# VisionLearningGroup/UDA_PoseEstimation

Hardware: AMD Instinct MI355X
Metric: images/sec (student+teacher step) 256x256 b=32 (higher is better)
Workload: dtype bf16; 1 GPU; pose_resnet101 K=16 mean-teacher step (student fwd+bwd on 2x32, teacher fwd on 32, JointsMSE+Cons, Adam, EMA), 256x256, b=32/GPU, no AdaIN (BASELINE.json configs[1]); global_batch=32, parallelism=dp1

## Files before the change

### include/udapose.h

```cpp
#ifndef UDAPOSE_H
#define UDAPOSE_H
#include <stddef.h>
#include <stdint.h>
#ifdef __cplusplus
extern "C" {
#endif

#define UDAPOSE_OK 0
#define UDAPOSE_ERR_ARG (-1)
#define UDAPOSE_ERR_LAUNCH (-2)
#define UDAPOSE_ERR_UNSUPPORTED (-3)
#define UDAPOSE_ERR_NOT_PREPARED (-4)

int udapose_version(void);
int udapose_elem_kind(void);

typedef struct {
    int igemm_tile;
    int igemm_h3;
    int igemm_lean;
    int igemm_short_lds;
    int igemm_tap0;
    int wgrad_tile;
    int wgrad_ksplit;
    int wgrad_fastgeo;
    int wgrad_group;
    int wgrad_stages;
    int wgrad_group_stem;
    int bn_bwd_fused;
    int bn_fwd_chunked;
    int bn_bwd_chunked;
    int bn_bwd_pre_legacy;
    int igemm_wg_min;
    int wgrad_row3;
    int bn3_mask;
    int stem_fused;
    int debug_sync;
    int igemm_big_min;
    int patch_conv;
    int eval_fold;
    int bn_xcd_rows;
    int wgrad_det;
    int igemm_ns3_k;
    void* timeline;
    int wgrad_order;
    int wgrad_fastgeo_strided;
} udapose_policy;
void udapose_policy_default(udapose_policy* p);

typedef struct {
    int N, Hi, Wi, Ci;
    int Co, KH, KW, stride, pad;
    int transposed;
    int reflect;
    int upsample;
    const udapose_policy* policy;
} udapose_conv_desc;
int udapose_conv_prepare(const udapose_conv_desc* d);

#define UDAPOSE_EPI_RELU 1
#define UDAPOSE_EPI_OUT_F32 2
#define UDAPOSE_EPI_F32 4
#define UDAPOSE_EPI_SPLIT 8
void udapose_conv_out_hw(const udapose_conv_desc* d, int* Ho, int* Wo);
int udapose_conv_stat_rows(const udapose_conv_desc* d);
int udapose_conv2d_fwd(void* stream, const udapose_conv_desc* d, const void* x, const void* w_fwd, void* y, const void* res,
                       const float* bias, float* stats, int epilogue_flags);
int udapose_conv2d_bwd_data(void* stream, const udapose_conv_desc* d, const void* dy, const void* w_bwd, void* dx, const void* res,
                            int out_f32);
int udapose_conv_bwd_stat_rows(const udapose_conv_desc* d);
int udapose_conv2d_bwd_data_bn(void* stream, const udapose_conv_desc* d, const void* dy, const void* w_bwd, void* dx, const void* res,
                               int out_f32, const void* bn_y, const void* bn_z, const float* bn_mean, const float* bn_invstd,
                               const float* bn_gamma, const float* bn_beta, float* slab);
int udapose_conv2d_bwd_weight(void* stream, const udapose_conv_desc* d, const void* dy, const void* x, float* dw, int accumulate);
int udapose_cast_f32_bf16(void* stream, const float* src, void* dst, size_t n);
int udapose_transpose_cast(void* stream, const float* src, void* dst, int A, int T, int B);
int udapose_pack_strided(void* stream, const float* src, void* dst, int A, int KH, int KWp, int KW, int Bp, int B, long sa, long skh,
                         long skw, long sb);

int udapose_nchw_f32_to_nhwc_bf16(void* stream, const float* src, void* dst, int N, int C, int HW, int Cpad);
int udapose_nchw_f32_to_nhwc_f32(void* stream, const float* src, float* dst, int N, int C, int HW, int Cpad);
int udapose_nchw_f32_to_nhwc_split(void* stream, const float* src, void* dst, int N, int C, int HW, int Cpad);
int udapose_f32_to_split(void* stream, const float* src, void* dst, size_t n);
int udapose_split_to_f32(void* stream, const void* src, float* dst, size_t n);
int udapose_nhwc_to_nchw_f32(void* stream, const void* src, int src_is_f32, float* dst, int N, int C, int HW, int Cstride,
                             const float* lo, const float* hi);

int udapose_bn_finalize(void* stream, const float* stats, int stat_rows, int C, double count, const float* gamma, const float* beta,
                        float* running_mean, float* running_var, long long* num_batches_tracked, float momentum, float eps,
                        float* scale, float* shift, float* save_mean, float* save_invstd);
int udapose_bn_eval_coeff(void* stream, int C, const float* gamma, const float* beta, const float* running_mean,
                          const float* running_var, float eps, float* scale, float* shift);
int udapose_bn_apply(void* stream, const void* y, const void* res, void* z, size_t numel, int C, const float* scale, const float* shift,
                     int relu);
int udapose_bn_bwd_rows(size_t npix);
int udapose_bn_bwd(void* stream, const void* dz, int dz_is_f32, const void* z, const void* y, void* dy, void* gout, size_t npix, int C,
                   const float* gamma, const float* save_mean, const float* save_invstd, int relu, float* slab, float* coef,
                   float* dgamma, float* dbeta, float beta_acc, const float* beta);
int udapose_bn_bwd_pre(void* stream, const void* g, int g_is_f32, const void* y, void* dy, size_t npix, int C, const float* gamma,
                       const float* save_mean, const float* save_invstd, const float* slab, int rows, float* coef, float* dgamma,
                       float* dbeta, float beta_acc);

int udapose_bn_train_fwd_ex(void* stream, int kind, const void* y, const void* res, void* z, size_t npix, int C, const float* slab, int rows,
                            const float* gamma, const float* beta, const float* pre_bias, float* running_mean, float* running_var,
                            long long* num_batches_tracked, float momentum, float eps, float* scale, float* shift, float* save, int relu,
                            int fwd_chunked, int xcd_rows, unsigned char* mask, void* y16, void* z16);
int udapose_bn_bwd_ex(void* stream, const void* dz, int dz_is_f32, const void* z, const void* y, void* dy, void* gout, size_t npix, int C,
                      const float* gamma, const float* save_mean, const float* save_invstd, int relu, float* slab, float* coef,
                      float* dgamma, float* dbeta, float beta_acc, const float* beta, int chunked);
int udapose_bn_bwd_pre_ex(void* stream, const void* g, int g_is_f32, const void* y, void* dy, size_t npix, int C, const float* gamma,
                          const float* save_mean, const float* save_invstd, const float* slab, int rows, float* coef, float* dgamma,
                          float* dbeta, float beta_acc, int chunked, int legacy);
int udapose_bn_relu_maxpool3x3s2(void* stream, const void* x, void* y, unsigned char* idx, int N, int H, int W, int C, const float* scale,
                                 const float* shift);
int udapose_bn_bwd_pooled(void* stream, const void* pool_dy, const unsigned char* pool_idx, int H, int W, const void* y, void* dy, size_t npix,
                          int C, const float* gamma, const float* save_mean, const float* save_invstd, float* slab, float* coef,
                          float* dgamma, float* dbeta, float beta_acc, const float* beta);
int udapose_bn_running_update(void* stream, const float* save, int C, float* running_mean, float* running_var,
                              long long* num_batches_tracked, float momentum);
int udapose_bn_running_update_multi(void* stream, const void* d_jobs, int njobs, int max_c, const void* act, float momentum);

int udapose_maxpool3x3s2_fwd(void* stream, const void* x, void* y, unsigned char* idx, int N, int H, int W, int C);
int udapose_maxpool3x3s2_fwd_ex(void* stream, int kind, const void* x, void* y, unsigned char* idx, int N, int H, int W, int C, void* y16);
int udapose_maxpool3x3s2_bwd(void* stream, const void* dy, const unsigned char* idx, void* dx, int N, int H, int W, int C);
int udapose_maxpool2x2_ceil(void* stream, const void* x, void* y, int N, int H, int W, int C);
int udapose_maxpool2x2_ceil_f32(void* stream, const float* x, float* y, int N, int H, int W, int C);
int udapose_maxpool2x2_ceil_split(void* stream, const void* x, void* y, int N, int H, int W, int C);

typedef void* udapose_net_t;
int udapose_net_create(const int layers[4], int num_keypoints, int N, int H, int W, int fp32, udapose_net_t* out);
void udapose_net_destroy(udapose_net_t net);
int udapose_net_num_params(udapose_net_t net);
int udapose_net_num_buffers(udapose_net_t net);
long long udapose_net_param_numel(udapose_net_t net, int i);
size_t udapose_net_wpack_bytes(udapose_net_t net);
size_t udapose_net_act_bytes(udapose_net_t net);
size_t udapose_net_ws_bytes(udapose_net_t net);
void udapose_net_out_shape(udapose_net_t net, int shape[4]);
int udapose_net_set_policy(udapose_net_t net, const udapose_policy* p);
int udapose_net_get_policy(udapose_net_t net, udapose_policy* p);
int udapose_net_bind(udapose_net_t net, const void* const* h_params, void* const* h_buffers, void* wpack);
int udapose_net_bind_grads(udapose_net_t net, void* const* h_grads);
int udapose_net_pack_weights(udapose_net_t net, void* stream, const void* const* h_params, void* wpack, int with_bwd);
int udapose_net_forward(udapose_net_t net, void* stream, const float* x_nchw, const void* const* h_params, void* const* h_buffers,
                        const void* wpack, void* act, void* ws, float* out_nchw, int training, float momentum);
int udapose_net_apply_running(udapose_net_t net, void* stream, const void* act, void* const* h_buffers, float momentum);
int udapose_axpy_f32(void* stream, float* y, const float* x, size_t n);
int udapose_net_backward(udapose_net_t net, void* stream, const float* dout_nchw, const void* const* h_params, const void* wpack,
                         void* act, void* ws, void* const* h_grads, float beta);
int udapose_net_backward_part(udapose_net_t net, void* stream, const float* dout_nchw, const void* const* h_params, const void* wpack,
                              void* act, void* ws, void* const* h_grads, float beta, int part);
int udapose_net_backward_phase(udapose_net_t net, void* stream, const float* dout_nchw, const void* const* h_params, const void* wpack,
                               void* act, void* ws, void* const* h_grads, float beta, int part, int phase);
int udapose_net_wgrad_pair(udapose_net_t net, void* stream, const void* act_a, void* ws_a, void* const* h_grads_a, float beta_a,
                           const void* act_b, void* ws_b, void* const* h_grads_b, float beta_b, int part);
int udapose_net_wgrad_pair_defer(udapose_net_t net, void* stream, const void* act_a, void* ws_a, void* const* h_grads_a, float beta_a,
                                 const void* act_b, void* ws_b, void* const* h_grads_b, float beta_b, int part, int* deferred);
int udapose_net_split_sum_flush(udapose_net_t net, void* stream);
int udapose_stem_dgrad(void* stream, const void* dy, const float* w, int N, int H, int W, float* dx);
int udapose_net_input_grad(udapose_net_t net, void* stream, const void* const* h_params, void* ws, float* dx);
#define UDAPOSE_PERTURB_L2 0
#define UDAPOSE_PERTURB_LINF 1
long long udapose_perturb_ws_bytes(int N, int C, int HW);
int udapose_perturb(void* stream, const float* x, const float* g, const float* x0, int N, int C, int HW, int mode, const float* eps_dev,
                    const float* step_dev, const float* lo, const float* hi, void* ws, float* out, float* gnorm);
int udapose_wgrad_deal(const int* nblk, const int* stages, int n_units, int order, int* ent_xcd, int* ent_unit, int* ent_first, int* ent_count, int cap,
                       double* finish_out);
long long udapose_net_grad_split_param(udapose_net_t net);

int udapose_joints_mse_fwd(void* stream, const float* pred, const float* gt, const float* w, int R, int HW, float* rows, float* mean_out);
int udapose_joints_mse_bwd(void* stream, const float* pred, const float* gt, const float* w, const float* gscale, int R, int HW,
                           float* dpred);
int udapose_cons_loss_fwd(void* stream, const float* stu, const float* tea, const unsigned char* mask, int R, int HW, float* rows,
                          float* mean_out);
int udapose_cons_loss_bwd(void* stream, const float* stu, const float* tea, const unsigned char* mask, const float* gscale, int R,
                          int HW, float* dstu);
int udapose_mask_count(void* stream, const unsigned char* mask, size_t n, float* count);
int udapose_cons_loss_valid_fwd(void* stream, const float* stu, const float* tea, const unsigned char* mask, const unsigned char* valid,
                                const float* valid_count, int R, int K, int HW, float* rows, float* mean_out);
int udapose_cons_loss_valid_bwd(void* stream, const float* stu, const float* tea, const unsigned char* mask, const unsigned char* valid,
                                const float* valid_count, const float* gscale, int R, int K, int HW, float* dstu);
int udapose_joints_kl_fwd(void* stream, const float* pred, const float* gt, const float* w, float epsilon, int R, int group, int HW, float* rows,
                          float* stats, float* out);
int udapose_joints_kl_bwd(void* stream, const float* pred, const float* gt, const float* w, float epsilon, const float* stats,
                          const float* gscale, int R, int HW, float* dpred);
int udapose_entropy_loss_fwd(void* stream, const float* x, int R, int group, int HW, float threshold, float* rows, float* stats, float* out,
                             float* count);
int udapose_entropy_loss_bwd(void* stream, const float* x, const float* rows, const float* stats, const float* count, const float* gscale,
                             float threshold, int R, int HW, float* dx);
int udapose_cons_softmax_fwd(void* stream, const float* stu, const float* tea, const unsigned char* mask, const unsigned char* valid,
                             const float* valid_count, int R, int K, int HW, float* rows, float* stats, float* out);
// ... 198 lines not shown
```

### uda_poseestimation_amd/_hip.py

```python
import ctypes as C
import os

import torch

_HERE = os.path.dirname(os.path.abspath(__file__))
LIB_PATH = os.path.join(_HERE, "libudapose_hip.so")
LIB_PATHS = {"bf16": LIB_PATH, "fp16": os.path.join(_HERE, "libudapose_hip_f16.so")}
_libs = {}

vp, ci, cf, cd, sz, ll, cl = C.c_void_p, C.c_int, C.c_float, C.c_double, C.c_size_t, C.c_longlong, C.c_long


class Policy(C.Structure):
    _fields_ = [(k, C.c_int) for k in ("igemm_tile", "igemm_h3", "igemm_lean", "igemm_short_lds", "igemm_tap0", "wgrad_tile", "wgrad_ksplit",
                                       "wgrad_fastgeo", "wgrad_group", "wgrad_stages", "wgrad_group_stem", "bn_bwd_fused", "bn_fwd_chunked",
                                       "bn_bwd_chunked", "bn_bwd_pre_legacy", "igemm_wg_min", "wgrad_row3", "bn3_mask", "stem_fused", "debug_sync", "igemm_big_min", "patch_conv",
                                       "eval_fold", "bn_xcd_rows", "wgrad_det", "igemm_ns3_k")] + [("timeline", C.c_void_p), ("wgrad_order", C.c_int),
                                                                                                   ("wgrad_fastgeo_strided", C.c_int)]


def policy(**overrides):
    p = Policy()
    lib().udapose_policy_default(C.byref(p))
    for k, v in overrides.items():
        if k not in dict(Policy._fields_):
            raise KeyError(f"udapose_policy has no field {k!r}")
        setattr(p, k, v)
    return p


class ConvDesc(C.Structure):
    _fields_ = [(k, C.c_int) for k in ("N", "Hi", "Wi", "Ci", "Co", "KH", "KW", "stride", "pad", "transposed", "reflect", "upsample")] + \
               [("policy", C.POINTER(Policy))]


_SIGS = {
    "udapose_version": (ci, []),
    "udapose_elem_kind": (ci, []),
    "udapose_grad_scaler_check": (ci, [vp, vp, vp, vp, vp, ci, vp]),
    "udapose_grad_scaler_check2": (ci, [vp, vp, vp, vp, vp, ci, vp, ll]),
    "udapose_grad_scaler_update": (ci, [vp, vp, cf, cf, ci]),
    "udapose_grad_sumsq": (ci, [vp, vp, vp, vp, vp, ci, ll, vp, vp]),
    "udapose_grad_clip": (ci, [vp, vp, vp, vp, ci, vp, vp]),
    "udapose_grad_clip_restore": (ci, [vp, ci, vp, vp]),
    "udapose_policy_default": (None, [vp]),
    "udapose_conv_prepare": (ci, [vp]),
    "udapose_net_set_policy": (ci, [vp, vp]),
    "udapose_net_get_policy": (ci, [vp, vp]),
    "udapose_net_bind": (ci, [vp, vp, vp, vp]),
    "udapose_net_bind_grads": (ci, [vp, vp]),
    "udapose_conv_out_hw": (None, [vp, vp, vp]),
    "udapose_conv_stat_rows": (ci, [vp]),
    "udapose_conv2d_fwd": (ci, [vp, vp, vp, vp, vp, vp, vp, vp, ci]),
    "udapose_conv2d_bwd_data": (ci, [vp, vp, vp, vp, vp, vp, ci]),
    "udapose_conv_bwd_stat_rows": (ci, [vp]),
    "udapose_conv2d_bwd_data_bn": (ci, [vp, vp, vp, vp, vp, vp, ci, vp, vp, vp, vp, vp, vp, vp]),
    "udapose_conv2d_bwd_weight": (ci, [vp, vp, vp, vp, vp, ci]),
    "udapose_cast_f32_bf16": (ci, [vp, vp, vp, sz]),
    "udapose_transpose_cast": (ci, [vp, vp, vp, ci, ci, ci]),
    "udapose_pack_strided": (ci, [vp, vp, vp, ci, ci, ci, ci, ci, ci, cl, cl, cl, cl]),
    "udapose_nchw_f32_to_nhwc_bf16": (ci, [vp, vp, vp, ci, ci, ci, ci]),
    "udapose_nchw_f32_to_nhwc_f32": (ci, [vp, vp, vp, ci, ci, ci, ci]),
    "udapose_nhwc_to_nchw_f32": (ci, [vp, vp, ci, vp, ci, ci, ci, ci, vp, vp]),
    "udapose_nchw_f32_to_nhwc_split": (ci, [vp, vp, vp, ci, ci, ci, ci]),
    "udapose_f32_to_split": (ci, [vp, vp, vp, sz]),
    "udapose_split_to_f32": (ci, [vp, vp, vp, sz]),
    "udapose_maxpool2x2_ceil_split": (ci, [vp, vp, vp, ci, ci, ci, ci]),
    "udapose_adain_split": (ci, [vp, vp, vp, vp, ci, ci, ci, ci, cf, cf, vp, vp]),
    "udapose_bn_finalize": (ci, [vp, vp, ci, ci, cd, vp, vp, vp, vp, vp, cf, cf, vp, vp, vp, vp]),
    "udapose_bn_eval_coeff": (ci, [vp, ci, vp, vp, vp, vp, cf, vp, vp]),
    "udapose_bn_apply": (ci, [vp, vp, vp, vp, sz, ci, vp, vp, ci]),
    "udapose_bn_bwd_rows": (ci, [sz]),
    "udapose_bn_bwd": (ci, [vp, vp, ci, vp, vp, vp, vp, sz, ci, vp, vp, vp, ci, vp, vp, vp, vp, cf, vp]),
    "udapose_bn_bwd_pre": (ci, [vp, vp, ci, vp, vp, sz, ci, vp, vp, vp, vp, ci, vp, vp, vp, cf]),
    "udapose_bn_train_fwd_ex": (ci, [vp, ci, vp, vp, vp, sz, ci, vp, ci, vp, vp, vp, vp, vp, vp, cf, cf, vp, vp, vp, ci, ci, ci, vp, vp, vp]),
    "udapose_bn_bwd_ex": (ci, [vp, vp, ci, vp, vp, vp, vp, sz, ci, vp, vp, vp, ci, vp, vp, vp, vp, cf, vp, ci]),
    "udapose_bn_bwd_pre_ex": (ci, [vp, vp, ci, vp, vp, sz, ci, vp, vp, vp, vp, ci, vp, vp, vp, cf, ci, ci]),
    "udapose_bn_relu_maxpool3x3s2": (ci, [vp, vp, vp, vp, ci, ci, ci, ci, vp, vp]),
    "udapose_bn_bwd_pooled": (ci, [vp, vp, vp, ci, ci, vp, vp, sz, ci, vp, vp, vp, vp, vp, vp, vp, cf, vp]),
    "udapose_bn_running_update": (ci, [vp, vp, ci, vp, vp, vp, cf]),
    "udapose_bn_running_update_multi": (ci, [vp, vp, ci, ci, vp, cf]),
    "udapose_maxpool3x3s2_fwd_ex":(ci, [vp, ci, vp, vp, vp, ci, ci, ci, ci, vp]),
    "udapose_maxpool3x3s2_fwd": (ci, [vp, vp, vp, vp, ci, ci, ci, ci]),
    "udapose_maxpool3x3s2_bwd": (ci, [vp, vp, vp, vp, ci, ci, ci, ci]),
    "udapose_maxpool2x2_ceil": (ci, [vp, vp, vp, ci, ci, ci, ci]),
    "udapose_maxpool2x2_ceil_f32": (ci, [vp, vp, vp, ci, ci, ci, ci]),
    "udapose_net_create": (ci, [vp, ci, ci, ci, ci, ci, vp]),
    "udapose_net_destroy": (None, [vp]),
    "udapose_net_num_params": (ci, [vp]),
    "udapose_net_num_buffers": (ci, [vp]),
    "udapose_net_param_numel": (ll, [vp, ci]),
    "udapose_net_wpack_bytes": (sz, [vp]),
    "udapose_net_act_bytes": (sz, [vp]),
    "udapose_net_ws_bytes": (sz, [vp]),
    "udapose_net_out_shape": (None, [vp, vp]),
    "udapose_net_pack_weights": (ci, [vp, vp, vp, vp, ci]),
    "udapose_net_forward": (ci, [vp, vp, vp, vp, vp, vp, vp, vp, vp, ci, cf]),
    "udapose_net_apply_running": (ci, [vp, vp, vp, vp, cf]),
    "udapose_axpy_f32": (ci, [vp, vp, vp, sz]),
    "udapose_net_backward": (ci, [vp, vp, vp, vp, vp, vp, vp, vp, cf]),
    "udapose_net_backward_part": (ci, [vp, vp, vp, vp, vp, vp, vp, vp, cf, ci]),
    "udapose_net_backward_phase": (ci, [vp, vp, vp, vp, vp, vp, vp, vp, cf, ci, ci]),
    "udapose_net_wgrad_pair": (ci, [vp, vp, vp, vp, vp, cf, vp, vp, vp, cf, ci]),
    "udapose_net_wgrad_pair_defer": (ci, [vp, vp, vp, vp, vp, cf, vp, vp, vp, cf, ci, vp]),
    "udapose_net_split_sum_flush": (ci, [vp, vp]),
    "udapose_stem_dgrad": (ci, [vp, vp, vp, ci, ci, ci, vp]),
    "udapose_net_input_grad": (ci, [vp, vp, vp, vp, vp]),
    "udapose_perturb_ws_bytes": (ll, [ci, ci, ci]),
    "udapose_perturb": (ci, [vp, vp, vp, vp, ci, ci, ci, ci, vp, vp, vp, vp, vp, vp, vp]),
    "udapose_wgrad_deal": (ci, [vp, vp, ci, ci, vp, vp, vp, vp, ci, vp]),
    "udapose_net_grad_split_param": (ll, [vp]),
    "udapose_net_bind_update": (ci, [vp, vp, vp, vp, vp, vp, vp, vp, vp]),
    "udapose_net_fused_update": (ci, [vp, vp, vp, vp, vp, vp, vp, vp, vp, cf, cf, cf, cf, cf, ci, cf, vp, cf, cf, ci, ll]),
    "udapose_net_bind_update_groups": (ci, [vp, vp, ci, vp, vp, vp, vp, vp, vp, vp, vp]),
    "udapose_net_fused_update_groups": (ci, [vp, vp, vp, ci, vp, vp, vp, vp, vp, vp, cf, cf, cf, ci, ci, vp, vp, cf, cf, ci, ll]),
    "udapose_net_fused_update_dev": (ci, [vp, vp, vp, vp, vp, vp, vp, vp, vp, cf, cf, cf, cf, cf, ci, cf, vp, vp, ci, ll]),
    "udapose_net_fused_update_groups_dev": (ci, [vp, vp, vp, ci, vp, vp, vp, vp, vp, vp, cf, cf, cf, ci, ci, vp, vp, vp, ci, ll]),
    "udapose_joints_mse_fwd": (ci, [vp, vp, vp, vp, ci, ci, vp, vp]),
    "udapose_joints_mse_bwd": (ci, [vp, vp, vp, vp, vp, ci, ci, vp]),
    "udapose_cons_loss_fwd": (ci, [vp, vp, vp, vp, ci, ci, vp, vp]),
    "udapose_cons_loss_bwd": (ci, [vp, vp, vp, vp, vp, ci, ci, vp]),
    "udapose_mask_count": (ci, [vp, vp, sz, vp]),
    "udapose_cons_loss_valid_fwd": (ci, [vp, vp, vp, vp, vp, vp, ci, ci, ci, vp, vp]),
    "udapose_cons_loss_valid_bwd": (ci, [vp, vp, vp, vp, vp, vp, vp, ci, ci, ci, vp]),
    "udapose_joints_kl_fwd": (ci, [vp, vp, vp, vp, cf, ci, ci, ci, vp, vp, vp]),
    "udapose_joints_kl_bwd": (ci, [vp, vp, vp, vp, cf, vp, vp, ci, ci, vp]),
    "udapose_entropy_loss_fwd": (ci, [vp, vp, ci, ci, ci, cf, vp, vp, vp, vp]),
    "udapose_entropy_loss_bwd": (ci, [vp, vp, vp, vp, vp, vp, cf, ci, ci, vp]),
    "udapose_cons_softmax_fwd": (ci, [vp, vp, vp, vp, vp, vp, ci, ci, ci, vp, vp, vp]),
    "udapose_cons_softmax_bwd": (ci, [vp, vp, vp, vp, vp, vp, vp, vp, ci, ci, ci, vp]),
    "udapose_cons_kl_fwd": (ci, [vp, vp, vp, vp, vp, vp, ci, ci, ci, ci, vp, vp, vp]),
    "udapose_cons_kl_bwd": (ci, [vp, vp, vp, vp, vp, vp, ci, vp, vp, ci, ci, ci, vp]),
    "udapose_coral_ws_bytes": (ll, [ci, ci, ci, ci, ci]),
    "udapose_coral_fwd": (ci, [vp, vp, vp, ci, ci, ci, ci, ci, vp, vp, vp]),
    "udapose_coral_bwd": (ci, [vp, vp, vp, vp, vp, ci, ci, ci, ci, ci, vp, vp]),
    "udapose_soft_argmax_fwd": (ci, [vp, vp, ci, ci, ci, cf, ci, vp, vp, vp, vp]),
    "udapose_soft_argmax_bwd": (ci, [vp, vp, vp, vp, vp, ci, ci, ci, cf, ci, vp]),
    "udapose_coord_loss_fwd": (ci, [vp, vp, vp, vp, vp, ci, ci, ci, ci, cf, ci, ci, vp, vp, vp, vp]),
    "udapose_coord_loss_bwd": (ci, [vp, vp, vp, vp, vp, vp, vp, vp, ci, ci, ci, cf, ci, ci, vp]),
    "udapose_heatmap_argmax": (ci, [vp, vp, ci, ci, ci, vp, vp, vp, vp, vp, ci]),
    "udapose_prior_weights": (ci, [vp, vp, ci, cf, cf, ci, vp]),
    "udapose_prior_map": (ci, [vp, vp, vp, vp, vp, vp, ci, ci, ci, ci, cf, ci, vp]),
    "udapose_pair_dist_accumulate": (ci, [vp, vp, vp, ci, ci, vp]),
    "udapose_pair_dist_finish": (ci, [vp, vp, ci, vp, vp]),
    "udapose_hflip_batch": (ci, [vp, vp, vp, ci, sz, ci, ci]),
    "udapose_flip_merge": (ci, [vp, vp, vp, vp, ci, ci, ci, ci, ci, ci, vp, vp, vp, vp]),
    "udapose_refine_decode": (ci, [vp, vp, ci, ci, ci, ci, ci, cf, vp, vp, vp]),
    "udapose_kth_mask": (ci, [vp, vp, vp, ci, ci, vp, vp, vp, ci]),
# ... 126 lines not shown
```

### uda_poseestimation_amd/csrc/capi.hip

```cpp
#include <cstdio>
#include "net.h"
#include "pointwise.h"
#include "losses.h"
#include "optim.h"
#include "style.h"
#include "data.h"
#include "../../include/udapose.h"

static Policy from_c(const udapose_policy& c) {
    Policy p;
    static_cast<udapose_policy&>(p) = c;
    if (p.wgrad_stages <= 0) p.wgrad_stages = 128;
    return p;
}
static void to_c(const Policy& p, udapose_policy* c) { *c = p; }
struct Geom {
    Policy pol;
    ConvGeom g;
    explicit Geom(const udapose_conv_desc* d)
        : g{d->N, d->Hi, d->Wi, d->Ci, d->Co, d->KH, d->KW, d->stride, d->pad, d->transposed, d->reflect, d->upsample} {
        if (d->policy) { pol = from_c(*d->policy); g.pol = &pol; }
    }
};
#define S(x) ((hipStream_t)(x))
// ... 70 lines not shown
}
int udapose_bn_bwd_pre(void* stream, const void* g, int g_is_f32, const void* y, void* dy, size_t npix, int C, const float* gamma, const float* mean,
                       const float* invstd, const float* slab, int rows, float* coef, float* dgamma, float* dbeta, float beta_acc) {
    if (!g || !y || !dy || !gamma || !mean || !invstd || !slab || !coef) return UDAPOSE_ERR_ARG;
    return pw_bn_bwd_pre(S(stream), g, g_is_f32, CB16(y), B16(dy), npix, C, gamma, mean, invstd, slab, rows, coef, dgamma, dbeta, beta_acc,
                         default_policy().bn_bwd_chunked, default_policy().bn_bwd_pre_legacy);
}
int udapose_bn_train_fwd_ex(void* stream, int kind, const void* y, const void* res, void* z, size_t npix, int C, const float* slab, int rows,
                            const float* gamma, const float* beta, const float* pre_bias, float* running_mean, float* running_var,
                            long long* num_batches_tracked, float momentum, float eps, float* scale, float* shift, float* save, int relu,
                            int fwd_chunked, int xcd_rows, unsigned char* mask, void* y16, void* z16) {
    if (!y || !z || !slab || !gamma || !beta || !scale || !shift || !save || npix < 1 || rows < 1 || C < 8 || C % 8 || kind < 0 || kind > 3)
        return UDAPOSE_ERR_ARG;
    if ((kind == 3) != (y16 != nullptr) || (kind == 3) != (z16 != nullptr) || (mask && (kind == 1 || kind == 2))) return UDAPOSE_ERR_ARG;
    if (kind == 3 && UDAPOSE_ELEM_KIND != 1) return UDAPOSE_ERR_UNSUPPORTED;
    const int chunked = fwd_chunked | (xcd_rows ? (1 << 30) : 0);
    int took = 0;
    if (kind == 0 && !pre_bias)
        took = pw_bn_train_fused(S(stream), CB16(y), CB16(res), B16(z), npix, C, slab, rows, gamma, beta, running_mean, running_var,
                                 num_batches_tracked, momentum, eps, save, relu, chunked, mask);
    else if (kind >= 2 && !pre_bias)
        took = pw_bn_train_fused_split(S(stream), (const float*)y, res, z, npix, C, slab, rows, gamma, beta, running_mean, running_var,
                                       num_batches_tracked, momentum, eps, save, relu, chunked, y16, z16, mask);
    if (took < 0) return took;
    if (took) return 1 | (xcd_rows ? 2 : 0);
    int rc = pw_bn_finalize(S(stream), slab, rows, C, (double)npix, gamma, beta, running_mean, running_var, num_batches_tracked, momentum, eps, scale,
                            shift, save, save + C, pre_bias);
    if (rc != UDAPOSE_OK) return rc;
    const int xcd = xcd_rows >= 2;
    if (kind == 0) rc = pw_bn_apply(S(stream), CB16(y), CB16(res), B16(z), npix * C, C, scale, shift, relu, mask, xcd);
    else if (kind == 1) rc = pw_bn_apply_f32(S(stream), (const float*)y, (const float*)res, (float*)z, npix * C, C, scale, shift, relu);
    else rc = pw_bn_apply_split(S(stream), (const float*)y, res, z, npix * C, C, scale, shift, relu, y16, z16, mask, xcd);
    if (rc != UDAPOSE_OK) return rc;
    return (xcd && (kind == 0 || kind == 3) && pw_bn_apply_xcd_ok(npix * (C / 8), C)) ? 2 : 0;
}
int udapose_bn_bwd_ex(void* stream, const void* dz, int dz_is_f32, const void* z, const void* y, void* dy, void* gout, size_t npix, int C,
                      const float* gamma, const float* mean, const float* invstd, int relu, float* slab, float* coef, float* dgamma, float* dbeta,
                      float beta_acc, const float* beta, int chunked) {
    if (!dz || !y || !dy || !gamma || !mean || !invstd || !slab || !coef || npix < 1 || C < 8) return UDAPOSE_ERR_ARG;
    const int rc = pw_bn_bwd(S(stream), dz, dz_is_f32, CB16(z), CB16(y), B16(dy), B16(gout), npix, C, gamma, mean, invstd, relu, slab, coef, dgamma,
                             dbeta, beta_acc, beta, chunked);
    return rc != UDAPOSE_OK ? rc : pw_bn_bwd_takes_chunked(npix, C, chunked);
}
int udapose_bn_bwd_pre_ex(void* stream, const void* g, int g_is_f32, const void* y, void* dy, size_t npix, int C, const float* gamma,
                          const float* mean, const float* invstd, const float* slab, int rows, float* coef, float* dgamma, float* dbeta,
                          float beta_acc, int chunked, int legacy) {
    if (!g || !y || !dy || !gamma || !mean || !invstd || !slab || !coef || npix < 1 || C < 8) return UDAPOSE_ERR_ARG;
    const int rc = pw_bn_bwd_pre(S(stream), g, g_is_f32, CB16(y), B16(dy), npix, C, gamma, mean, invstd, slab, rows, coef, dgamma, dbeta, beta_acc,
                                 chunked, legacy);
    if (rc != UDAPOSE_OK) return rc;
    if (pw_bn_bwd_pre_takes_chunked(npix, C, rows, chunked)) return 1 | (((chunked >> 30) & 1) ? 2 : 0);
    return (!legacy && ((chunked >> 29) & 1) && pw_bn_apply_xcd_ok(npix * (C / 8), C)) ? 2 : 0;
}
int udapose_bn_relu_maxpool3x3s2(void* stream, const void* x, void* y, unsigned char* idx, int N, int H, int W, int C, const float* scale,
                                 const float* shift) {
    if (!x || !y || !scale || !shift || N < 1 || H < 1 || W < 1 || C < 8) return UDAPOSE_ERR_ARG;
    return pw_bn_relu_maxpool3x3s2(S(stream), CB16(x), B16(y), idx, N, H, W, C, scale, shift);
}
int udapose_bn_bwd_pooled(void* stream, const void* pool_dy, const unsigned char* pool_idx, int H, int W, const void* y, void* dy, size_t npix, int C,
                          const float* gamma, const float* mean, const float* invstd, float* slab, float* coef, float* dgamma, float* dbeta,
                          float beta_acc, const float* beta) {
    if (!pool_dy || !pool_idx || !y || !dy || !gamma || !mean || !invstd || !slab || !coef || H < 1 || W < 1 || npix < 1 || C < 8) return UDAPOSE_ERR_ARG;
    return pw_bn_bwd_pooled(S(stream), CB16(pool_dy), pool_idx, H, W, CB16(y), B16(dy), npix, C, gamma, mean, invstd, slab, coef, dgamma, dbeta,
                            beta_acc, beta);
}
int udapose_bn_running_update(void* stream, const float* save, int C, float* running_mean, float* running_var, long long* num_batches_tracked,
                              float momentum) {
    if (!save || !running_mean || !running_var || C < 1) return UDAPOSE_ERR_ARG;
    return pw_bn_running_update(S(stream), save, C, running_mean, running_var, num_batches_tracked, momentum);
}
int udapose_bn_running_update_multi(void* stream, const void* d_jobs, int njobs, int max_c, const void* act, float momentum) {
    if (!d_jobs || !act || njobs < 1 || max_c < 1) return UDAPOSE_ERR_ARG;
    return pw_bn_running_update_multi(S(stream), (const BnRunJob*)d_jobs, njobs, max_c, act, momentum);
}
int udapose_maxpool3x3s2_fwd_ex(void* stream, int kind, const void* x, void* y, unsigned char* idx, int N, int H, int W, int C, void* y16) {
    if (!x || !y || N < 1 || H < 1 || W < 1 || C < 8 || C % 8 || kind < 0 || kind > 3 || (kind == 3) != (y16 != nullptr)) return UDAPOSE_ERR_ARG;
    if (kind == 3 && UDAPOSE_ELEM_KIND != 1) return UDAPOSE_ERR_UNSUPPORTED;
    if (kind == 0) return pw_maxpool3x3s2_fwd(S(stream), CB16(x), B16(y), idx, N, H, W, C);
    if (kind == 1) return pw_maxpool3x3s2_fwd_f32(S(stream), (const float*)x, (float*)y, idx, N, H, W, C);
    return pw_maxpool3x3s2_fwd_split(S(stream), x, y, idx, N, H, W, C, y16);
}
int udapose_maxpool3x3s2_fwd(void* stream, const void* x, void* y, unsigned char* idx, int N, int H, int W, int C) {
    return pw_maxpool3x3s2_fwd(S(stream), CB16(x), B16(y), idx, N, H, W, C);
}
int udapose_maxpool3x3s2_bwd(void* stream, const void* dy, const unsigned char* idx, void* dx, int N, int H, int W, int C) {
    return pw_maxpool3x3s2_bwd(S(stream), CB16(dy), idx, B16(dx), N, H, W, C);
}
int udapose_maxpool2x2_ceil(void* stream, const void* x, void* y, int N, int H, int W, int C) {
    return pw_maxpool2x2_ceil(S(stream), CB16(x), B16(y), N, H, W, C);
}
int udapose_maxpool2x2_ceil_f32(void* stream, const float* x, float* y, int N, int H, int W, int C) {
    return pw_maxpool2x2_ceil_f32(S(stream), x, y, N, H, W, C);
}
int udapose_nchw_f32_to_nhwc_f32(void* stream, const float* src, float* dst, int N, int C, int HW, int Cpad) {
    return pw_nchw_f32_to_nhwc_f32(S(stream), src, dst, N, C, HW, Cpad);
}
int udapose_nchw_f32_to_nhwc_split(void* stream, const float* src, void* dst, int N, int C, int HW, int Cpad) {
    if (!src || !dst) return UDAPOSE_ERR_ARG;
    return pw_nchw_f32_to_nhwc_split(S(stream), src, dst, N, C, HW, Cpad);
}
int udapose_f32_to_split(void* stream, const float* src, void* dst, size_t n) {
    if (!src || !dst) return UDAPOSE_ERR_ARG;
    return pw_f32_to_split(S(stream), src, dst, n);
}
int udapose_split_to_f32(void* stream, const void* src, float* dst, size_t n) {
    if (!src || !dst) return UDAPOSE_ERR_ARG;
    return pw_split_to_f32(S(stream), src, dst, n);
}
int udapose_maxpool2x2_ceil_split(void* stream, const void* x, void* y, int N, int H, int W, int C) {
    if (!x || !y) return UDAPOSE_ERR_ARG;
    return pw_maxpool2x2_ceil_split(S(stream), x, y, N, H, W, C);
}

int udapose_net_create(const int layers[4], int K, int N, int H, int W, int fp32, udapose_net_t* out) {
    if (!out) return UDAPOSE_ERR_ARG;
    *out = net_create(layers, K, N, H, W, fp32);
    return *out ? UDAPOSE_OK : UDAPOSE_ERR_ARG;
}
void udapose_net_destroy(udapose_net_t n) { net_destroy(n); }
int udapose_net_set_policy(udapose_net_t n, const udapose_policy* p) {
    if (!n || !p) return UDAPOSE_ERR_ARG;
    net_set_policy(n, from_c(*p));
    return UDAPOSE_OK;
}
int udapose_net_get_policy(udapose_net_t n, udapose_policy* p) {
    if (!n || !p) return UDAPOSE_ERR_ARG;
    to_c(net_get_policy(n), p);
    return UDAPOSE_OK;
}
int udapose_net_bind(udapose_net_t n, const void* const* params, void* const* buffers, void* wpack) {
    if (!n || !params || !wpack) return UDAPOSE_ERR_ARG;
    return net_bind(n, params, buffers, wpack);
}
int udapose_net_bind_grads(udapose_net_t n, void* const* grads) {
    if (!n || !grads) return UDAPOSE_ERR_ARG;
    return net_bind_grads(n, grads);
}
int udapose_net_num_params(udapose_net_t n) { return net_num_params(n); }
int udapose_net_num_buffers(udapose_net_t n) { return net_num_buffers(n); }
long long udapose_net_param_numel(udapose_net_t n, int i) { return net_param_numel(n, i); }
size_t udapose_net_wpack_bytes(udapose_net_t n) { return net_wpack_bytes(n); }
size_t udapose_net_act_bytes(udapose_net_t n) { return net_act_bytes(n); }
size_t udapose_net_ws_bytes(udapose_net_t n) { return net_ws_bytes(n); }
void udapose_net_out_shape(udapose_net_t n, int shape[4]) { net_out_shape(n, shape); }
int udapose_net_pack_weights(udapose_net_t n, void* stream, const void* const* params, void* wpack, int with_bwd) {
    return net_pack_weights(n, S(stream), params, wpack, with_bwd);
}
int udapose_net_forward(udapose_net_t n, void* stream, const float* x, const void* const* params, void* const* buffers, const void* wpack, void* act,
                        void* ws, float* out, int training, float momentum) {
    return net_forward(n, S(stream), x, params, buffers, wpack, act, ws, out, training, momentum);
}
int udapose_net_apply_running(udapose_net_t n, void* stream, const void* act, void* const* buffers, float momentum) {
    return net_apply_running(n, S(stream), act, buffers, momentum);
}
int udapose_axpy_f32(void* stream, float* y, const float* x, size_t n) { return pw_axpy(S(stream), y, x, n); }
int udapose_net_backward(udapose_net_t n, void* stream, const float* dout, const void* const* params, const void* wpack, void* act, void* ws,
                         void* const* grads, float beta) {
    return net_backward(n, S(stream), dout, params, wpack, act, ws, grads, beta, 0, 0);
}
int udapose_net_backward_part(udapose_net_t n, void* stream, const float* dout, const void* const* params, const void* wpack, void* act,
                              void* ws, void* const* grads, float beta, int part) {
    if (part != 1 && part != 2) return UDAPOSE_ERR_ARG;
    return net_backward(n, S(stream), dout, params, wpack, act, ws, grads, beta, part, 0);
}
int udapose_net_wgrad_pair(udapose_net_t n, void* stream, const void* act_a, void* ws_a, void* const* grads_a, float beta_a, const void* act_b,
                           void* ws_b, void* const* grads_b, float beta_b, int part) {
    if (!n || !act_a || !ws_a || !grads_a || !act_b || !ws_b || !grads_b) return UDAPOSE_ERR_ARG;
    return net_wgrad_pair(n, S(stream), act_a, ws_a, grads_a, beta_a, act_b, ws_b, grads_b, beta_b, part);
}
int udapose_net_wgrad_pair_defer(udapose_net_t n, void* stream, const void* act_a, void* ws_a, void* const* grads_a, float beta_a, const void* act_b,
                                 void* ws_b, void* const* grads_b, float beta_b, int part, int* deferred) {
    if (!n || !act_a || !ws_a || !grads_a || !act_b || !ws_b || !grads_b) return UDAPOSE_ERR_ARG;
    return net_wgrad_pair_defer(n, S(stream), act_a, ws_a, grads_a, beta_a, act_b, ws_b, grads_b, beta_b, part, deferred);
}
int udapose_net_split_sum_flush(udapose_net_t n, void* stream) { return n ? net_split_sum_flush(n, S(stream)) : UDAPOSE_ERR_ARG; }
int udapose_wgrad_deal(const int* nblk, const int* stages, int n_units, int order, int* ent_xcd, int* ent_unit, int* ent_first, int* ent_count, int cap,
                       double* finish_out) {
    return net_wgrad_deal(nblk, stages, n_units, order, ent_xcd, ent_unit, ent_first, ent_count, cap, finish_out);
}
int udapose_net_backward_phase(udapose_net_t n, void* stream, const float* dout, const void* const* params, const void* wpack, void* act,
                               void* ws, void* const* grads, float beta, int part, int phase) {
    if (!n) return UDAPOSE_ERR_ARG;
    return net_backward(n, S(stream), dout, params, wpack, act, ws, grads, beta, part, phase);
}
int udapose_stem_dgrad(void* stream, const void* dy, const float* w, int N, int H, int W, float* dx) {
    return stem_dgrad(S(stream), (const elem_t*)dy, w, N, H, W, dx);
}
int udapose_net_input_grad(udapose_net_t n, void* stream, const void* const* params, void* ws, float* dx) {
    if (!n || !params || !ws || !dx) return UDAPOSE_ERR_ARG;
    return net_input_grad(n, S(stream), params, ws, dx);
}
long long udapose_perturb_ws_bytes(int N, int C, int HW) { return perturb_ws_bytes(N, C, HW); }
int udapose_perturb(void* stream, const float* x, const float* g, const float* x0, int N, int C, int HW, int mode, const float* eps_dev,
                    const float* step_dev, const float* lo, const float* hi, void* ws, float* out, float* gnorm) {
    return perturb(S(stream), x, g, x0, N, C, HW, mode, eps_dev, step_dev, lo, hi, ws, out, gnorm);
}
long long udapose_net_grad_split_param(udapose_net_t n) { return net_grad_split_param(n); }
// ... 421 lines not shown
```

### uda_poseestimation_amd/csrc/conv_plan.h

```cpp
#pragma once
#include <atomic>
#include <mutex>
#include <vector>
#include "igemm.h"

struct Policy : udapose_policy {
    Policy() : udapose_policy{} {
        igemm_tile = -1; igemm_h3 = 1; igemm_lean = 1; igemm_short_lds = 1; igemm_tap0 = 1;
        wgrad_tile = -1; wgrad_ksplit = -1; wgrad_fastgeo = 2;
        wgrad_group = 1; wgrad_stages = 128; wgrad_group_stem = 1;
        bn_bwd_fused = 1; bn_fwd_chunked = 1; bn_bwd_chunked = 1; bn_bwd_pre_legacy = 0;
        igemm_wg_min = 512; wgrad_row3 = 1; bn3_mask = 1; stem_fused = 1; debug_sync = 0;
        igemm_big_min = 0; patch_conv = 2; eval_fold = 1; bn_xcd_rows = 1; wgrad_det = 1; igemm_ns3_k = 0;
        timeline = nullptr; wgrad_order = 1; wgrad_fastgeo_strided = 1;
    }
};
inline const Policy& default_policy() { static const Policy p; return p; }

template <auto Kernel>
inline void max_dynamic_lds(int bytes) {
    static std::atomic<unsigned long long> done{0};
    static std::mutex mu;
    int dev = 0;
    (void)hipGetDevice(&dev);
    const unsigned long long bit = 1ull << (dev & 63);
    if (done.load(std::memory_order_acquire) & bit) return;
    std::lock_guard<std::mutex> lk(mu);
    if (done.load(std::memory_order_relaxed) & bit) return;
    (void)hipFuncSetAttribute((const void*)Kernel, hipFuncAttributeMaxDynamicSharedMemorySize, bytes);
    done.fetch_or(bit, std::memory_order_release);
}

struct ConvGeom {
    int N, Hi, Wi, Ci;
    int Co, KH, KW, stride, pad;
    int transposed;
    int reflect;
    int upsample;
    const Policy* pol = nullptr;
    const Policy& policy() const { return pol ? *pol : default_policy(); }
    int Ho() const { return transposed ? (Hi - 1) * stride - 2 * pad + KH : (((Hi << upsample) + 2 * pad - KH) / stride + 1); }
    int Wo() const { return transposed ? (Wi - 1) * stride - 2 * pad + KW : (((Wi << upsample) + 2 * pad - KW) / stride + 1); }
    bool smallc() const { return Ci == 8; }
    int KWp() const { return smallc() ? ((KW + 7) & ~7) : KW; }
    int wtaps() const { return KH * KWp(); }
};

struct TapPlan {
    std::vector<IgTap> taps;
    int nclass = 1;
    IgClass cls[4];
    const IgTap* d_taps = nullptr;
};

const TapPlan* get_tap_plan(const ConvGeom& g, int direction, hipStream_t stream = nullptr);
int conv_prepare(const ConvGeom& g);

int igemm_pick_tile(int M, int Co, int nclass, int K, int h3_ok, const Policy& pol);
int conv_h3_ok(const ConvGeom& g);
int igemm_stat_rows(int M, int Co, int nclass, int tile);
int igemm_launch(IgParams& p, int tile, hipStream_t stream, const Policy& pol);
int wgrad_pick_tile(int Rdim, int Cdim, int smallc, const Policy& pol);
int wgrad_launch(WgParams& p, int tile, int accumulate, hipStream_t stream, const Policy& pol);
int wgrad_parts_plan(int M, int Ci, int Co, int total_taps, int* tile_out);
int wgrad_launch_parts(WgParams& p, float* parts, hipStream_t stream);
#define WG_STAMP_BLOCKS (1 << 17)
#define WG_CLASSES 2
// ... 39 lines not shown
```

### uda_poseestimation_amd/csrc/net.h

```cpp
#pragma once
#include "conv_plan.h"

void* net_create(const int layers[4], int K, int N, int H, int W, int mode);
void net_destroy(void* h);
void net_set_policy(void* h, const Policy& p);
const Policy& net_get_policy(void* h);
int net_num_params(void* h);
int net_num_buffers(void* h);
long long net_param_numel(void* h, int i);
size_t net_wpack_bytes(void* h);
size_t net_act_bytes(void* h);
size_t net_ws_bytes(void* h);
void net_out_shape(void* h, int* shp);
int net_bind(void* h, const void* const* params, void* const* buffers, void* wpack_);
int net_pack_weights(void* h, hipStream_t s, const void* const* params, void* wpack_, int with_bwd);
int net_forward(void* h, hipStream_t s, const float* x_nchw, const void* const* params, void* const* buffers, const void* wpack_, void* act_, void* ws_,
                float* out_nchw, int training, float momentum);
int net_wgrad_pair(void* h, hipStream_t s, const void* actA, void* wsA, void* const* gradsA, float betaA, const void* actB, void* wsB,
                   void* const* gradsB, float betaB, int part);
int net_wgrad_pair_defer(void* h, hipStream_t s, const void* actA, void* wsA, void* const* gradsA, float betaA, const void* actB, void* wsB,
                         void* const* gradsB, float betaB, int part, int* deferred);
int net_split_sum_flush(void* h, hipStream_t s);
int net_wgrad_deal(const int* nblk, const int* stages, int n_units, int order, int* ent_xcd, int* ent_unit, int* ent_first, int* ent_count, int cap,
                   double* finish_out);
int net_backward(void* h, hipStream_t s, const float* dout_nchw, const void* const* params, const void* wpack_, void* act_, void* ws_,
                 void* const* grads, float beta, int part, int phase);
int net_input_grad(void* h, hipStream_t s, const void* const* params, void* ws_, float* dx);
int net_apply_running(void* h, hipStream_t s, const void* act_, void* const* buffers, float momentum);
int net_bind_grads(void* h, void* const* grads);
long long net_grad_split_param(void* h);
int net_bind_update_groups(void* hs, void* ht, int kind, void* const* params_s, void* const* grads, void* const* h_m, void* const* h_v,
                           void* const* params_t, void* wpack_s_, void* wpack_t_, const int* group_idx);
int net_bind_update(void* hs, void* ht, void* const* params_s, void* const* grads, void* const* h_m, void* const* h_v, void* const* params_t,
                    void* wpack_s_, void* wpack_t_);
int net_fused_update(void* hs, void* ht, hipStream_t s, void* const* params_s, void* const* grads, void* const* h_m, void* const* params_t,
                     void* wpack_s_, void* wpack_t_, float lr, float beta1, float beta2, float eps, float wd, int step, float gscale,
                     float* dev_state, float alpha, float oma, int do_adam, long long grad2_delta, const float* ema_dev);
int net_fused_update_groups(void* hs, void* ht, hipStream_t s, int kind, void* const* params_s, void* const* grads, void* const* h_m,
                            void* const* params_t, void* wpack_s_, void* wpack_t_, float beta1, float beta2, float eps, int nesterov, int ngroups,
                            float* const* states, const float* wds, float alpha, float oma, int do_opt, long long grad2_delta, const float* ema_dev);
int prof_before(hipStream_t s, int kind, double flops);
void prof_after(hipStream_t s, int token);
void prof_begin();
int prof_end(double* out);
```

### uda_poseestimation_amd/csrc/net.hip

```cpp
#include <algorithm>
#include <deque>
#include <functional>
#include <queue>
#include <cstdio>
#include <cstdlib>
#include <string>
#include <type_traits>
#include <vector>
#include "net.h"
#include "pointwise.h"
#include "optim.h"

namespace {

inline size_t align_up(size_t v, size_t a = 256) { return (v + a - 1) / a * a; }
static thread_local int t_dbg_sync = 0;
struct DbgSyncScope { int prev; explicit DbgSyncScope(int on) : prev(t_dbg_sync) { t_dbg_sync = on; } ~DbgSyncScope() { t_dbg_sync = prev; } };
#define CK(expr) do { int _e = (expr); \
    if (t_dbg_sync) { fprintf(stderr, "[udapose] net.hip:%d %s\n", __LINE__, #expr); fflush(stderr); \
        if (hipDeviceSynchronize() != hipSuccess) { fprintf(stderr, "[udapose] FAILED at net.hip:%d\n", __LINE__); return UDAPOSE_ERR_LAUNCH; } } \
    if (_e != UDAPOSE_OK) return _e; } while (0)

struct ConvL {
    ConvGeom g;
// ... 241 lines not shown
        for (int k = 0; k < SC_COUNT; ++k) n.sc.off[k] = act_alloc(n, n.sc.need[k]);
    }
    const int hw_out = layout(n);
    const int Hc = hw_out >> 16, Wc = hw_out & 0xffff;

    size_t max_slab = 0, max_act = 0;
    auto upd = [&](const ConvL& c) {
        const size_t rows = (size_t)conv_stat_rows(c.g);
        max_slab = std::max(max_slab, rows * 2 * c.g.Co * 4);
        max_act = std::max(max_act, (size_t)n.N * c.g.Ho() * c.g.Wo() * c.g.Co * 2);
        max_act = std::max(max_act, (size_t)n.N * c.g.Hi * c.g.Wi * c.g.Ci * 2);
    };
    for_each_conv(n, upd);
    max_slab = std::max(max_slab, (size_t)1024 * 2 * 2048 * 4);
    size_t o = 0;
    n.ws_slab = o; o = align_up(o + max_slab);
    n.ws_slabf = o; o = align_up(o + max_slab);
    n.ws_coef = o; o = align_up(o + (size_t)3 * 2048 * 4 + 2 * 2048 * 4);
    for_each_conv(n, [&](ConvL& c) { c.g.pol = &n.policy; });
    n.head.g.pol = &n.policy;
    if (n.fwd_only) {
        n.ws_bytes = o;
        return np;
    }
    n.gbuf_bytes = align_up(2 * max_act);
    for (int i = 0; i < 6; ++i) { n.ws_gbuf[i] = o; o += n.gbuf_bytes; }
    n.ws_dyhead = o; o = align_up(o + (size_t)N * Hc * Wc * 64 * 2);
    n.ws_dwtmp = o; o = align_up(o + std::max((size_t)64 * 56 * 8 * 4, (size_t)64 * 256 * 4));
    auto dyb = [&](ConvL& c) { c.dy_off = o; o = align_up(o + (size_t)n.N * c.g.Ho() * c.g.Wo() * c.g.Co * 2); };
    for_each_conv(n, dyb);
    n.ws_wgpart = o;
    n.ws_bytes = o;
    return np;
}

struct Pool {
    char* base; size_t off[6]; bool used[6] = {false, false, false, false, false, false};
    elem_t* get() { for (int i = 0; i < 6; ++i) if (!used[i]) { used[i] = true; return (elem_t*)(base + off[i]); } return nullptr; }
    void put(const void* p) { for (int i = 0; i < 6; ++i) if ((char*)p == base + off[i]) used[i] = false; }
};

int pack_conv(hipStream_t s, const Net& n, const ConvL& c, const void* const* params, char* wpack) {
    const float* w = (const float*)params[c.w_idx];
    const ConvGeom& g = c.g;
    if (g.smallc()) {
        if (n.f32 == 2) return pw_pack_strided_split(s, w, wpack + c.wf_off, g.Co, g.KH, g.KWp(), g.KW, 8, 3, (long)g.KH * g.KW * 3, (long)g.KW * 3, 3, 1);
        if (n.f32) return pw_pack_strided_f32(s, w, (float*)(wpack + c.wf_off), g.Co, g.KH, g.KWp(), g.KW, 8, 3, (long)g.KH * g.KW * 3, (long)g.KW * 3, 3, 1);
        return pw_pack_strided(s, w, (elem_t*)(wpack + c.wf_off), g.Co, g.KH, g.KWp(), g.KW, 8, 3, (long)g.KH * g.KW * 3, (long)g.KW * 3, 3, 1);
    }
    if (n.f32 != 1) return UDAPOSE_ERR_UNSUPPORTED;
    return g.transposed ? pw_transpose_f32(s, w, (float*)(wpack + c.wf_off), g.Ci, g.KH * g.KW, g.Co) : UDAPOSE_OK;
}

int conv_bn_fwd(hipStream_t s, const Net& n, const ConvL& c, const BnL& b, const void* const* params, void* const* buffers, const char* wpack,
                char* act, char* ws, int training, float momentum, const elem_t* res, int relu, bool upd, bool no_apply = false) {
    ConvEpilogue e;
    float* slab = (float*)(ws + n.ws_slab);
    float* scale = (float*)(ws + n.ws_coef);
    float* shift = scale + 2048;
    float* save = (float*)(act + b.save_off);
    e.stats = training ? slab : nullptr;
    e.f32 = n.f32 != 0;
    e.split = n.f32 == 2;
    e.out_f32 = n.f32 == 2;
    const float* pre_bias = c.bias_idx >= 0 ? (const float*)params[c.bias_idx] : nullptr;
    e.bias = pre_bias;
    unsigned char* mask = (b.mask_off && n.policy.bn3_mask && relu) ? (unsigned char*)(act + b.mask_off) : nullptr;
    const bool sh = n.strict && training;
    void* y16 = sh ? (void*)(act + c.y_off) : nullptr;
    void* z16 = sh ? (void*)(act + b.z_off) : nullptr;
    const void* wptr = (n.f32 == 1 && !c.g.smallc() && !c.g.transposed) ? params[c.w_idx] : (const void*)(wpack + c.wf_off);
    const float* gamma = (const float*)params[b.g_idx];
    const float* beta = (const float*)params[b.b_idx];
    float* rm = upd ? (float*)buffers[b.rm_idx] : nullptr;
    float* rv = upd ? (float*)buffers[b.rv_idx] : nullptr;
    long long* nbt = upd ? (long long*)buffers[b.nbt_idx] : nullptr;
    const int chunked = n.policy.bn_fwd_chunked | (n.policy.bn_xcd_rows ? (1 << 30) : 0);
    if (!training && !no_apply && !pre_bias && n.policy.eval_fold) {
        CK(pw_bn_eval_coeff(s, b.C, gamma, beta, (const float*)buffers[b.rm_idx], (const float*)buffers[b.rv_idx], 1e-5f, scale, shift));
        e.stats = nullptr;
        e.scale = scale; e.bias = shift; e.relu = relu;
        e.res = res;
        e.out_f32 = 0;
        return conv_fprop(s, c.g, (const elem_t*)(act + c.fin_off), (const elem_t*)wptr, act + b.fz_off, e);
    }
    CK(conv_fprop(s, c.g, (const elem_t*)(act + c.fin_off), (const elem_t*)wptr, act + c.fy_off, e));
    if (training && !n.f32 && !no_apply && !pre_bias) {
        const int took = pw_bn_train_fused(s, (const elem_t*)(act + c.y_off), res, (elem_t*)(act + b.z_off), b.npix, b.C, slab, conv_stat_rows(c.g), gamma,
                                           beta, rm, rv, nbt, momentum, 1e-5f, save, relu, chunked, mask);
        if (took < 0) return took;
        if (took) return UDAPOSE_OK;
    }
    if (training && n.f32 == 2 && !no_apply && !pre_bias) {
        const int took = pw_bn_train_fused_split(s, (const float*)(act + c.fy_off), res, act + b.fz_off, b.npix, b.C, slab, conv_stat_rows(c.g), gamma, beta,
                                                 rm, rv, nbt, momentum, 1e-5f, save, relu, chunked, y16, z16, sh ? mask : nullptr);
        if (took < 0) return took;
        if (took) return UDAPOSE_OK;
    }
    if (training)
        CK(pw_bn_finalize(s, slab, conv_stat_rows(c.g), b.C, (double)b.npix, gamma, beta, rm, rv, nbt, momentum, 1e-5f, scale, shift, save,
                          save + b.C, pre_bias));
    else
        CK(pw_bn_eval_coeff(s, b.C, gamma, beta, (const float*)buffers[b.rm_idx], (const float*)buffers[b.rv_idx], 1e-5f, scale, shift));
    if (no_apply) return UDAPOSE_OK;
    if (n.f32 == 2)
        return pw_bn_apply_split(s, (const float*)(act + c.fy_off), res, act + b.fz_off, b.npix * b.C, b.C, scale, shift, relu, y16, z16, sh ? mask : nullptr,
                                 n.policy.bn_xcd_rows >= 2);
    if (n.f32)
        return pw_bn_apply_f32(s, (const float*)(act + c.y_off), (const float*)res, (float*)(act + b.z_off), b.npix * b.C, b.C, scale, shift, relu);
    return pw_bn_apply(s, (const elem_t*)(act + c.y_off), res, (elem_t*)(act + b.z_off), b.npix * b.C, b.C, scale, shift, relu, mask, n.policy.bn_xcd_rows >= 2);
}

}

void* net_create(const int layers[4], int K, int N, int H, int W, int mode) {
    if (K < 1 || K > 64 || N < 1 || H % 32 || W % 32 || (mode & 0xff) > 3 || (mode >> 10)) return nullptr;
    if ((mode & 0xff) == 3 && ((mode >> 9) & 1 || UDAPOSE_ELEM_KIND != 1)) return nullptr;
    return build(layers, K, N, H, W, mode);
}
void net_destroy(void* h) {
    delete (Net*)h;
}
void net_set_policy(void* h, const Policy& p) { ((Net*)h)->policy = p; }
const Policy& net_get_policy(void* h) { return ((Net*)h)->policy; }
int net_num_params(void* h) { return ((Net*)h)->n_params; }
int net_num_buffers(void* h) { return ((Net*)h)->n_buffers; }
long long net_param_numel(void* h, int i) { return ((Net*)h)->param_numel[i]; }
size_t net_wpack_bytes(void* h) { return ((Net*)h)->wpack_bytes; }
size_t net_act_bytes(void* h) { return ((Net*)h)->act_bytes; }
namespace { size_t wg_partial_bytes(Net& n); }
size_t net_ws_bytes(void* h) {
    Net& n = *(Net*)h;
    if ((n.f32 && !n.strict) || n.fwd_only || !n.policy.wgrad_group || !n.policy.wgrad_det) { n.ws_wgpart_bytes = 0; return n.ws_bytes; }
    n.ws_wgpart_bytes = wg_partial_bytes(n);
    return n.ws_bytes + n.ws_wgpart_bytes;
}
void net_out_shape(void* h, int* shp) { Net& n = *(Net*)h; shp[0] = n.N; shp[1] = n.K; shp[2] = n.Hout; shp[3] = n.Wout; }

namespace {
void add_pack_jobs(const Net& n, const ConvL& c, const void* const* params, char* wpack, bool with_bwd, std::vector<PackJobH>& jobs) {
    const ConvGeom& g = c.g;
    if (g.smallc()) return;
    const float* w = (const float*)params[c.w_idx];
    const int T = g.KH * g.KW;
    elem_t* wf = (elem_t*)(wpack + c.wf_off);
    elem_t* wb = (elem_t*)(wpack + c.wb_off);
    const int sp = n.f32 == 2 ? 2 : 0;
    if (sp && !n.strict) with_bwd = false;
    if (!g.transposed) {
        jobs.push_back(PackJobH{w, wf, 0, 0, 0, sp, (long long)g.Co * T * g.Ci});
        if (with_bwd) jobs.push_back(PackJobH{w, wb, g.Co, T, g.Ci, 1, 0});
    } else {
        jobs.push_back(PackJobH{w, wf, g.Ci, T, g.Co, 1 | sp, 0});
        if (with_bwd) jobs.push_back(PackJobH{w, wb, 0, 0, 0, 0, (long long)g.Ci * T * g.Co});
    }
}
int build_pack_table(Net& n, Net::PackTab& tab, const void* const* params, char* wpack, bool with_bwd) {
    std::vector<PackJobH> jobs;
    for_each_conv(n, [&](const ConvL& c) { add_pack_jobs(n, c, params, wpack, with_bwd, jobs); });
    jobs.push_back(PackJobH{(const float*)params[n.head.w_idx], (elem_t*)(wpack + n.head.wf_off), 0, 0, 0, n.f32 == 2 ? 2 : 0, (long long)n.K * 256});
    std::vector<int> bj, bs;
    for (size_t j = 0; j < jobs.size(); ++j) {
        const PackJobH& q = jobs[j];
        const long nb = (q.kind & 1) == 0 ? (long)((q.n + 8191) / 8192) : (long)((q.A + 31) / 32) * ((q.B + 31) / 32) * q.T;
        for (long k = 0; k < nb; ++k) { bj.push_back((int)j); bs.push_back((int)k); }
    }
    CK(tab.upload(jobs, bj, bs));
    tab.key0 = params[0]; tab.key1 = params[n.n_params - 1]; tab.keyw = wpack;
    return UDAPOSE_OK;
}
int build_run_jobs(Net& n, void* const* buffers) {
    std::vector<BnRunJob> jobs;
    for_each_bn(n, [&](const BnL& b) {
        jobs.push_back(BnRunJob{b.save_off, (float*)buffers[b.rm_idx], (float*)buffers[b.rv_idx], (long long*)buffers[b.nbt_idx], b.C, 0});
    });
    CK(n.d_runjobs.upload(jobs));
    n.runjobs_key = buffers[0];
    return UDAPOSE_OK;
}
}

int net_bind(void* h, const void* const* params, void* const* buffers, void* wpack_) {
    Net& n = *(Net*)h;
    char* wpack = (char*)wpack_;
    CK(for_each_conv(n, [](const ConvL& c) { return conv_prepare(c.g); }));
    { ConvGeom hg = n.head.g; CK(conv_prepare(hg)); hg.Co = 64; CK(conv_prepare(hg)); }
    if (n.f32 != 1) {
        CK(build_pack_table(n, n.pack_fwd, params, wpack, false));
// ... 2 lines not shown
    if (buffers) CK(build_run_jobs(n, buffers));
    return UDAPOSE_OK;
}

int net_pack_weights(void* h, hipStream_t s, const void* const* params, void* wpack_, int with_bwd) {
    Net& n = *(Net*)h;
    DbgSyncScope dbg(n.policy.debug_sync);
    char* wpack = (char*)wpack_;
    if (n.f32 != 1) {
        if (n.f32 == 2 && !n.strict) with_bwd = 0;
        Net::PackTab& tab = with_bwd ? n.pack_all : n.pack_fwd;
        if (!tab.jobs.d || tab.key0 != params[0] || tab.key1 != params[n.n_params - 1] || tab.keyw != (const void*)wpack)
            return UDAPOSE_ERR_NOT_PREPARED;
        CK(pack_conv(s, n, n.stem, params, wpack));
        CK(pw_pack_multi(s, tab.jobs.d, tab.blk_job.d, tab.blk_sub.d, tab.nblocks()));
        if (with_bwd)
            CK(pw_pack_strided(s, (const float*)params[n.head.w_idx], (elem_t*)(wpack + n.head.wb_off), 256, 1, 1, 1, 64, n.K, 1, 0, 0, 256));
        return UDAPOSE_OK;
    }
    return for_each_conv(n, [&](const ConvL& c) -> int { CK(pack_conv(s, n, c, params, wpack)); return UDAPOSE_OK; });
}

int net_forward(void* h, hipStream_t s, const float* x_nchw, const void* const* params, void* const* buffers, const void* wpack_, void* act_, void* ws_,
                float* out_nchw, int training, float momentum) {
    const Net& n = *(const Net*)h;
    DbgSyncScope dbg(n.policy.debug_sync);
    const bool upd = !(training & 2);
    training &= 1;
    const char* wpack = (const char*)wpack_;
    char* act = (char*)act_;
    char* ws = (char*)ws_;
    const bool sh = n.strict && training;
    if (n.f32 == 2) CK(pw_nchw_f32_to_nhwc_split(s, x_nchw, act + n.fx8_off, n.N, 3, n.H * n.W, 8, sh ? act + n.x8_off : nullptr));
    else if (n.f32) CK(pw_nchw_f32_to_nhwc_f32(s, x_nchw, (float*)(act + n.x8_off), n.N, 3, n.H * n.W, 8));
    else CK(pw_nchw_f32_to_nhwc_bf16(s, x_nchw, (elem_t*)(act + n.x8_off), n.N, 3, n.H * n.W, 8));
    const bool stem_fused = n.policy.stem_fused && !n.f32;
    CK(conv_bn_fwd(s, n, n.stem, n.stem_bn, params, buffers, wpack, act, ws, training, momentum, nullptr, 1, upd, stem_fused));
    if (stem_fused)
        CK(pw_bn_relu_maxpool3x3s2(s, (const elem_t*)(act + n.stem.y_off), (elem_t*)(act + n.pool_off), (unsigned char*)(act + n.poolidx_off), n.N,
                                   n.Hs, n.Ws, 64, (const float*)(ws + n.ws_coef), (const float*)(ws + n.ws_coef) + 2048));
    else if (n.f32 == 2)
        CK(pw_maxpool3x3s2_fwd_split(s, act + n.stem_bn.fz_off, act + n.fpool_off, (unsigned char*)(act + n.poolidx_off), n.N, n.Hs, n.Ws, 64,
                                     sh ? act + n.pool_off : nullptr));
    else if (n.f32)
        CK(pw_maxpool3x3s2_fwd_f32(s, (const float*)(act + n.stem_bn.z_off), (float*)(act + n.pool_off), (unsigned char*)(act + n.poolidx_off), n.N,
                                   n.Hs, n.Ws, 64));
    else
        CK(pw_maxpool3x3s2_fwd(s, (const elem_t*)(act + n.stem_bn.z_off), (elem_t*)(act + n.pool_off), (unsigned char*)(act + n.poolidx_off), n.N,
                               n.Hs, n.Ws, 64));
    for (auto& b : n.blocks) {
        CK(conv_bn_fwd(s, n, b.c1, b.b1, params, buffers, wpack, act, ws, training, momentum, nullptr, 1, upd));
        CK(conv_bn_fwd(s, n, b.c2, b.b2, params, buffers, wpack, act, ws, training, momentum, nullptr, 1, upd));
        const elem_t* res = (const elem_t*)(act + b.fin_off);
        if (b.has_ds) {
            CK(conv_bn_fwd(s, n, b.cd, b.bd, params, buffers, wpack, act, ws, training, momentum, nullptr, 0, upd));
            res = (const elem_t*)(act + b.fzd_off);
        }
        CK(conv_bn_fwd(s, n, b.c3, b.b3, params, buffers, wpack, act, ws, training, momentum, res, 1, upd));
    }
    for (int i = 0; i < 3; ++i) CK(conv_bn_fwd(s, n, n.up[i], n.up_bn[i], params, buffers, wpack, act, ws, training, momentum, nullptr, 1, upd));
    ConvEpilogue e;
    e.bias = (const float*)params[n.head.bias_idx];
    e.out_f32 = 1;
    e.f32 = n.f32 != 0;
    e.split = n.f32 == 2;
    const void* hwp = n.f32 == 1 ? params[n.head.w_idx] : (const void*)(wpack + n.head.wf_off);
    CK(conv_fprop(s, n.head.g, (const elem_t*)(act + n.head.fin_off), (const elem_t*)hwp, act + n.head_out_off, e));
    return pw_nhwc_to_nchw_f32(s, act + n.head_out_off, 1, out_nchw, n.N, n.K, n.Hout * n.Wout, n.K, nullptr, nullptr);
}

namespace {
int conv_bn_bwd(hipStream_t s, const Net& n, const ConvL& c, const BnL& b, const void* const* params, const char* wpack, char* act, char* ws,
                void* const* grads, float beta, Pool& pool, const void* dz, int dz_f32, elem_t* gout, int relu, const elem_t* dx_res,
                elem_t** dx_out, bool need_dx, int dx_f32, bool grouped_wgrad, const DgradBnStat* pre = nullptr, DgradBnStat* next = nullptr) {
    float* slab = (float*)(ws + n.ws_slab);
    float* coef = (float*)(ws + n.ws_coef) + 4096;
    const float* save = (const float*)(act + b.save_off);
    elem_t* dy = (elem_t*)(ws + c.dy_off);
    if (pre)
        CK(pw_bn_bwd_pre(s, dz, dz_f32, (const elem_t*)(act + c.y_off), dy, b.npix, b.C, (const float*)params[b.g_idx], save, save + b.C, pre->slab,
                         pre->rows, coef, (float*)grads[b.g_idx], (float*)grads[b.b_idx], beta, n.policy.bn_bwd_chunked | (n.policy.bn_xcd_rows ? (1 << 30) : 0) | (n.policy.bn_xcd_rows >= 2 ? (1 << 29) : 0),
                         n.policy.bn_bwd_pre_legacy));
    else
        CK(pw_bn_bwd(s, dz, dz_f32, (const elem_t*)(act + b.z_off), (const elem_t*)(act + c.y_off), dy, gout, b.npix, b.C, (const float*)params[b.g_idx],
                     save, save + b.C, relu, slab, coef, (float*)grads[b.g_idx], (float*)grads[b.b_idx], beta, (const float*)params[b.b_idx],
                     n.policy.bn_bwd_chunked));
    const elem_t* xin = (const elem_t*)(act + c.in_off);
    if (c.bias_idx >= 0 && beta == 0.f) {
        if (pw_zero(s, grads[c.bias_idx], (size_t)c.g.Co * sizeof(float)) != UDAPOSE_OK) return UDAPOSE_ERR_LAUNCH;
    }
    if (c.g.smallc() && grouped_wgrad && n.policy.wgrad_group_stem) {
    } else if (c.g.smallc()) {
        float* tmp = (float*)(ws + n.ws_dwtmp);
        CK(conv_wgrad(s, c.g, dy, xin, tmp, 0, -1));
        CK(pw_unpack_strided(s, tmp, (float*)grads[c.w_idx], c.g.Co, c.g.KH, c.g.KWp(), c.g.KW, 8, 3, (long)c.g.KH * c.g.KW * 3, (long)c.g.KW * 3, 3, 1,
                             beta));
    } else if (!grouped_wgrad) {
        CK(conv_wgrad(s, c.g, dy, xin, (float*)grads[c.w_idx], beta != 0.f, -1));
    }
    if (need_dx) {
        elem_t* dx = pool.get();
        if (!dx) return UDAPOSE_ERR_ARG;
        CK(conv_dgrad(s, c.g, dy, (const elem_t*)(wpack + c.wb_off), dx, dx_res, dx_f32, next));
        *dx_out = dx;
    }
    return UDAPOSE_OK;
}

DgradBnStat bn_stat_of(const Net& n, const ConvL& c, const BnL& b, const void* const* params, char* act, char* ws, int relu) {
    DgradBnStat st;
    const float* save = (const float*)(act + b.save_off);
    st.y = (const elem_t*)(act + c.y_off);
    st.z = relu == 1 ? (const elem_t*)(act + b.z_off) : nullptr;
    st.mask = (relu == 1 && b.mask_off && n.policy.bn3_mask) ? (const unsigned char*)(act + b.mask_off) : nullptr;
    st.mean = save; st.invstd = save + b.C;
    st.gamma = (const float*)params[b.g_idx]; st.beta = (const float*)params[b.b_idx];
    st.slab = (float*)(ws + n.ws_slabf);
    return st;
}


inline int split_block(const Net& n) { return n.layers[0] + n.layers[1]; }

struct PartSel { bool head_up; int hi, lo; bool stem; };
PartSel part_sel(const Net& n, int part) {
    const int nb = (int)n.blocks.size(), split = split_block(n);
    if (part == 1) return PartSel{true, nb - 1, split, false};
    if (part == 2) return PartSel{false, split - 1, 0, true};
    return PartSel{true, nb - 1, 0, true};
}
template <class N, class F> int for_each_conv_wgrad(N& n, const PartSel& sel, F fn) {
    int rc = UDAPOSE_OK;
    for (int i = 2; sel.head_up && rc == UDAPOSE_OK && i >= 0; --i) rc = walk_rc(fn, n.up[i]);
    for (int bi = sel.hi; rc == UDAPOSE_OK && bi >= sel.lo; --bi) {
        auto& b = n.blocks[bi];
// ... 354 lines not shown
    char* ws = (char*)ws_;
    Pool pool;
    pool.base = ws;
    for (int i = 0; i < 6; ++i) pool.off[i] = n.ws_gbuf[i];
    const bool grouped = n.policy.wgrad_group != 0;
    if (grouped && (!find_wg_group(n, grads, beta, part))) return UDAPOSE_ERR_NOT_PREPARED;
    const int HWo = n.Hout * n.Wout;
    const int split = split_block(n);
    const bool fused = n.policy.bn_bwd_fused != 0;
    DgradBnStat cur, nxt;
    bool have = false;
    elem_t* dz = nullptr;
    if (part != 2) {
    elem_t* dyh = (elem_t*)(ws + n.ws_dyhead);
    CK(pw_nchw_f32_to_nhwc_bf16(s, dout_nchw, dyh, n.N, n.K, HWo, 64));
    ConvGeom hg = n.head.g;
    hg.Co = 64;
    float* tmp = (float*)(ws + n.ws_dwtmp);
    if (!grouped) {
        CK(conv_wgrad(s, hg, dyh, (const elem_t*)(act + n.head.in_off), tmp, 0, n.K));
        CK(pw_unpack_strided(s, tmp, (float*)grads[n.head.w_idx], n.K, 1, 1, 1, 256, 256, 256, 0, 0, 1, beta));
    }
    dz = pool.get();
    if (fused) { cur = bn_stat_of(n, n.up[2], n.up_bn[2], params, act, ws, 2); have = true; }
    CK(conv_dgrad(s, hg, dyh, (const elem_t*)(wpack + n.head.wb_off), dz, nullptr, 1, have ? &cur : nullptr));
    CK(pw_plane_sum(s, dout_nchw, (float*)grads[n.head.bias_idx], n.N, n.K, HWo, beta));
    for (int i = 2; i >= 0; --i) {
        elem_t* dx = nullptr;
        if (fused) {
            if (i > 0) nxt = bn_stat_of(n, n.up[i - 1], n.up_bn[i - 1], params, act, ws, 2);
            else nxt = bn_stat_of(n, n.blocks.back().c3, n.blocks.back().b3, params, act, ws, 1);
        }
        CK(conv_bn_bwd(s, n, n.up[i], n.up_bn[i], params, wpack, act, ws, grads, beta, pool, dz, 1, nullptr, 2, nullptr, &dx, true, i > 0, grouped,
                       have ? &cur : nullptr, fused ? &nxt : nullptr));
        if (fused) cur = nxt;
        pool.put(dz);
        dz = dx;
    }
    } else {
        if (split < 1 || split >= (int)n.blocks.size() || n.split_dz_idx < 0) return UDAPOSE_ERR_ARG;
        pool.used[n.split_dz_idx] = true;
        dz = (elem_t*)(ws + pool.off[n.split_dz_idx]);
        if (fused) {
            cur = bn_stat_of(n, n.blocks[split - 1].c3, n.blocks[split - 1].b3, params, act, ws, 1);
            cur.rows = conv_dgrad_stat_rows(n.blocks[split].c1.g);
            have = true;
        }
    }
    const int bi_hi = part == 2 ? split - 1 : (int)n.blocks.size() - 1, bi_lo = part == 1 ? split : 0;
    for (int bi = bi_hi; bi >= bi_lo; --bi) {
        Block& b = n.blocks[bi];
        elem_t *dz2 = nullptr, *dz1 = nullptr, *dxd = nullptr, *dxin = nullptr;
        if (fused) nxt = bn_stat_of(n, b.c2, b.b2, params, act, ws, 2);
        CK(conv_bn_bwd(s, n, b.c3, b.b3, params, wpack, act, ws, grads, beta, pool, dz, 0, dz, 1, nullptr, &dz2, true, 0, grouped, have ? &cur : nullptr,
                       fused ? &nxt : nullptr));
        if (fused) { cur = nxt; nxt = bn_stat_of(n, b.c1, b.b1, params, act, ws, 2); }
        CK(conv_bn_bwd(s, n, b.c2, b.b2, params, wpack, act, ws, grads, beta, pool, dz2, 0, nullptr, 2, nullptr, &dz1, true, 0, grouped,
                       have ? &cur : nullptr, fused ? &nxt : nullptr));
        if (fused) cur = nxt;
        pool.put(dz2);
        const elem_t* skip = dz;
        if (b.has_ds) {
            CK(conv_bn_bwd(s, n, b.cd, b.bd, params, wpack, act, ws, grads, beta, pool, dz, 0, nullptr, 0, nullptr, &dxd, true, 0, grouped));
            skip = dxd;
        }
        const bool chain = fused && bi > 0;
        if (chain) nxt = bn_stat_of(n, n.blocks[bi - 1].c3, n.blocks[bi - 1].b3, params, act, ws, 1);
        CK(conv_bn_bwd(s, n, b.c1, b.b1, params, wpack, act, ws, grads, beta, pool, dz1, 0, nullptr, 2, skip, &dxin, true, 0, grouped,
                       have ? &cur : nullptr, chain ? &nxt : nullptr));
        if (chain) cur = nxt;
        pool.put(dz1);
        if (dxd) pool.put(dxd);
        pool.put(dz);
        dz = dxin;
    }
    if (part == 1) {
        for (int i = 0; i < 6; ++i) if ((char*)dz == ws + pool.off[i]) n.split_dz_idx = i;
        if (grouped && phase == 0) CK(run_wg_group(s, n, act, ws, grads, beta, 1));
        if (beta == 0.f) {
            if (pw_zero(s, grads[n.fc_w_idx], (size_t)1000 * 2048 * 4) != UDAPOSE_OK) return UDAPOSE_ERR_LAUNCH;
            if (pw_zero(s, grads[n.fc_b_idx], (size_t)1000 * 4) != UDAPOSE_OK) return UDAPOSE_ERR_LAUNCH;
        }
        return UDAPOSE_OK;
    }
    if (n.policy.stem_fused >= 2 && grouped && n.policy.wgrad_group_stem) {
        const BnL& sb = n.stem_bn;
        const float* save = (const float*)(act + sb.save_off);
        CK(pw_bn_bwd_pooled(s, dz, (const unsigned char*)(act + n.poolidx_off), n.Hs, n.Ws, (const elem_t*)(act + n.stem.y_off),
                            (elem_t*)(ws + n.stem.dy_off), sb.npix, sb.C, (const float*)params[sb.g_idx], save, save + sb.C, (float*)(ws + n.ws_slab),
                            (float*)(ws + n.ws_coef) + 4096, (float*)grads[sb.g_idx], (float*)grads[sb.b_idx], beta, (const float*)params[sb.b_idx]));
        pool.put(dz);
    } else {
    elem_t* dzs = pool.get();
    CK(pw_maxpool3x3s2_bwd(s, dz, (const unsigned char*)(act + n.poolidx_off), dzs, n.N, n.Hs, n.Ws, 64));
    pool.put(dz);
    elem_t* none = nullptr;
    CK(conv_bn_bwd(s, n, n.stem, n.stem_bn, params, wpack, act, ws, grads, beta, pool, dzs, 0, nullptr, 2, nullptr, &none, false, 0, grouped));
    pool.put(dzs);
    }
    if (grouped && phase == 0) CK(run_wg_group(s, n, act, ws, grads, beta, part));
    if (beta == 0.f && part == 0) {
        if (pw_zero(s, grads[n.fc_w_idx], (size_t)1000 * 2048 * 4) != UDAPOSE_OK) return UDAPOSE_ERR_LAUNCH;
        if (pw_zero(s, grads[n.fc_b_idx], (size_t)1000 * 4) != UDAPOSE_OK) return UDAPOSE_ERR_LAUNCH;
    }
    return UDAPOSE_OK;
}

int net_input_grad(void* h, hipStream_t s, const void* const* params, void* ws_, float* dx) {
    Net& n = *(Net*)h;
    if ((n.f32 && !n.strict) || n.fwd_only) return UDAPOSE_ERR_UNSUPPORTED;
    DbgSyncScope dbg(n.policy.debug_sync);
    CK(stem_dgrad(s, (const elem_t*)((const char*)ws_ + n.stem.dy_off), (const float*)params[n.stem.w_idx], n.N, n.H, n.W, dx));
    return UDAPOSE_OK;
}

int net_apply_running(void* h, hipStream_t s, const void* act_, void* const* buffers, float momentum) {
// ... 140 lines not shown
```

### uda_poseestimation_amd/csrc/pointwise.h

```cpp
#pragma once
#include "common.h"

struct BnRunJob { size_t save_off; float* rm; float* rv; long long* nbt; int C, pad; };
struct ZeroJob { long long off; long long n16; };
#define UDAPOSE_SPLIT_SUM_CHUNK 1024u
struct SumJob { long long part_off; long long dst_off; unsigned n; unsigned stride; int ks; int dst_ws; float beta; int pad; };

int pw_zero(hipStream_t s, void* p, size_t bytes);
int pw_split_sum(hipStream_t s, const SumJob* d_jobs, const int* d_blk, int nblk, void* ws, void* grad_base, void* ws2 = nullptr, void* grad_base2 = nullptr);

int pw_nchw_f32_to_nhwc_bf16(hipStream_t s, const float* src, elem_t* dst, int N, int C, int HW, int Cp);
int pw_nchw_f32_to_nhwc_f32(hipStream_t s, const float* src, float* dst, int N, int C, int HW, int Cp);
int pw_nchw_f32_to_nhwc_split(hipStream_t s, const float* src, void* dst, int N, int C, int HW, int Cp, void* dst16 = nullptr);
int pw_nhwc_to_nchw_f32(hipStream_t s, const void* src, int src_is_f32, float* dst, int N, int C, int HW, int Cs, const float* lo, const float* hi);
int pw_cast_f32_bf16(hipStream_t s, const float* src, elem_t* dst, size_t n);
int pw_transpose_cast(hipStream_t s, const float* src, elem_t* dst, int A, int T, int B);
int pw_transpose_f32(hipStream_t s, const float* src, float* dst, int A, int T, int B);
int pw_f32_to_split(hipStream_t s, const float* src, void* dst, size_t n);
int pw_split_to_f32(hipStream_t s, const void* src, float* dst, size_t n);
int pw_transpose_split(hipStream_t s, const float* src, void* dst, int A, int T, int B);
int pw_pack_strided_split(hipStream_t s, const float* src, void* dst, int A, int KH, int KWp, int KW, int Bp, int B, long sa, long skh, long skw, long sb);
int pw_pack_multi(hipStream_t s, const void* jobs, const int* blk_job, const int* blk_sub, int nblocks);
int pw_pack_strided(hipStream_t s, const float* src, elem_t* dst, int A, int KH, int KWp, int KW, int Bp, int B, long sa, long skh, long skw, long sb);
int pw_pack_strided_f32(hipStream_t s, const float* src, float* dst, int A, int KH, int KWp, int KW, int Bp, int B, long sa, long skh, long skw, long sb);
int pw_unpack_strided(hipStream_t s, const float* src, float* dst, int A, int KH, int KWp, int KW, int Bp, int B, long sa, long skh, long skw, long sb, float beta);
int pw_bn_finalize(hipStream_t s, const float* slab, int rows, int C, double count, const float* gamma, const float* beta, float* rm, float* rv,
                   long long* nbt, float momentum, float eps, float* scale, float* shift, float* save_mean, float* save_invstd, const float* pre_bias);
int pw_bn_train_fused(hipStream_t s, const elem_t* y, const elem_t* res, elem_t* z, size_t npix, int C, const float* slab, int rows,
                      const float* gamma, const float* beta, float* rm, float* rv, long long* nbt, float momentum, float eps, float* save,
                      int relu, int enabled, unsigned char* mask);
int pw_bn_train_fused_split(hipStream_t s, const float* y, const void* res, void* z, size_t npix, int C, const float* slab, int rows,
                            const float* gamma, const float* beta, float* rm, float* rv, long long* nbt, float momentum, float eps, float* save,
                            int relu, int enabled, void* y16, void* z16, unsigned char* mask);
int pw_bn_running_update_multi(hipStream_t s, const BnRunJob* d_jobs, int njobs, int maxC, const void* act, float momentum);
int pw_bn_running_update(hipStream_t s, const float* save, int C, float* rm, float* rv, long long* nbt, float momentum);
int pw_zero_multi(hipStream_t s, const ZeroJob* d_jobs, int njobs, void* base);
int pw_axpy(hipStream_t s, float* y, const float* x, size_t n);
int pw_bn_eval_coeff(hipStream_t s, int C, const float* gamma, const float* beta, const float* rm, const float* rv, float eps, float* scale, float* shift);
int pw_bn_apply_xcd_ok(size_t n8, int C);
int pw_bn_apply(hipStream_t s, const elem_t* y, const elem_t* res, elem_t* z, size_t n, int C, const float* scale, const float* shift, int relu,
                unsigned char* mask, int xcd);
int pw_bn_apply_split(hipStream_t s, const float* y, const void* res, void* z, size_t n, int C, const float* scale, const float* shift, int relu,
                      void* y16, void* z16, unsigned char* mask, int xcd);
int pw_bn_apply_f32(hipStream_t s, const float* y, const float* res, float* z, size_t n, int C, const float* scale, const float* shift, int relu);
int pw_bn_bwd_rows(size_t npix);
int pw_bn_bwd_takes_chunked(size_t npix, int C, int chunked);
int pw_bn_bwd_pre_takes_chunked(size_t npix, int C, int rows, int chunked);
int pw_bn_bwd(hipStream_t s, const void* dz, int dz_is_f32, const elem_t* z, const elem_t* y, elem_t* dy, elem_t* gout, size_t npix, int C,
              const float* gamma, const float* mean, const float* invstd, int relu, float* slab, float* coef, float* dgamma, float* dbeta,
              float beta_acc, const float* beta, int chunked);
int pw_bn_bwd_pre(hipStream_t s, const void* g, int g_is_f32, const elem_t* y, elem_t* dy, size_t npix, int C, const float* gamma, const float* mean,
                  const float* invstd, const float* slab, int rows, float* coef, float* dgamma, float* dbeta, float beta_acc, int chunked,
                  int legacy);
int pw_maxpool3x3s2_fwd(hipStream_t s, const elem_t* x, elem_t* y, unsigned char* idx, int N, int H, int W, int C);
int pw_bn_relu_maxpool3x3s2(hipStream_t s, const elem_t* x, elem_t* y, unsigned char* idx, int N, int H, int W, int C, const float* scale,
                            const float* shift);
int pw_bn_bwd_pooled(hipStream_t s, const elem_t* pool_dy, const unsigned char* pool_idx, int H, int W, const elem_t* y, elem_t* dy, size_t npix, int C,
                     const float* gamma, const float* mean, const float* invstd, float* slab, float* coef, float* dgamma, float* dbeta, float beta_acc,
                     const float* beta);
int pw_maxpool3x3s2_fwd_f32(hipStream_t s, const float* x, float* y, unsigned char* idx, int N, int H, int W, int C);
int pw_maxpool3x3s2_fwd_split(hipStream_t s, const void* x, void* y, unsigned char* idx, int N, int H, int W, int C, void* y16);
int pw_maxpool2x2_ceil_split(hipStream_t s, const void* x, void* y, int N, int H, int W, int C);
int pw_maxpool3x3s2_bwd(hipStream_t s, const elem_t* dy, const unsigned char* idx, elem_t* dx, int N, int H, int W, int C);
int pw_maxpool2x2_ceil(hipStream_t s, const elem_t* x, elem_t* y, int N, int H, int W, int C);
int pw_maxpool2x2_ceil_f32(hipStream_t s, const float* x, float* y, int N, int H, int W, int C);
int pw_plane_sum(hipStream_t s, const float* x, float* out, int N, int C, int HW, float beta);
unsigned long long sp_sat_read_pointwise(int reset);
long long perturb_ws_bytes(int N, int C, int HW);
int perturb(hipStream_t s, const float* x, const float* g, const float* x0, int N, int C, int HW, int mode, const float* eps, const float* step,
            const float* lo, const float* hi, void* ws, float* out, float* gnorm);
```

### uda_poseestimation_amd/csrc/pointwise.hip

```cpp
#include <stdlib.h>
#include <type_traits>
#include "pointwise.h"
#include "storage8.h"

namespace {

constexpr int TPB = 256;
constexpr size_t GRID_CAP = 8192;

__device__ __forceinline__ void st8_f16(_Float16* p, const float (&v)[8]) {
    half8 o;
#pragma unroll
    for (int e = 0; e < 8; ++e) o[e] = (_Float16)v[e];
    *(half8*)p = o;
}
__device__ __forceinline__ half8 st8_split_shadow(sp32* p, _Float16* h16, const float (&v)[8]) {
    half8 h, l;
    sp_split8(v, h, l);
    char* c = (char*)p;
    *(half8*)c = h;
    *(half8*)(c + 16) = l;
    *(half8*)h16 = h;
    return h;
}
// ... 158 lines not shown
            a += ((double)a0 + (double)a1) + ((double)a2 + (double)a3);
            b += ((double)b0 + (double)b1) + ((double)b2 + (double)b3);
            a += ((double)a4 + (double)a5) + ((double)a6 + (double)a7);
            b += ((double)b4 + (double)b5) + ((double)b6 + (double)b7);
        }
        for (; r + 3 * FIN_RL < rows; r += 4 * FIN_RL) {
            const float* q = slab + (size_t)r * 2 * C + c;
            const size_t st = (size_t)FIN_RL * 2 * C;
            const float a0 = q[0], b0 = q[C], a1 = q[st], b1 = q[st + C];
            const float a2 = q[2 * st], b2 = q[2 * st + C], a3 = q[3 * st], b3 = q[3 * st + C];
            a += ((double)a0 + (double)a1) + ((double)a2 + (double)a3);
            b += ((double)b0 + (double)b1) + ((double)b2 + (double)b3);
        }
        for (; r < rows; r += FIN_RL) {
            a += (double)slab[(size_t)r * 2 * C + c];
            b += (double)slab[(size_t)r * 2 * C + C + c];
        }
    }
    red[rl][cl][0] = a; red[rl][cl][1] = b;
    __syncthreads();
    for (int st = FIN_RL / 2; st > 0; st >>= 1) {
        if (rl < st) { red[rl][cl][0] += red[rl + st][cl][0]; red[rl][cl][1] += red[rl + st][cl][1]; }
        __syncthreads();
    }
    s1 = red[0][cl][0]; s2 = red[0][cl][1];
}
__device__ __forceinline__ void bn_stats_finish(double s1, double s2, double count, double& mean, double& var) {
    mean = s1 / count;
    var = s2 / count - mean * mean;
    if (var < 0.0) var = 0.0;
}
__device__ __forceinline__ float bn_invstd(double var, float eps) { return (float)(1.0 / sqrt(var + (double)eps)); }
__device__ __forceinline__ double bn_unbiased_var(double var, double count) { return count > 1.0 ? var * count / (count - 1.0) : var; }
__device__ __forceinline__ void bn_running_update1(float* __restrict__ rm, float* __restrict__ rv, int c, float momentum, float mean, float unb) {
    rm[c] = (1.f - momentum) * rm[c] + momentum * mean;
    rv[c] = (1.f - momentum) * rv[c] + momentum * unb;
}
__device__ __forceinline__ float bn_affine(float v, float sc, float sh) { return v * sc + sh; }
__device__ __forceinline__ float bn_relu(float o, int relu) { return (relu && o < 0.f) ? 0.f : o; }
template <typename T>
__device__ __forceinline__ void bn_apply8(const float (&v)[8], const float (&sc)[8], const float (&sh)[8], const T* __restrict__ res, size_t off, int relu,
                                          float (&o)[8]) {
#pragma unroll
    for (int e = 0; e < 8; ++e) o[e] = bn_affine(v[e], sc[e], sh[e]);
    if (res) {
        float r[8];
        ld8<T>(res + off, r);
#pragma unroll
        for (int e = 0; e < 8; ++e) o[e] += r[e];
    }
#pragma unroll
    for (int e = 0; e < 8; ++e) o[e] = bn_relu(o[e], relu);
}
template <typename T, bool SH>
__device__ __forceinline__ void bn_store8(T* __restrict__ z, _Float16* __restrict__ z16, unsigned char* __restrict__ mask, size_t off, size_t mi,
                                          const float (&o)[8]) {
    if constexpr (SH) {
        const half8 h = st8_split_shadow(z + off, z16 + off, o);
        if (mask) mask[mi] = mask_of(h);
    } else {
        st8<T>(z + off, o);
        if constexpr (sizeof(T) == sizeof(elem_t)) {
            if (mask) mask[mi] = mask_of_stored(o);
        }
    }
}
__device__ __forceinline__ void pix_range(size_t sp, int P, size_t npix, size_t& p0, size_t& p1) {
    p0 = sp * P;
    p1 = p0 + P;
    if (p1 > npix) p1 = npix;
}
__device__ __forceinline__ void xcd_stream_range(size_t n8, int G, int xcd, size_t& i, size_t& iend, size_t& istep) {
    i = (size_t)blockIdx.x * TPB + threadIdx.x, iend = n8, istep = (size_t)gridDim.x * TPB;
    if (xcd) {
        const size_t rows = n8 / G, per = (rows + 7) / 8;
        const unsigned x = blockIdx.x & 7u, local = blockIdx.x >> 3, nb = gridDim.x >> 3;
        const unsigned RB = TPB / G;
        size_t rend = (size_t)(x + 1) * per;
        if (rend > rows) rend = rows;
        i = ((size_t)x * per + (size_t)local * RB + threadIdx.x / G) * G + threadIdx.x % G;
        iend = rend * G;
        istep = (size_t)nb * RB * G;
    }
}
__device__ __forceinline__ void xcd_chunk_of(int xcd, int& chunk, int& sp) {
    chunk = blockIdx.x, sp = blockIdx.y;
    if (xcd) {
        const uint32_t w = xcd_remap(blockIdx.x + gridDim.x * blockIdx.y, gridDim.x * gridDim.y);
        sp = (int)(w / gridDim.x);
        chunk = (int)(w - (uint32_t)sp * gridDim.x);
    }
}
__device__ __forceinline__ void slab_colsum64(const float* __restrict__ slab, int rows, int C, int chunk, double (*part)[128]) {
    const int q = threadIdx.x & 31, rg = threadIdx.x >> 5;
    const float* base = slab + (size_t)(q >> 4) * C + chunk * 64 + (q & 15) * 4;
    double a0 = 0.0, a1 = 0.0, a2 = 0.0, a3 = 0.0;
    int r = rg;
    for (; r + 56 < rows; r += 64) {
        const f32x4 u = *(const f32x4*)(base + (size_t)r * 2 * C), v = *(const f32x4*)(base + (size_t)(r + 8) * 2 * C);
        const f32x4 w = *(const f32x4*)(base + (size_t)(r + 16) * 2 * C), x = *(const f32x4*)(base + (size_t)(r + 24) * 2 * C);
        const f32x4 u2 = *(const f32x4*)(base + (size_t)(r + 32) * 2 * C), v2 = *(const f32x4*)(base + (size_t)(r + 40) * 2 * C);
        const f32x4 w2 = *(const f32x4*)(base + (size_t)(r + 48) * 2 * C), x2 = *(const f32x4*)(base + (size_t)(r + 56) * 2 * C);
        a0 += ((double)u[0] + (double)v[0]) + ((double)w[0] + (double)x[0]);
        a1 += ((double)u[1] + (double)v[1]) + ((double)w[1] + (double)x[1]);
        a2 += ((double)u[2] + (double)v[2]) + ((double)w[2] + (double)x[2]);
        a3 += ((double)u[3] + (double)v[3]) + ((double)w[3] + (double)x[3]);
// ... 17 lines not shown
    part[rg][q * 4 + 0] = a0; part[rg][q * 4 + 1] = a1; part[rg][q * 4 + 2] = a2; part[rg][q * 4 + 3] = a3;
}
__global__ __launch_bounds__(FIN_T) void bn_finalize_k(const float* __restrict__ slab, int rows, int C, double count, const float* __restrict__ gamma,
                              const float* __restrict__ beta, float* __restrict__ running_mean, float* __restrict__ running_var,
                              long long* __restrict__ nbt, float momentum, float eps, float* __restrict__ scale,
                              float* __restrict__ shift, float* __restrict__ save_mean, float* __restrict__ save_invstd,
                              const float* __restrict__ pre_bias = nullptr) {
    __shared__ double red[FIN_RL][FIN_C][2];
    const int c = blockIdx.x * FIN_C + (threadIdx.x % FIN_C);
    if (blockIdx.x == 0 && threadIdx.x == 0 && nbt) *nbt += 1;
    double s1, s2;
    slab_colsum(slab, rows, C, c, c < C, s1, s2, red);
    if ((threadIdx.x / FIN_C) != 0 || c >= C) return;
    double mean, var;
    bn_stats_finish(s1, s2, count, mean, var);
    if (pre_bias) mean += (double)pre_bias[c];
    const float invstd = bn_invstd(var, eps);
    const float sc = bn_scale(gamma[c], invstd);
    scale[c] = sc;
    shift[c] = bn_shift(beta[c], (float)mean, sc);
    save_mean[c] = (float)mean;
    save_invstd[c] = invstd;
    const double unb = bn_unbiased_var(var, count);
    save_invstd[C + c] = (float)unb;
    if (running_mean) bn_running_update1(running_mean, running_var, c, momentum, (float)mean, (float)unb);
}
__global__ void bn_running_update_k(const float* __restrict__ save, int C, float* __restrict__ rm, float* __restrict__ rv,
                                    long long* __restrict__ nbt, float momentum) {
    const int c = blockIdx.x * TPB + threadIdx.x;
    if (c == 0 && nbt) *nbt += 1;
    if (c >= C) return;
    bn_running_update1(rm, rv, c, momentum, save[c], save[2 * C + c]);
}
__global__ void axpy_k(float* __restrict__ y, const float* __restrict__ x, size_t n4) {
    for (size_t i = (size_t)blockIdx.x * TPB + threadIdx.x; i < n4; i += (size_t)gridDim.x * TPB) {
        f32x4 a = *(f32x4*)(y + i * 4);
        const f32x4 b = *(const f32x4*)(x + i * 4);
        a[0] += b[0]; a[1] += b[1]; a[2] += b[2]; a[3] += b[3];
        *(f32x4*)(y + i * 4) = a;
    }
}
__global__ void axpy_tail_k(float* __restrict__ y, const float* __restrict__ x, int n) {
    if ((int)threadIdx.x < n) y[threadIdx.x] += x[threadIdx.x];
}
__global__ void bn_eval_coeff_k(int C, const float* __restrict__ gamma, const float* __restrict__ beta, const float* __restrict__ rm,
                                const float* __restrict__ rv, float eps, float* __restrict__ scale, float* __restrict__ shift) {
    const int c = blockIdx.x * TPB + threadIdx.x;
    if (c >= C) return;
    const float sc = gamma[c] / sqrtf(rv[c] + eps);
    scale[c] = sc;
    shift[c] = beta[c] - rm[c] * sc;
}

template <typename T, typename TY = T, bool SH = false>
__global__ void bn_apply_k(const TY* __restrict__ y, const T* __restrict__ res, T* __restrict__ z, size_t n8, int C,
                           const float* __restrict__ scale, const float* __restrict__ shift, int relu, unsigned char* __restrict__ mask = nullptr,
                           int xcd = 0, _Float16* __restrict__ y16 = nullptr, _Float16* __restrict__ z16 = nullptr) {
    const int G = C >> 3;
    const int c0 = (int)(((size_t)blockIdx.x * TPB + threadIdx.x) % G) * 8;
    float sc[8], sh[8];
    ld8<float>(scale + c0, sc);
    ld8<float>(shift + c0, sh);
    size_t i, iend, istep;
    xcd_stream_range(n8, G, xcd, i, iend, istep);
    for (; i < iend; i += istep) {
        float v[8], o[8];
        ld8<TY>(y + i * 8, v);
        if constexpr (SH) st8_f16(y16 + i * 8, v);
        bn_apply8<T>(v, sc, sh, res, i * 8, relu, o);
        bn_store8<T, SH>(z, z16, mask, i * 8, i, o);
    }
}

__host__ __device__ inline int pool3x3s2_out(int H) { return (H + 2 - 3) / 2 + 1; }
struct PoolSrc { const elem_t* dy; const unsigned char* idx; int H, W; };
__device__ __forceinline__ void pool_grad8(const PoolSrc& ps, size_t pix, int C, int c0, float (&d)[8]) {
    const int w = (int)(pix % ps.W);
    const size_t r = pix / ps.W;
    const int h = (int)(r % ps.H);
    const size_t n = r / ps.H;
    const int Ho = pool3x3s2_out(ps.H), Wo = pool3x3s2_out(ps.W);
    float acc[8];
#pragma unroll
    for (int e = 0; e < 8; ++e) acc[e] = 0.f;
    for (int ho = h >> 1; ho <= ((h + 1) >> 1); ++ho)
        for (int wo = w >> 1; wo <= ((w + 1) >> 1); ++wo) {
            if (ho >= Ho || wo >= Wo) continue;
            const int kh = h - (ho * 2 - 1), kw = w - (wo * 2 - 1);
            if (kh < 0 || kh > 2 || kw < 0 || kw > 2) continue;
            const size_t o = ((n * Ho + ho) * Wo + wo) * C + c0;
            const unsigned long long pk = *(const unsigned long long*)(ps.idx + o);
            const elem8 dd = *(const elem8*)(ps.dy + o);
            const unsigned tap = (unsigned)(kh * 3 + kw);
#pragma unroll
            for (int e = 0; e < 8; ++e)
                if (((pk >> (8 * e)) & 0xFF) == tap) acc[e] += (float)dd[e];
        }
#pragma unroll
    for (int e = 0; e < 8; ++e) d[e] = (float)(elem_t)acc[e];
}

__device__ __forceinline__ void bn_bwd_mask_coef8(int relu, const float* __restrict__ gamma, const float* __restrict__ beta, int c0, const float (&mu)[8],
                                                  const float (&is)[8], float (&sc)[8], float (&sh)[8]) {
#pragma unroll
    for (int e = 0; e < 8; ++e) { sc[e] = 0.f; sh[e] = 0.f; }
    if (relu == 2) {
        float ga[8], be[8];
        ld8<float>(gamma + c0, ga);
        ld8<float>(beta + c0, be);
        bn_scale_shift8(ga, be, mu, is, sc, sh);
    }
}
__device__ __forceinline__ elem8 bn_bwd_ldz8(int relu, const elem_t* __restrict__ z, size_t off) {
    elem8 zz = {};
    if (relu == 1) zz = *(const elem8*)(z + off);
    return zz;
}
__device__ __forceinline__ float bn_bwd_g(int relu, float d, float y, float z, float sc, float sh) {
    float gv = d;
    if (relu == 1 && !(z > 0.f)) gv = 0.f;
    if (relu == 2 && !(y * sc + sh > 0.f)) gv = 0.f;
    return gv;
// ... 70 lines not shown
#pragma unroll
    for (int e = 0; e < 8; ++e) { red[threadIdx.x][e] = s1[e]; red[threadIdx.x][8 + e] = s2[e]; }
    __syncthreads();
    if (threadIdx.x < G) {
        float a[16];
#pragma unroll
        for (int e = 0; e < 16; ++e) a[e] = 0.f;
        for (int k = 0; k < pstep; ++k)
#pragma unroll
            for (int e = 0; e < 16; ++e) a[e] += red[threadIdx.x + k * G][e];
        float* sp = slab + (size_t)blockIdx.x * 2 * C;
#pragma unroll
        for (int e = 0; e < 8; ++e) { sp[c0 + e] = a[e]; sp[C + c0 + e] = a[8 + e]; }
    }
}
__global__ __launch_bounds__(FIN_T) void bn_bwd_finalize_k(const float* __restrict__ slab, int rows, int C, double count, const float* __restrict__ gamma,
                                  const float* __restrict__ invstd, float* __restrict__ dgamma, float* __restrict__ dbeta,
                                  float beta_acc, float* __restrict__ coef) {
    __shared__ double red[FIN_RL][FIN_C][2];
    const int c = blockIdx.x * FIN_C + (threadIdx.x % FIN_C);
    double s1, s2;
    slab_colsum(slab, rows, C, c, c < C, s1, s2, red);
    if ((threadIdx.x / FIN_C) != 0 || c >= C) return;
    if (dgamma) bwd_param_acc(dgamma, dbeta, c, beta_acc, s1, s2);
    bn_bwd_coef(gamma[c], invstd[c], s1, s2, count, coef[c], coef[C + c], coef[2 * C + c]);
}
template <typename DZ, bool POOL = false>
__global__ void bn_bwd_apply_k(const DZ* __restrict__ dz, const elem_t* __restrict__ z, const elem_t* __restrict__ y,
                               elem_t* __restrict__ dy, elem_t* __restrict__ gout, size_t n8, int C, const float* __restrict__ mean,
                               const float* __restrict__ invstd, const float* __restrict__ coef, int relu, const float* __restrict__ gamma,
                               const float* __restrict__ beta, PoolSrc ps = PoolSrc{nullptr, nullptr, 0, 0}) {
    const int G = C >> 3;
    for (size_t i = (size_t)blockIdx.x * TPB + threadIdx.x; i < n8; i += (size_t)gridDim.x * TPB) {
        const int c0 = (int)(i % G) * 8;
        float d[8];
        if constexpr (POOL) pool_grad8(ps, i / G, C, c0, d);
        else ld8<DZ>(dz + i * 8, d);
        const elem8 yy = *(const elem8*)(y + i * 8);
        const elem8 zz = bn_bwd_ldz8(relu, z, i * 8);
        float mu[8], is[8], ca[8], cb[8], cc[8], sc[8], sh[8];
        ld8<float>(mean + c0, mu);
        ld8<float>(invstd + c0, is);
        ld8<float>(coef + c0, ca);
        ld8<float>(coef + C + c0, cb);
        ld8<float>(coef + 2 * C + c0, cc);
        bn_bwd_mask_coef8(relu, gamma, beta, c0, mu, is, sc, sh);
        elem8 o, go;
        bn_bwd_g8_dy8(relu, d, yy, zz, sc, sh, mu, is, ca, cb, cc, o, go);
        *(elem8*)(dy + i * 8) = o;
        if (gout) *(elem8*)(gout + i * 8) = go;
    }
}

template <typename TY, typename TZ, bool SH = false>
__global__ __launch_bounds__(TPB) void bn_apply_chunk_k(const TY* __restrict__ y, const TZ* __restrict__ res, TZ* __restrict__ z,
                                                        size_t npix, int C, const float* __restrict__ slab, int rows, double count,
                                                        const float* __restrict__ gamma, const float* __restrict__ beta, float eps,
                                                        float momentum, float* __restrict__ running_mean, float* __restrict__ running_var,
                                                        long long* __restrict__ nbt, float* __restrict__ save, int relu, int P,
                                                        unsigned char* __restrict__ mask, int xcd, _Float16* __restrict__ y16 = nullptr,
                                                        _Float16* __restrict__ z16 = nullptr) {
    __shared__ double part[8][128];
    __shared__ float scs[64], shs[64];
    int chunk, sp;
    xcd_chunk_of(xcd, chunk, sp);
    slab_colsum64(slab, rows, C, chunk, part);
    __syncthreads();
    if (threadIdx.x < 64) {
        const int col = threadIdx.x, c = chunk * 64 + col;
        double s1 = 0.0, s2 = 0.0;
#pragma unroll
        for (int k = 0; k < 8; ++k) { s1 += part[k][col]; s2 += part[k][64 + col]; }
        double mean, var;
        bn_stats_finish(s1, s2, count, mean, var);
        const float invstd = bn_invstd(var, eps);
        const float sc = bn_scale(gamma[c], invstd);
        scs[col] = sc;
        shs[col] = bn_shift(beta[c], (float)mean, sc);
        if (sp == 0) {
            const double unb = bn_unbiased_var(var, count);
            save[c] = (float)mean;
            save[C + c] = invstd;
            save[2 * C + c] = (float)unb;
            if (running_mean) bn_running_update1(running_mean, running_var, c, momentum, (float)mean, (float)unb);
            if (c == 0 && nbt) *nbt += 1;
        }
    }
    __syncthreads();
    const int cg = threadIdx.x & 7, prow = threadIdx.x >> 3;
    const int c0 = chunk * 64 + cg * 8;
    float sc[8], sh[8];
#pragma unroll
    for (int e = 0; e < 8; ++e) { sc[e] = scs[cg * 8 + e]; sh[e] = shs[cg * 8 + e]; }
    size_t p0, p1;
    pix_range(sp, P, npix, p0, p1);
    for (size_t p = p0 + prow; p < p1; p += 32) {
        const size_t off = p * C + c0;
        float v[8], o[8];
        ld8<TY>(y + off, v);
        if constexpr (SH) st8_f16(y16 + off, v);
        bn_apply8<TZ>(v, sc, sh, res, off, relu, o);
        bn_store8<TZ, SH>(z, z16, mask, off, off >> 3, o);
    }
}

template <typename DZ>
__global__ __launch_bounds__(TPB) void bn_bwd_reduce_chunk_k(const DZ* __restrict__ dz, const elem_t* __restrict__ z, const elem_t* __restrict__ y,
                                                             size_t npix, int C, const float* __restrict__ mean,
                                                             const float* __restrict__ invstd, int relu, float* __restrict__ slab, int P,
                                                             const float* __restrict__ gamma, const float* __restrict__ beta) {
    __shared__ float red[32][8][17];
    const int chunk = blockIdx.x, sp = blockIdx.y, S = gridDim.y;
    const int cg = threadIdx.x & 7, prow = threadIdx.x >> 3;
    const int c0 = chunk * 64 + cg * 8;
    float mu[8], is[8], s1[8], s2[8], sc[8], sh[8];
    ld8<float>(mean + c0, mu);
    ld8<float>(invstd + c0, is);
#pragma unroll
    for (int e = 0; e < 8; ++e) { s1[e] = 0.f; s2[e] = 0.f; }
    bn_bwd_mask_coef8(relu, gamma, beta, c0, mu, is, sc, sh);
    size_t p0, p1;
    pix_range(sp, P, npix, p0, p1);
    for (size_t p = p0 + prow; p < p1; p += 32) {
        const size_t off = p * C + c0;
        float d[8];
        ld8<DZ>(dz + off, d);
        const elem8 yy = *(const elem8*)(y + off);
        bn_bwd_sums8(relu, d, yy, bn_bwd_ldz8(relu, z, off), sc, sh, mu, is, s1, s2);
    }
#pragma unroll
    for (int e = 0; e < 8; ++e) { red[prow][cg][e] = s1[e]; red[prow][cg][8 + e] = s2[e]; }
    __syncthreads();
    if (threadIdx.x < 128) {
        const int g = threadIdx.x >> 4, e = threadIdx.x & 15;
        float a = 0.f;
        for (int k = 0; k < 32; ++k) a += red[k][g][e];
        slab[(((size_t)chunk * S + sp) * 2 + (e >> 3)) * 64 + g * 8 + (e & 7)] = a;
    }
}
template <typename DZ>
__global__ __launch_bounds__(TPB) void bn_bwd_apply_chunk_k(const DZ* __restrict__ dz, const elem_t* __restrict__ z, const elem_t* __restrict__ y,
                                                            elem_t* __restrict__ dy, elem_t* __restrict__ gout, size_t npix, int C,
                                                            const float* __restrict__ mean, const float* __restrict__ invstd, int relu,
                                                            const float* __restrict__ gamma, const float* __restrict__ beta,
                                                            const float* __restrict__ slab, int P, float* __restrict__ dgamma,
                                                            float* __restrict__ dbeta, float beta_acc) {
    __shared__ double tot[2][64];
    const int chunk = blockIdx.x, sp = blockIdx.y, S = gridDim.y;
    if (threadIdx.x < 128) {
        const int st = threadIdx.x >> 6, col = threadIdx.x & 63;
        const float* q = slab + ((size_t)chunk * S * 2 + st) * 64 + col;
        double a = 0.0;
        int k = 0;
        for (; k + 4 <= S; k += 4)
            a += ((double)q[(size_t)k * 128] + (double)q[(size_t)(k + 1) * 128]) + ((double)q[(size_t)(k + 2) * 128] + (double)q[(size_t)(k + 3) * 128]);
        for (; k < S; ++k) a += (double)q[(size_t)k * 128];
        tot[st][col] = a;
    }
    __syncthreads();
    if (sp == 0 && threadIdx.x < 64 && dgamma) bwd_param_acc(dgamma, dbeta, chunk * 64 + threadIdx.x, beta_acc, tot[0][threadIdx.x], tot[1][threadIdx.x]);
    const int cg = threadIdx.x & 7, prow = threadIdx.x >> 3;
    const int c0 = chunk * 64 + cg * 8;
    float mu[8], is[8], ga[8], ca[8], cb[8], cc[8], sc[8], sh[8];
    ld8<float>(mean + c0, mu);
    ld8<float>(invstd + c0, is);
    ld8<float>(gamma + c0, ga);
    chunk_bwd_coef8(tot, cg, (double)npix, ga, is, ca, cb, cc);
    bn_bwd_mask_coef8(relu, gamma, beta, c0, mu, is, sc, sh);
    size_t p0, p1;
    pix_range(sp, P, npix, p0, p1);
    for (size_t p = p0 + prow; p < p1; p += 32) {
        const size_t off = p * C + c0;
        float d[8];
        ld8<DZ>(dz + off, d);
        const elem8 yy = *(const elem8*)(y + off);
        elem8 o, go;
        bn_bwd_g8_dy8(relu, d, yy, bn_bwd_ldz8(relu, z, off), sc, sh, mu, is, ca, cb, cc, o, go);
        *(elem8*)(dy + off) = o;
        if (gout) *(elem8*)(gout + off) = go;
    }
}

template <typename DZ>
__global__ __launch_bounds__(TPB) void bn_bwd_apply_pre_k(const DZ* __restrict__ g, const elem_t* __restrict__ y, elem_t* __restrict__ dy, size_t n8,
                                                          int C, const float* __restrict__ mean, const float* __restrict__ invstd,
                                                          const float* __restrict__ coef, int xcd = 0) {
    const int G = C >> 3;
    const int c0 = (int)(((size_t)blockIdx.x * TPB + threadIdx.x) % G) * 8;
    float mu[8], is[8], ca[8], cb[8], cc[8];
    ld8<float>(mean + c0, mu);
    ld8<float>(invstd + c0, is);
    ld8<float>(coef + c0, ca);
    ld8<float>(coef + C + c0, cb);
    ld8<float>(coef + 2 * C + c0, cc);
    size_t i, iend, istep;
    xcd_stream_range(n8, G, xcd, i, iend, istep);
    for (; i < iend; i += istep) {
        float d[8];
        ld8<DZ>(g + i * 8, d);
        const elem8 yy = *(const elem8*)(y + i * 8);
        *(elem8*)(dy + i * 8) = bn_bwd_dy8(d, yy, mu, is, ca, cb, cc);
    }
}

template <typename DZ>
__global__ __launch_bounds__(TPB) void bn_bwd_apply_pre_chunk_k(const DZ* __restrict__ g, const elem_t* __restrict__ y, elem_t* __restrict__ dy,
                                                                size_t npix, int C, const float* __restrict__ mean,
                                                                const float* __restrict__ invstd, const float* __restrict__ gamma,
                                                                const float* __restrict__ slab, int rows, int P, float* __restrict__ dgamma,
                                                                float* __restrict__ dbeta, float beta_acc, int xcd) {
    __shared__ double part[8][128];
    __shared__ double tot[2][64];
    int chunk, sp;
    xcd_chunk_of(xcd, chunk, sp);
    slab_colsum64(slab, rows, C, chunk, part);
    __syncthreads();
    if (threadIdx.x < 128) {
        double a = 0.0;
#pragma unroll
        for (int k = 0; k < 8; ++k) a += part[k][threadIdx.x];
        tot[threadIdx.x >> 6][threadIdx.x & 63] = a;
    }
    __syncthreads();
    if (sp == 0 && threadIdx.x < 64 && dgamma) bwd_param_acc(dgamma, dbeta, chunk * 64 + threadIdx.x, beta_acc, tot[0][threadIdx.x], tot[1][threadIdx.x]);
    const int cg = threadIdx.x & 7, prow = threadIdx.x >> 3;
    const int c0 = chunk * 64 + cg * 8;
    float mu[8], is[8], ga[8], ca[8], cb[8], cc[8];
    ld8<float>(mean + c0, mu);
    ld8<float>(invstd + c0, is);
    ld8<float>(gamma + c0, ga);
    chunk_bwd_coef8(tot, cg, (double)npix, ga, is, ca, cb, cc);
    size_t p0, p1;
    pix_range(sp, P, npix, p0, p1);
    for (size_t p = p0 + prow; p < p1; p += 32) {
        const size_t off = p * C + c0;
        float d[8];
        ld8<DZ>(g + off, d);
        const elem8 yy = *(const elem8*)(y + off);
        *(elem8*)(dy + off) = bn_bwd_dy8(d, yy, mu, is, ca, cb, cc);
    }
}

template <typename T, typename F>
__device__ __forceinline__ void pool3x3s2_scan(const T* __restrict__ x, int n, int ho, int wo, int g, int H, int W, int C, const F& tap, float (&best)[8],
                                               unsigned char (&bi)[8]) {
#pragma unroll
    for (int e = 0; e < 8; ++e) { best[e] = -INFINITY; bi[e] = 0; }
    bool first = true;
#pragma unroll
    for (int kh = 0; kh < 3; ++kh)
#pragma unroll
        for (int kw = 0; kw < 3; ++kw) {
            const int h = ho * 2 - 1 + kh, w = wo * 2 - 1 + kw;
            if ((unsigned)h < (unsigned)H && (unsigned)w < (unsigned)W) {
                float v[8];
                ld8<T>(x + (((size_t)n * H + h) * W + w) * C + g * 8, v);
#pragma unroll
                for (int e = 0; e < 8; ++e) {
                    const float f = tap(v[e], e);
                    if (first || f > best[e] || f != f) { best[e] = f; bi[e] = (unsigned char)(kh * 3 + kw); }
                }
                first = false;
            }
        }
}
__device__ __forceinline__ unsigned long long pack_taps(const unsigned char (&bi)[8]) {
    unsigned long long pk = 0;
#pragma unroll
    for (int e = 0; e < 8; ++e) pk |= (unsigned long long)bi[e] << (8 * e);
    return pk;
}
struct TapIdentity {
    __device__ __forceinline__ float operator()(float v, int) const { return v; }
};
struct TapBnRelu {
    float sc[8], sh[8];
    __device__ __forceinline__ float operator()(float v, int e) const { return (float)(elem_t)bn_relu(bn_affine(v, sc[e], sh[e]), 1); }
};
template <typename T, bool SH = false>
__global__ void maxpool3x3s2_fwd_k(const T* __restrict__ x, T* __restrict__ y, unsigned char* __restrict__ idx, int N, int H,
                                   int W, int C, int Ho, int Wo, _Float16* __restrict__ y16 = nullptr) {
    const int G = C >> 3;
    const size_t total = (size_t)N * Ho * Wo * G;
    for (size_t i = (size_t)blockIdx.x * TPB + threadIdx.x; i < total; i += (size_t)gridDim.x * TPB) {
        int n, ho, wo, g;
        nhwg_of(i, G, Ho, Wo, n, ho, wo, g);
        float best[8];
        unsigned char bi[8];
        pool3x3s2_scan<T>(x, n, ho, wo, g, H, W, C, TapIdentity{}, best, bi);
        if constexpr (SH) (void)st8_split_shadow(y + i * 8, y16 + i * 8, best);
        else st8<T>(y + i * 8, best);
        if (idx) *(unsigned long long*)(idx + i * 8) = pack_taps(bi);
// ... 160 lines not shown
    hipLaunchKernelGGL(pack_strided_k<sp32>, dim3(grid_for((size_t)A * KH * KWp * Bp, TPB, GRID_CAP)), dim3(TPB), 0, s, src, (sp32*)dst, A, KH, KWp, KW, Bp, B, sa, skh, skw, sb);
    return udapose_check_launch();
}
int pw_pack_multi(hipStream_t s, const void* jobs, const int* blk_job, const int* blk_sub, int nblocks) {
    if (nblocks <= 0) return UDAPOSE_OK;
    hipLaunchKernelGGL(pack_multi_k, dim3(nblocks), dim3(TPB), 0, s, (const PackJob*)jobs, blk_job, blk_sub);
    return udapose_check_launch();
}
int pw_pack_strided(hipStream_t s, const float* src, elem_t* dst, int A, int KH, int KWp, int KW, int Bp, int B, long sa, long skh, long skw, long sb) {
    hipLaunchKernelGGL(pack_strided_k<elem_t>, dim3(grid_for((size_t)A * KH * KWp * Bp, TPB, GRID_CAP)), dim3(TPB), 0, s, src, dst, A, KH, KWp, KW, Bp, B, sa, skh, skw, sb);
    return udapose_check_launch();
}
int pw_pack_strided_f32(hipStream_t s, const float* src, float* dst, int A, int KH, int KWp, int KW, int Bp, int B, long sa, long skh, long skw, long sb) {
    hipLaunchKernelGGL(pack_strided_k<float>, dim3(grid_for((size_t)A * KH * KWp * Bp, TPB, GRID_CAP)), dim3(TPB), 0, s, src, dst, A, KH, KWp, KW, Bp, B, sa, skh, skw, sb);
    return udapose_check_launch();
}
int pw_unpack_strided(hipStream_t s, const float* src, float* dst, int A, int KH, int KWp, int KW, int Bp, int B, long sa, long skh, long skw, long sb, float beta) {
    hipLaunchKernelGGL(unpack_strided_k, dim3(grid_for((size_t)A * KH * KW * B, TPB, GRID_CAP)), dim3(TPB), 0, s, src, dst, A, KH, KWp, KW, Bp, B, sa, skh, skw, sb, beta);
    return udapose_check_launch();
}
int pw_bn_finalize(hipStream_t s, const float* slab, int rows, int C, double count, const float* gamma, const float* beta, float* rm, float* rv,
                   long long* nbt, float momentum, float eps, float* scale, float* shift, float* save_mean, float* save_invstd, const float* pre_bias) {
    hipLaunchKernelGGL(bn_finalize_k, dim3((C + FIN_C - 1) / FIN_C), dim3(FIN_T), 0, s, slab, rows, C, count, gamma, beta, rm, rv, nbt, momentum, eps, scale, shift,
                       save_mean, save_invstd, pre_bias);
    return udapose_check_launch();
}
struct ChunkGeom { int chunks, S, P; };
static ChunkGeom chunk_geometry(size_t npix, int C, int target) {
    const int chunks = C / 64;
    int S = (target > 1 ? target : 1024) / chunks;
    if (S > 64) S = 64;
    if (S < 1) S = 1;
    int P = (int)((npix + S - 1) / S);
    P = (P + 31) & ~31;
    S = (int)((npix + P - 1) / P);
    return {chunks, S, P};
}
static bool fused_fwd_geometry(size_t npix, int C, int rows, int enabled, ChunkGeom& g, int& xcd) {
    xcd = (enabled >> 30) & 1;
    enabled &= ~(1 << 30);
    if (!enabled || C < 256 || C % 64 || npix > 8192 || npix < 1024 || rows > 128) return false;
    g = chunk_geometry(npix, C, enabled);
    return true;
}
int pw_bn_train_fused(hipStream_t s, const elem_t* y, const elem_t* res, elem_t* z, size_t npix, int C, const float* slab, int rows,
                      const float* gamma, const float* beta, float* rm, float* rv, long long* nbt, float momentum, float eps, float* save,
                      int relu, int enabled, unsigned char* mask) {
    ChunkGeom g;
    int xcd;
    if (!fused_fwd_geometry(npix, C, rows, enabled, g, xcd)) return 0;
    hipLaunchKernelGGL((bn_apply_chunk_k<elem_t, elem_t>), dim3(g.chunks, g.S), dim3(TPB), 0, s, y, res, z, npix, C, slab, rows, (double)npix, gamma, beta, eps,
                       momentum, rm, rv, nbt, save, relu, g.P, mask, xcd);
    return udapose_check_launch() == UDAPOSE_OK ? 1 : UDAPOSE_ERR_LAUNCH;
}
int pw_bn_train_fused_split(hipStream_t s, const float* y, const void* res, void* z, size_t npix, int C, const float* slab, int rows,
                            const float* gamma, const float* beta, float* rm, float* rv, long long* nbt, float momentum, float eps, float* save,
                            int relu, int enabled, void* y16, void* z16, unsigned char* mask) {
    ChunkGeom g;
    int xcd;
    if (!fused_fwd_geometry(npix, C, rows, enabled, g, xcd)) return 0;
    if (y16)
        hipLaunchKernelGGL((bn_apply_chunk_k<float, sp32, true>), dim3(g.chunks, g.S), dim3(TPB), 0, s, y, (const sp32*)res, (sp32*)z, npix, C, slab, rows,
                           (double)npix, gamma, beta, eps, momentum, rm, rv, nbt, save, relu, g.P, mask, xcd, (_Float16*)y16, (_Float16*)z16);
    else
        hipLaunchKernelGGL((bn_apply_chunk_k<float, sp32>), dim3(g.chunks, g.S), dim3(TPB), 0, s, y, (const sp32*)res, (sp32*)z, npix, C, slab, rows, (double)npix,
                           gamma, beta, eps, momentum, rm, rv, nbt, save, relu, g.P, (unsigned char*)nullptr, xcd);
    return udapose_check_launch() == UDAPOSE_OK ? 1 : UDAPOSE_ERR_LAUNCH;
}
__global__ void bn_running_update_multi_k(const BnRunJob* __restrict__ jobs, const char* __restrict__ act, float momentum) {
    const BnRunJob j = jobs[blockIdx.x];
    const int c = blockIdx.y * TPB + threadIdx.x;
    if (c == 0 && j.nbt) *j.nbt += 1;
    if (c >= j.C) return;
    const float* save = (const float*)(act + j.save_off);
    bn_running_update1(j.rm, j.rv, c, momentum, save[c], save[2 * j.C + c]);
}
int pw_bn_running_update_multi(hipStream_t s, const BnRunJob* d_jobs, int njobs, int maxC, const void* act, float momentum) {
    hipLaunchKernelGGL(bn_running_update_multi_k, dim3(njobs, grid_for(maxC, TPB, GRID_NO_CAP)), dim3(TPB), 0, s, d_jobs, (const char*)act, momentum);
    return udapose_check_launch();
}
int pw_bn_running_update(hipStream_t s, const float* save, int C, float* rm, float* rv, long long* nbt, float momentum) {
    hipLaunchKernelGGL(bn_running_update_k, dim3(grid_for(C, TPB, GRID_NO_CAP)), dim3(TPB), 0, s, save, C, rm, rv, nbt, momentum);
    return udapose_check_launch();
}
__global__ void zero_multi_k(const ZeroJob* __restrict__ jobs, char* __restrict__ base) {
    const ZeroJob j = jobs[blockIdx.x];
    u32x4* p = (u32x4*)(base + j.off);
    const u32x4 z = {0u, 0u, 0u, 0u};
    for (long long i = (long long)blockIdx.y * TPB + threadIdx.x; i < j.n16; i += (long long)gridDim.y * TPB) p[i] = z;
}
int pw_zero_multi(hipStream_t s, const ZeroJob* d_jobs, int njobs, void* base) {
    if (njobs <= 0) return UDAPOSE_OK;
    hipLaunchKernelGGL(zero_multi_k, dim3(njobs, 32), dim3(TPB), 0, s, d_jobs, (char*)base);
    return udapose_check_launch();
}
__global__ void zero_k(unsigned int* __restrict__ p, size_t head, size_t n16, size_t tail) {
    const size_t t = (size_t)blockIdx.x * TPB + threadIdx.x, step = (size_t)gridDim.x * TPB;
    if (t < head) p[t] = 0u;
    u32x4* b = (u32x4*)(p + head);
    const u32x4 z = {0u, 0u, 0u, 0u};
    for (size_t i = t; i < n16; i += step) b[i] = z;
    if (t < tail) p[head + n16 * 4 + t] = 0u;
}
int pw_zero(hipStream_t s, void* p, size_t bytes) {
    if (!bytes) return UDAPOSE_OK;
    if (!p || (bytes & 3) || ((uintptr_t)p & 3)) return UDAPOSE_ERR_ARG;
// ... 19 lines not shown
        for (unsigned e = c0 + threadIdx.x * 4u; e < c1; e += TPB * 4u) {
            f32x4 a = *(const f32x4*)(part + e);
#pragma unroll 8
            for (int z = 1; z < j.ks; ++z) a += *(const f32x4*)(part + (size_t)z * j.stride + e);
            if (j.beta != 0.f) a = *(const f32x4*)(dst + e) + a;
            *(f32x4*)(dst + e) = a;
        }
    } else {
        for (unsigned e = c0 + threadIdx.x; e < c1; e += TPB) {
            float a = part[e];
            for (int z = 1; z < j.ks; ++z) a += part[(size_t)z * j.stride + e];
            if (j.beta != 0.f) a = dst[e] + a;
            dst[e] = a;
        }
    }
}
int pw_split_sum(hipStream_t s, const SumJob* d_jobs, const int* d_blk, int nblk, void* ws, void* grad_base, void* ws2, void* grad_base2) {
    if (nblk <= 0) return UDAPOSE_OK;
    hipLaunchKernelGGL(split_sum_k, dim3(ws2 ? 2 * nblk : nblk), dim3(TPB), 0, s, d_jobs, d_blk, nblk, (char*)ws, (char*)grad_base, (char*)ws2, (char*)grad_base2);
    return udapose_check_launch();
}
int pw_axpy(hipStream_t s, float* y, const float* x, size_t n) {
    const size_t n4 = n / 4;
    if (n4) hipLaunchKernelGGL(axpy_k, dim3(grid_for(n4, TPB, GRID_CAP)), dim3(TPB), 0, s, y, x, n4);
    if (n % 4) hipLaunchKernelGGL(axpy_tail_k, dim3(1), dim3(64), 0, s, y + n4 * 4, x + n4 * 4, (int)(n % 4));
    return udapose_check_launch();
}
int pw_bn_eval_coeff(hipStream_t s, int C, const float* gamma, const float* beta, const float* rm, const float* rv, float eps, float* scale, float* shift) {
    hipLaunchKernelGGL(bn_eval_coeff_k, dim3(grid_for(C, TPB, GRID_NO_CAP)), dim3(TPB), 0, s, C, gamma, beta, rm, rv, eps, scale, shift);
    return udapose_check_launch();
}
static int bn_apply_grid(size_t n8, int C) {
    const int G = C / 8;
    int g = grid_for(n8, TPB, GRID_CAP);
    if (g > 2048) g = 2048;
    if ((TPB % G) != 0) {
        g = (g / G) * G;
        if (g < G) g = G;
    }
    return g;
}
int pw_bn_apply_xcd_ok(size_t n8, int C) {
    const int grid = bn_apply_grid(n8, C), G = C / 8;
    return (TPB % G) == 0 && (grid % 8) == 0 && (n8 / G) >= (size_t)8 * (TPB / G);
}
int pw_bn_apply(hipStream_t s, const elem_t* y, const elem_t* res, elem_t* z, size_t n, int C, const float* scale, const float* shift, int relu,
                unsigned char* mask, int xcd) {
    if (C % 8 || n % 8) return UDAPOSE_ERR_ARG;
    const int grid = bn_apply_grid(n / 8, C);
    const int ok = xcd && pw_bn_apply_xcd_ok(n / 8, C);
    hipLaunchKernelGGL(bn_apply_k<elem_t>, dim3(grid), dim3(TPB), 0, s, y, res, z, n / 8, C, scale, shift, relu, mask, ok);
    return udapose_check_launch();
}
int pw_bn_apply_split(hipStream_t s, const float* y, const void* res, void* z, size_t n, int C, const float* scale, const float* shift, int relu,
                      void* y16, void* z16, unsigned char* mask, int xcd) {
    if (C % 8 || n % 8) return UDAPOSE_ERR_ARG;
    if (y16) {
        const int grid = bn_apply_grid(n / 8, C);
        const int ok = xcd && pw_bn_apply_xcd_ok(n / 8, C);
        hipLaunchKernelGGL((bn_apply_k<sp32, float, true>), dim3(grid), dim3(TPB), 0, s, y, (const sp32*)res, (sp32*)z, n / 8, C, scale, shift, relu, mask,
                           ok, (_Float16*)y16, (_Float16*)z16);
        return udapose_check_launch();
    }
    hipLaunchKernelGGL((bn_apply_k<sp32, float>), dim3(bn_apply_grid(n / 8, C)), dim3(TPB), 0, s, y, (const sp32*)res, (sp32*)z, n / 8, C, scale, shift, relu,
                       (unsigned char*)nullptr);
    return udapose_check_launch();
}
int pw_bn_apply_f32(hipStream_t s, const float* y, const float* res, float* z, size_t n, int C, const float* scale, const float* shift, int relu) {
    if (C % 8 || n % 8) return UDAPOSE_ERR_ARG;
    hipLaunchKernelGGL(bn_apply_k<float>, dim3(bn_apply_grid(n / 8, C)), dim3(TPB), 0, s, y, res, z, n / 8, C, scale, shift, relu, (unsigned char*)nullptr);
    return udapose_check_launch();
}
int pw_bn_bwd_rows(size_t npix) {
    return (int)(npix < 1024 ? (npix < 1 ? 1 : npix) : 1024);
}
int pw_bn_bwd_takes_chunked(size_t npix, int C, int chunked) { return chunked && C >= 256 && npix <= 32768 && npix >= 1024; }
int pw_bn_bwd_pre_takes_chunked(size_t npix, int C, int rows, int chunked) {
    return pw_bn_bwd_takes_chunked(npix, C, chunked & ~(3 << 29)) && rows <= 128;
}
struct ReduceGeom { int rows, ppb; };
static ReduceGeom stream_reduce_geometry(size_t npix, int G) {
    const int pstep = TPB / G;
    size_t want = (npix + pstep - 1) / pstep;
    if (want > 1024) want = 1024;
    const int rows = (int)(want < 1 ? 1 : want);
    return {rows, (int)((npix + rows - 1) / rows)};
}
static void launch_bwd_finalize(hipStream_t s, const float* slab, int rows, int C, size_t npix, const float* gamma, const float* invstd, float* dgamma,
                                float* dbeta, float beta_acc, float* coef) {
    hipLaunchKernelGGL(bn_bwd_finalize_k, dim3((C + FIN_C - 1) / FIN_C), dim3(FIN_T), 0, s, slab, rows, C, (double)npix, gamma, invstd, dgamma, dbeta, beta_acc, coef);
}
template <typename F>
static void with_grad_type(const void* g, int is_f32, F&& f) {
    if (is_f32) f((const float*)g);
    else f((const elem_t*)g);
}
template <typename P> using pointee_t = std::remove_const_t<std::remove_pointer_t<P>>;
int pw_bn_bwd(hipStream_t s, const void* dz, int dz_is_f32, const elem_t* z, const elem_t* y, elem_t* dy, elem_t* gout, size_t npix, int C,
              const float* gamma, const float* mean, const float* invstd, int relu, float* slab, float* coef, float* dgamma, float* dbeta,
              float beta_acc, const float* beta, int chunked) {
    if (relu == 2 && !beta) return UDAPOSE_ERR_ARG;
    if (relu == 1 && !z) return UDAPOSE_ERR_ARG;
    const int G = C / 8;
    if (C % 8 || G > 256 || (G & (G - 1))) return UDAPOSE_ERR_UNSUPPORTED;
    if (pw_bn_bwd_takes_chunked(npix, C, chunked)) {
        const ChunkGeom cg = chunk_geometry(npix, C, 1024);
        const dim3 grid(cg.chunks, cg.S);
        with_grad_type(dz, dz_is_f32, [&](auto d) {
            using DZ = pointee_t<decltype(d)>;
            hipLaunchKernelGGL(bn_bwd_reduce_chunk_k<DZ>, grid, dim3(TPB), 0, s, d, z, y, npix, C, mean, invstd, relu, slab, cg.P, gamma, beta);
            hipLaunchKernelGGL(bn_bwd_apply_chunk_k<DZ>, grid, dim3(TPB), 0, s, d, z, y, dy, gout, npix, C, mean, invstd, relu, gamma, beta, slab, cg.P, dgamma,
                               dbeta, beta_acc);
        });
        return udapose_check_launch();
    }
    const ReduceGeom rg = stream_reduce_geometry(npix, G);
    with_grad_type(dz, dz_is_f32, [&](auto d) {
        using DZ = pointee_t<decltype(d)>;
        hipLaunchKernelGGL(bn_bwd_reduce_k<DZ>, dim3(rg.rows), dim3(TPB), 0, s, d, z, y, npix, C, mean, invstd, relu, slab, rg.ppb, gamma, beta);
        launch_bwd_finalize(s, slab, rg.rows, C, npix, gamma, invstd, dgamma, dbeta, beta_acc, coef);
        hipLaunchKernelGGL(bn_bwd_apply_k<DZ>, dim3(grid_for(npix * G, TPB, GRID_CAP)), dim3(TPB), 0, s, d, z, y, dy, gout, npix * G, C, mean, invstd, coef, relu, gamma, beta);
    });
    return udapose_check_launch();
}
int pw_bn_bwd_pre(hipStream_t s, const void* g, int g_is_f32, const elem_t* y, elem_t* dy, size_t npix, int C, const float* gamma, const float* mean,
                  const float* invstd, const float* slab, int rows, float* coef, float* dgamma, float* dbeta, float beta_acc, int chunked,
                  int legacy) {
    const int G = C / 8;
    if (C % 8 || G > 256 || (G & (G - 1)) || rows < 1) return UDAPOSE_ERR_UNSUPPORTED;
    const int xcd = (chunked >> 30) & 1, xcd_stream = (chunked >> 29) & 1;
    chunked &= ~(3 << 29);
    if (pw_bn_bwd_pre_takes_chunked(npix, C, rows, chunked)) {
        const ChunkGeom cg = chunk_geometry(npix, C, chunked);
        with_grad_type(g, g_is_f32, [&](auto d) {
            hipLaunchKernelGGL(bn_bwd_apply_pre_chunk_k<pointee_t<decltype(d)>>, dim3(cg.chunks, cg.S), dim3(TPB), 0, s, d, y, dy, npix, C, mean, invstd, gamma, slab,
                               rows, cg.P, dgamma, dbeta, beta_acc, xcd);
        });
        return udapose_check_launch();
    }
    launch_bwd_finalize(s, slab, rows, C, npix, gamma, invstd, dgamma, dbeta, beta_acc, coef);
    if (legacy) {
        with_grad_type(g, g_is_f32, [&](auto d) {
            hipLaunchKernelGGL(bn_bwd_apply_k<pointee_t<decltype(d)>>, dim3(grid_for(npix * G, TPB, GRID_CAP)), dim3(TPB), 0, s, d, (const elem_t*)nullptr, y, dy, (elem_t*)nullptr,
                               npix * G, C, mean, invstd, coef, 0, gamma, (const float*)nullptr);
        });
        return udapose_check_launch();
    }
    const int grid = bn_apply_grid(npix * G, C);
    const int ok = xcd_stream && pw_bn_apply_xcd_ok(npix * G, C);
    with_grad_type(g, g_is_f32, [&](auto d) {
        hipLaunchKernelGGL(bn_bwd_apply_pre_k<pointee_t<decltype(d)>>, dim3(grid), dim3(TPB), 0, s, d, y, dy, npix * G, C, mean, invstd, coef, ok);
    });
    return udapose_check_launch();
}
int pw_maxpool3x3s2_fwd(hipStream_t s, const elem_t* x, elem_t* y, unsigned char* idx, int N, int H, int W, int C) {
    const int Ho = pool3x3s2_out(H), Wo = pool3x3s2_out(W);
    hipLaunchKernelGGL(maxpool3x3s2_fwd_k<elem_t>, dim3(grid_for((size_t)N * Ho * Wo * (C / 8), TPB, GRID_CAP)), dim3(TPB), 0, s, x, y, idx, N, H, W, C, Ho, Wo);
    return udapose_check_launch();
}
int pw_bn_relu_maxpool3x3s2(hipStream_t s, const elem_t* x, elem_t* y, unsigned char* idx, int N, int H, int W, int C, const float* scale,
                            const float* shift) {
    if (C % 8 || !idx) return UDAPOSE_ERR_ARG;
    const int Ho = pool3x3s2_out(H), Wo = pool3x3s2_out(W);
    hipLaunchKernelGGL(bn_relu_maxpool3x3s2_k, dim3(grid_for((size_t)N * Ho * Wo * (C / 8), TPB, GRID_CAP)), dim3(TPB), 0, s, x, y, idx, N, H, W, C, Ho, Wo, scale, shift);
    return udapose_check_launch();
}
int pw_bn_bwd_pooled(hipStream_t s, const elem_t* pool_dy, const unsigned char* pool_idx, int H, int W, const elem_t* y, elem_t* dy, size_t npix, int C,
                     const float* gamma, const float* mean, const float* invstd, float* slab, float* coef, float* dgamma, float* dbeta, float beta_acc,
                     const float* beta) {
    const int G = C / 8;
    if (C % 8 || G > 256 || (G & (G - 1)) || !beta || npix % ((size_t)H * W)) return UDAPOSE_ERR_UNSUPPORTED;
    const PoolSrc ps{pool_dy, pool_idx, H, W};
    const ReduceGeom rg = stream_reduce_geometry(npix, G);
    hipLaunchKernelGGL((bn_bwd_reduce_k<elem_t, true>), dim3(rg.rows), dim3(TPB), 0, s, (const elem_t*)nullptr, (const elem_t*)nullptr, y, npix, C, mean, invstd,
                       2, slab, rg.ppb, gamma, beta, ps);
    launch_bwd_finalize(s, slab, rg.rows, C, npix, gamma, invstd, dgamma, dbeta, beta_acc, coef);
    hipLaunchKernelGGL((bn_bwd_apply_k<elem_t, true>), dim3(grid_for(npix * G, TPB, GRID_CAP)), dim3(TPB), 0, s, (const elem_t*)nullptr, (const elem_t*)nullptr, y, dy,
                       (elem_t*)nullptr, npix * G, C, mean, invstd, coef, 2, gamma, beta, ps);
    return udapose_check_launch();
}
int pw_maxpool3x3s2_fwd_f32(hipStream_t s, const float* x, float* y, unsigned char* idx, int N, int H, int W, int C) {
    const int Ho = pool3x3s2_out(H), Wo = pool3x3s2_out(W);
    hipLaunchKernelGGL(maxpool3x3s2_fwd_k<float>, dim3(grid_for((size_t)N * Ho * Wo * (C / 8), TPB, GRID_CAP)), dim3(TPB), 0, s, x, y, idx, N, H, W, C, Ho, Wo);
    return udapose_check_launch();
}
int pw_maxpool3x3s2_fwd_split(hipStream_t s, const void* x, void* y, unsigned char* idx, int N, int H, int W, int C, void* y16) {
    const int Ho = pool3x3s2_out(H), Wo = pool3x3s2_out(W);
    if (y16) {
        hipLaunchKernelGGL((maxpool3x3s2_fwd_k<sp32, true>), dim3(grid_for((size_t)N * Ho * Wo * (C / 8), TPB, GRID_CAP)), dim3(TPB), 0, s, (const sp32*)x, (sp32*)y, idx, N, H, W,
                           C, Ho, Wo, (_Float16*)y16);
        return udapose_check_launch();
    }
    hipLaunchKernelGGL(maxpool3x3s2_fwd_k<sp32>, dim3(grid_for((size_t)N * Ho * Wo * (C / 8), TPB, GRID_CAP)), dim3(TPB), 0, s, (const sp32*)x, (sp32*)y, idx, N, H, W, C, Ho, Wo);
    return udapose_check_launch();
}
int pw_maxpool2x2_ceil_split(hipStream_t s, const void* x, void* y, int N, int H, int W, int C) {
    if (C % 8) return UDAPOSE_ERR_ARG;
    const int Ho = (H + 1) / 2, Wo = (W + 1) / 2;
    hipLaunchKernelGGL(maxpool2x2_ceil_k<sp32>, dim3(grid_for((size_t)N * Ho * Wo * (C / 8), TPB, GRID_CAP)), dim3(TPB), 0, s, (const sp32*)x, (sp32*)y, N, H, W, C, Ho, Wo);
    return udapose_check_launch();
}
int pw_maxpool3x3s2_bwd(hipStream_t s, const elem_t* dy, const unsigned char* idx, elem_t* dx, int N, int H, int W, int C) {
    hipLaunchKernelGGL(maxpool3x3s2_bwd_k, dim3(grid_for((size_t)N * H * W * (C / 8), TPB, GRID_CAP)), dim3(TPB), 0, s, dy, idx, dx, N, H, W, C);
    return udapose_check_launch();
}
int pw_maxpool2x2_ceil(hipStream_t s, const elem_t* x, elem_t* y, int N, int H, int W, int C) {
// ... 17 lines not shown
```

### uda_poseestimation_amd/ops.py

```python
import ctypes as C

import torch

from . import _hip
from ._hip import ConvDesc, check, lib, lib_for, ptr, require_cuda, stream

EPI_RELU, EPI_OUT_F32, EPI_F32, EPI_SPLIT = 1, 2, 4, 8
SPLIT = torch.int32


def conv_desc(N, Hi, Wi, Ci, Co, K, stride=1, pad=0, transposed=False, reflect=False, upsample=False, policy=None):
    d = ConvDesc(N, Hi, Wi, Ci, Co, K, K, stride, pad, int(transposed), int(reflect), int(upsample))
    if policy is not None:
        d.policy = C.pointer(policy)
    return d


def with_policy(d, policy):
    return conv_desc(d.N, d.Hi, d.Wi, d.Ci, d.Co, d.KH, d.stride, d.pad, d.transposed, d.reflect, d.upsample, policy)


def conv_out_hw(d):
    ho, wo = C.c_int(), C.c_int()
    lib().udapose_conv_out_hw(C.byref(d), C.byref(ho), C.byref(wo))
# ... 166 lines not shown
    dbeta = torch.empty(C_, dtype=torch.float32, device=dev)
    dy = torch.empty_like(y)
    g = torch.empty_like(y) if want_g else None
    check(lib_for(y).udapose_bn_bwd(stream(), ptr(dz), int(dz.dtype == torch.float32), ptr(z), ptr(y), ptr(dy), ptr(g), npix, C_, ptr(gamma), ptr(mean),
                               ptr(invstd), int(relu),
                               ptr(slab), ptr(coef), ptr(dgamma), ptr(dbeta), 0.0, ptr(beta)), "bn_bwd")
    return dy, dgamma, dbeta, g


def bn_bwd_pre(g, y, gamma, mean, invstd, slab):
    C_ = y.shape[-1]
    npix = y.numel() // C_
    dev = y.device
    coef = torch.empty(3, C_, dtype=torch.float32, device=dev)
    dgamma = torch.empty(C_, dtype=torch.float32, device=dev)
    dbeta = torch.empty(C_, dtype=torch.float32, device=dev)
    dy = torch.empty_like(y)
    check(lib_for(y).udapose_bn_bwd_pre(stream(), ptr(g), int(g.dtype == torch.float32), ptr(y), ptr(dy), npix, C_, ptr(gamma), ptr(mean), ptr(invstd),
                                   ptr(slab), slab.shape[0], ptr(coef), ptr(dgamma), ptr(dbeta), 0.0), "bn_bwd_pre")
    return dy, dgamma, dbeta


BN_KINDS = {"16bit": 0, "f32": 1, "split": 2, "strict": 3}


def _form(code, what):
    if code < 0:
        check(code, what)
    return code


def bn_train_fwd_ex(kind, y, z, slab, gamma, beta, scale, shift, save, res=None, pre_bias=None, running_mean=None, running_var=None, nbt=None,
                    momentum=0.1, eps=1e-5, relu=True, fwd_chunked=1, xcd_rows=1, mask=None, y16=None, z16=None, build=None):
    npix, C_ = y.shape
    L = lib(build) if build else lib_for(y, z)
    return _form(L.udapose_bn_train_fwd_ex(stream(), BN_KINDS[kind], ptr(y), ptr(res), ptr(z), npix, C_, ptr(slab), slab.shape[0], ptr(gamma),
                                           ptr(beta), ptr(pre_bias), ptr(running_mean), ptr(running_var), ptr(nbt), momentum, eps, ptr(scale),
                                           ptr(shift), ptr(save), int(relu), int(fwd_chunked), int(xcd_rows), ptr(mask), ptr(y16), ptr(z16)),
                 "bn_train_fwd_ex")


def bn_bwd_ex(dz, z, y, dy, gamma, mean, invstd, slab, coef, dgamma, dbeta, relu=1, gout=None, beta=None, beta_acc=0.0, chunked=1):
    npix, C_ = y.shape
    return _form(lib_for(y).udapose_bn_bwd_ex(stream(), ptr(dz), int(dz.dtype == torch.float32), ptr(z), ptr(y), ptr(dy), ptr(gout), npix, C_,
                                              ptr(gamma), ptr(mean), ptr(invstd), int(relu), ptr(slab), ptr(coef), ptr(dgamma), ptr(dbeta),
                                              float(beta_acc), ptr(beta), int(chunked)), "bn_bwd_ex")


def bn_bwd_pre_ex(g, y, dy, gamma, mean, invstd, slab, coef, dgamma, dbeta, beta_acc=0.0, chunked=1, legacy=0):
    npix, C_ = y.shape
    return _form(lib_for(y).udapose_bn_bwd_pre_ex(stream(), ptr(g), int(g.dtype == torch.float32), ptr(y), ptr(dy), npix, C_, ptr(gamma), ptr(mean),
                                                  ptr(invstd), ptr(slab), slab.shape[0], ptr(coef), ptr(dgamma), ptr(dbeta), float(beta_acc),
                                                  int(chunked), int(legacy)), "bn_bwd_pre_ex")


def bn_relu_maxpool3x3s2(x, y, idx, scale, shift):
    N, H, W, C_ = x.shape
    check(lib_for(x).udapose_bn_relu_maxpool3x3s2(stream(), ptr(x), ptr(y), ptr(idx), N, H, W, C_, ptr(scale), ptr(shift)), "bn_relu_maxpool3x3s2")


def bn_bwd_pooled(pool_dy, pool_idx, y, dy, gamma, mean, invstd, beta, slab, coef, dgamma, dbeta, beta_acc=0.0):
    N, H, W, C_ = y.shape
    check(lib_for(y).udapose_bn_bwd_pooled(stream(), ptr(pool_dy), ptr(pool_idx), H, W, ptr(y), ptr(dy), N * H * W, C_, ptr(gamma), ptr(mean),
                                           ptr(invstd), ptr(slab), ptr(coef), ptr(dgamma), ptr(dbeta), float(beta_acc), ptr(beta)), "bn_bwd_pooled")


def maxpool3x3s2_fwd_ex(kind, x, y, idx, y16=None, build=None):
    N, H, W, C_ = x.shape
    L = lib(build) if build else lib_for(x)
    check(L.udapose_maxpool3x3s2_fwd_ex(stream(), BN_KINDS[kind], ptr(x), ptr(y), ptr(idx), N, H, W, C_, ptr(y16)), "maxpool3x3s2_fwd_ex")


def maxpool3x3s2_fwd(x):
    N, H, W, C_ = x.shape
    Ho, Wo = (H - 1) // 2 + 1, (W - 1) // 2 + 1
    y = torch.empty(N, Ho, Wo, C_, dtype=x.dtype, device=x.device)
    idx = torch.empty(N, Ho, Wo, C_, dtype=torch.uint8, device=x.device)
    check(lib_for(x).udapose_maxpool3x3s2_fwd(stream(), ptr(x), ptr(y), ptr(idx), N, H, W, C_), "maxpool_fwd")
    return y, idx


def maxpool3x3s2_bwd(dy, idx, H, W):
    N, _, _, C_ = dy.shape
    dx = torch.empty(N, H, W, C_, dtype=dy.dtype, device=dy.device)
    check(lib_for(dy).udapose_maxpool3x3s2_bwd(stream(), ptr(dy), ptr(idx), ptr(dx), N, H, W, C_), "maxpool_bwd")
    return dx


def maxpool2x2_ceil(x):
    N, H, W, C_ = x.shape
    y = torch.empty(N, (H + 1) // 2, (W + 1) // 2, C_, dtype=x.dtype, device=x.device)
    fn = lib().udapose_maxpool2x2_ceil_split if x.dtype == SPLIT else (
        lib().udapose_maxpool2x2_ceil_f32 if x.dtype == torch.float32 else lib_for(x).udapose_maxpool2x2_ceil)
    check(fn(stream(), ptr(x), ptr(y), N, H, W, C_), "maxpool2x2")
    return y


def adain(content, style, alpha=1.0, eps=1e-5, want_stats=False, stats_only=False):
    N, H, W, C_ = content.shape
    assert content.dtype == style.dtype and content.dtype in (torch.bfloat16, torch.float16, torch.float32, SPLIT)
    assert style.shape[0] == N and style.shape[3] == C_
    out = None if stats_only else torch.empty_like(content)
    st = torch.empty(N, C_, 4, dtype=torch.float32, device=content.device) if (want_stats or stats_only) else None
    f32 = content.dtype == torch.float32
    if content.dtype == SPLIT:
        dev_alpha = torch.is_tensor(alpha)
# ... 107 lines not shown
```

Before: 2044 images/sec.

## Fold downsample-branch BN into bottleneck conv3 BN apply in forward and backward

In bottleneck blocks that have a downsample branch, the downsample BN normalize is no longer applied as its own pass. Its normalized output is computed inline inside the conv3 BN apply (residual add plus ReLU) kernel, and in backward the downsample BN statistics are gathered inside the conv3 BN bwd-pre kernel. This removes separate elementwise passes and their full-activation reads and writes for four blocks, in exchange for more template variants, extra slab workspace and coupling of the two BN geometries.

```diff
diff --git a/include/udapose.h b/include/udapose.h
--- a/include/udapose.h
+++ b/include/udapose.h
@@ -45,6 +45,8 @@
     void* timeline;
     int wgrad_order;
     int wgrad_fastgeo_strided;
+    int ds_fold;
+    int ds_bwd_fold;
 } udapose_policy;
 void udapose_policy_default(udapose_policy* p);
 
@@ -111,6 +113,10 @@
 int udapose_bn_bwd_pre_ex(void* stream, const void* g, int g_is_f32, const void* y, void* dy, size_t npix, int C, const float* gamma,
                           const float* save_mean, const float* save_invstd, const float* slab, int rows, float* coef, float* dgamma,
                           float* dbeta, float beta_acc, int chunked, int legacy);
+int udapose_bn_bwd_pre_ds(void* stream, const void* g, int g_is_f32, const void* y, void* dy, size_t npix, int C, const float* gamma,
+                          const float* mean, const float* invstd, const float* slab, int rows, float* coef, float* dgamma, float* dbeta,
+                          float beta_acc, int chunked, const void* yd, const float* mean_d, const float* invstd_d, float* slab_d, int slab_d_rows,
+                          int* rows_d);
 int udapose_bn_relu_maxpool3x3s2(void* stream, const void* x, void* y, unsigned char* idx, int N, int H, int W, int C, const float* scale,
                                  const float* shift);
 int udapose_bn_bwd_pooled(void* stream, const void* pool_dy, const unsigned char* pool_idx, int H, int W, const void* y, void* dy, size_t npix,
@@ -137,6 +143,7 @@
 size_t udapose_net_act_bytes(udapose_net_t net);
 size_t udapose_net_ws_bytes(udapose_net_t net);
 void udapose_net_out_shape(udapose_net_t net, int shape[4]);
+int udapose_net_block_tensor(udapose_net_t net, int block, int what, size_t* off, size_t* bytes);
 int udapose_net_set_policy(udapose_net_t net, const udapose_policy* p);
 int udapose_net_get_policy(udapose_net_t net, udapose_policy* p);
 int udapose_net_bind(udapose_net_t net, const void* const* h_params, void* const* h_buffers, void* wpack);
diff --git a/uda_poseestimation_amd/_hip.py b/uda_poseestimation_amd/_hip.py
--- a/uda_poseestimation_amd/_hip.py
+++ b/uda_poseestimation_amd/_hip.py
@@ -16,7 +16,7 @@
                                        "wgrad_fastgeo", "wgrad_group", "wgrad_stages", "wgrad_group_stem", "bn_bwd_fused", "bn_fwd_chunked",
                                        "bn_bwd_chunked", "bn_bwd_pre_legacy", "igemm_wg_min", "wgrad_row3", "bn3_mask", "stem_fused", "debug_sync", "igemm_big_min", "patch_conv",
                                        "eval_fold", "bn_xcd_rows", "wgrad_det", "igemm_ns3_k")] + [("timeline", C.c_void_p), ("wgrad_order", C.c_int),
-                                                                                                   ("wgrad_fastgeo_strided", C.c_int)]
+                                                                                                   ("wgrad_fastgeo_strided", C.c_int), ("ds_fold", C.c_int), ("ds_bwd_fold", C.c_int)]
 
 
 def policy(**overrides):
@@ -77,6 +77,7 @@
     "udapose_bn_bwd_ex": (ci, [vp, vp, ci, vp, vp, vp, vp, sz, ci, vp, vp, vp, ci, vp, vp, vp, vp, cf, vp, ci]),
     "udapose_bn_bwd_pre_ex": (ci, [vp, vp, ci, vp, vp, sz, ci, vp, vp, vp, vp, ci, vp, vp, vp, cf, ci, ci]),
     "udapose_bn_relu_maxpool3x3s2": (ci, [vp, vp, vp, vp, ci, ci, ci, ci, vp, vp]),
+    "udapose_bn_bwd_pre_ds": (ci, [vp, vp, ci, vp, vp, sz, ci, vp, vp, vp, vp, ci, vp, vp, vp, cf, ci, vp, vp, vp, vp, ci, vp]),
     "udapose_bn_bwd_pooled": (ci, [vp, vp, vp, ci, ci, vp, vp, sz, ci, vp, vp, vp, vp, vp, vp, vp, cf, vp]),
     "udapose_bn_running_update": (ci, [vp, vp, ci, vp, vp, vp, cf]),
     "udapose_bn_running_update_multi": (ci, [vp, vp, ci, ci, vp, cf]),
@@ -94,6 +95,7 @@
     "udapose_net_act_bytes": (sz, [vp]),
     "udapose_net_ws_bytes": (sz, [vp]),
     "udapose_net_out_shape": (None, [vp, vp]),
+    "udapose_net_block_tensor": (ci, [vp, ci, ci, vp, vp]),
     "udapose_net_pack_weights": (ci, [vp, vp, vp, vp, ci]),
     "udapose_net_forward": (ci, [vp, vp, vp, vp, vp, vp, vp, vp, vp, ci, cf]),
     "udapose_net_apply_running": (ci, [vp, vp, vp, vp, cf]),
diff --git a/uda_poseestimation_amd/csrc/capi.hip b/uda_poseestimation_amd/csrc/capi.hip
--- a/uda_poseestimation_amd/csrc/capi.hip
+++ b/uda_poseestimation_amd/csrc/capi.hip
@@ -146,6 +146,20 @@
     if (pw_bn_bwd_pre_takes_chunked(npix, C, rows, chunked)) return 1 | (((chunked >> 30) & 1) ? 2 : 0);
     return (!legacy && ((chunked >> 29) & 1) && pw_bn_apply_xcd_ok(npix * (C / 8), C)) ? 2 : 0;
 }
+int udapose_bn_bwd_pre_ds(void* stream, const void* g, int g_is_f32, const void* y, void* dy, size_t npix, int C, const float* gamma,
+                          const float* mean, const float* invstd, const float* slab, int rows, float* coef, float* dgamma, float* dbeta,
+                          float beta_acc, int chunked, const void* yd, const float* mean_d, const float* invstd_d, float* slab_d, int slab_d_rows,
+                          int* rows_d) {
+    if (!g || !y || !dy || !gamma || !mean || !invstd || !slab || !coef || !yd || !mean_d || !invstd_d || !slab_d || !rows_d || npix < 1 || C < 8 ||
+        C % 8 || rows < 1)
+        return UDAPOSE_ERR_ARG;
+    if (pw_bn_bwd_pre_ds_rows(npix, C, rows, chunked) > slab_d_rows) return UDAPOSE_ERR_ARG;
+    const int rc = pw_bn_bwd_pre_ds(S(stream), g, g_is_f32, CB16(y), B16(dy), npix, C, gamma, mean, invstd, slab, rows, coef, dgamma, dbeta, beta_acc,
+                                    chunked, CB16(yd), mean_d, invstd_d, slab_d, rows_d);
+    if (rc != UDAPOSE_OK) return rc;
+    if (pw_bn_bwd_pre_takes_chunked(npix, C, rows, chunked)) return 1 | (((chunked >> 30) & 1) ? 2 : 0);
+    return (((chunked >> 29) & 1) && pw_bn_apply_xcd_ok(npix * (C / 8), C)) ? 2 : 0;
+}
 int udapose_bn_relu_maxpool3x3s2(void* stream, const void* x, void* y, unsigned char* idx, int N, int H, int W, int C, const float* scale,
                                  const float* shift) {
     if (!x || !y || !scale || !shift || N < 1 || H < 1 || W < 1 || C < 8) return UDAPOSE_ERR_ARG;
@@ -237,6 +251,10 @@
 size_t udapose_net_act_bytes(udapose_net_t n) { return net_act_bytes(n); }
 size_t udapose_net_ws_bytes(udapose_net_t n) { return net_ws_bytes(n); }
 void udapose_net_out_shape(udapose_net_t n, int shape[4]) { net_out_shape(n, shape); }
+int udapose_net_block_tensor(udapose_net_t n, int block, int what, size_t* off, size_t* bytes) {
+    if (!n || !off || !bytes) return UDAPOSE_ERR_ARG;
+    return net_block_tensor(n, block, what, off, bytes);
+}
 int udapose_net_pack_weights(udapose_net_t n, void* stream, const void* const* params, void* wpack, int with_bwd) {
     return net_pack_weights(n, S(stream), params, wpack, with_bwd);
 }
diff --git a/uda_poseestimation_amd/csrc/conv_plan.h b/uda_poseestimation_amd/csrc/conv_plan.h
--- a/uda_poseestimation_amd/csrc/conv_plan.h
+++ b/uda_poseestimation_amd/csrc/conv_plan.h
@@ -12,7 +12,7 @@
         bn_bwd_fused = 1; bn_fwd_chunked = 1; bn_bwd_chunked = 1; bn_bwd_pre_legacy = 0;
         igemm_wg_min = 512; wgrad_row3 = 1; bn3_mask = 1; stem_fused = 1; debug_sync = 0;
         igemm_big_min = 0; patch_conv = 2; eval_fold = 1; bn_xcd_rows = 1; wgrad_det = 1; igemm_ns3_k = 0;
-        timeline = nullptr; wgrad_order = 1; wgrad_fastgeo_strided = 1;
+        timeline = nullptr; wgrad_order = 1; wgrad_fastgeo_strided = 1; ds_fold = 1; ds_bwd_fold = 1;
     }
 };
 inline const Policy& default_policy() { static const Policy p; return p; }
diff --git a/uda_poseestimation_amd/csrc/net.h b/uda_poseestimation_amd/csrc/net.h
--- a/uda_poseestimation_amd/csrc/net.h
+++ b/uda_poseestimation_amd/csrc/net.h
@@ -12,6 +12,7 @@
 size_t net_act_bytes(void* h);
 size_t net_ws_bytes(void* h);
 void net_out_shape(void* h, int* shp);
+int net_block_tensor(void* h, int block, int what, size_t* off, size_t* bytes);
 int net_bind(void* h, const void* const* params, void* const* buffers, void* wpack_);
 int net_pack_weights(void* h, hipStream_t s, const void* const* params, void* wpack_, int with_bwd);
 int net_forward(void* h, hipStream_t s, const float* x_nchw, const void* const* params, void* const* buffers, const void* wpack_, void* act_, void* ws_,
diff --git a/uda_poseestimation_amd/csrc/net.hip b/uda_poseestimation_amd/csrc/net.hip
--- a/uda_poseestimation_amd/csrc/net.hip
+++ b/uda_poseestimation_amd/csrc/net.hip
@@ -317,11 +317,22 @@
     return g.transposed ? pw_transpose_f32(s, w, (float*)(wpack + c.wf_off), g.Ci, g.KH * g.KW, g.Co) : UDAPOSE_OK;
 }
 
+int ds_fold_form(const Net& n, const Block& b, int training) {
+    if (!b.has_ds || !training || n.f32 || !n.policy.ds_fold) return 0;
+    const int chunked = n.policy.bn_fwd_chunked | (n.policy.bn_xcd_rows ? (1 << 30) : 0);
+    const int t3 = pw_bn_train_fused_takes(b.b3.npix, b.b3.C, conv_stat_rows(b.c3.g), chunked);
+    const int td = pw_bn_train_fused_takes(b.bd.npix, b.bd.C, conv_stat_rows(b.cd.g), chunked);
+    return t3 != td ? 0 : (t3 ? 2 : 1);
+}
+
 int conv_bn_fwd(hipStream_t s, const Net& n, const ConvL& c, const BnL& b, const void* const* params, void* const* buffers, const char* wpack,
-                char* act, char* ws, int training, float momentum, const elem_t* res, int relu, bool upd, bool no_apply = false) {
+                char* act, char* ws, int training, float momentum, const elem_t* res, int relu, bool upd, bool no_apply = false, int ds_form = 0,
+                const Block* ds_of = nullptr) {
     ConvEpilogue e;
-    float* slab = (float*)(ws + n.ws_slab);
-    float* scale = (float*)(ws + n.ws_coef);
+    const size_t y_off = (ds_of && n.fwd_only) ? n.sc.off[SC_DS] : c.y_off;
+    const size_t fy_off = (ds_of && n.fwd_only) ? y_off : c.fy_off;
+    float* slab = (float*)(ws + ((ds_form == 2 && !ds_of) ? n.ws_slabf : n.ws_slab));
+    float* scale = (float*)(ws + n.ws_coef) + ((ds_form && !ds_of) ? 4096 : 0);
     float* shift = scale + 2048;
     float* save = (float*)(act + b.save_off);
     e.stats = training ? slab : nullptr;
@@ -349,8 +360,18 @@
         e.out_f32 = 0;
         return conv_fprop(s, c.g, (const elem_t*)(act + c.fin_off), (const elem_t*)wptr, act + b.fz_off, e);
     }
-    CK(conv_fprop(s, c.g, (const elem_t*)(act + c.fin_off), (const elem_t*)wptr, act + c.fy_off, e));
-    if (training && !n.f32 && !no_apply && !pre_bias) {
+    CK(conv_fprop(s, c.g, (const elem_t*)(act + c.fin_off), (const elem_t*)wptr, act + fy_off, e));
+    if (ds_form == 2) {
+        if (!ds_of) return UDAPOSE_OK;
+        const ConvL& cd = ds_of->cd;
+        const BnL& bd = ds_of->bd;
+        return pw_bn_train_fused_ds(s, (const elem_t*)(act + y_off), (const elem_t*)(act + cd.y_off), (elem_t*)(act + b.z_off), b.npix, b.C, slab,
+                                    conv_stat_rows(c.g), gamma, beta, rm, rv, nbt, save, (const float*)(ws + n.ws_slabf), conv_stat_rows(cd.g),
+                                    (const float*)params[bd.g_idx], (const float*)params[bd.b_idx], upd ? (float*)buffers[bd.rm_idx] : nullptr,
+                                    upd ? (float*)buffers[bd.rv_idx] : nullptr, upd ? (long long*)buffers[bd.nbt_idx] : nullptr,
+                                    (float*)(act + bd.save_off), momentum, 1e-5f, relu, chunked, mask);
+    }
+    if (training && !n.f32 && !no_apply && !pre_bias && !ds_form) {
         const int took = pw_bn_train_fused(s, (const elem_t*)(act + c.y_off), res, (elem_t*)(act + b.z_off), b.npix, b.C, slab, conv_stat_rows(c.g), gamma,
                                            beta, rm, rv, nbt, momentum, 1e-5f, save, relu, chunked, mask);
         if (took < 0) return took;
@@ -368,6 +389,9 @@
     else
         CK(pw_bn_eval_coeff(s, b.C, gamma, beta, (const float*)buffers[b.rm_idx], (const float*)buffers[b.rv_idx], 1e-5f, scale, shift));
     if (no_apply) return UDAPOSE_OK;
+    if (ds_form == 1 && ds_of)
+        return pw_bn_apply_ds(s, (const elem_t*)(act + y_off), (const elem_t*)(act + ds_of->cd.y_off), (elem_t*)(act + b.z_off), b.npix * b.C, b.C, scale,
+                              shift, scale + 4096, shift + 4096, relu, mask, n.policy.bn_xcd_rows >= 2);
     if (n.f32 == 2)
         return pw_bn_apply_split(s, (const float*)(act + c.fy_off), res, act + b.fz_off, b.npix * b.C, b.C, scale, shift, relu, y16, z16, sh ? mask : nullptr,
                                  n.policy.bn_xcd_rows >= 2);
@@ -399,6 +423,20 @@
     if ((n.f32 && !n.strict) || n.fwd_only || !n.policy.wgrad_group || !n.policy.wgrad_det) { n.ws_wgpart_bytes = 0; return n.ws_bytes; }
     n.ws_wgpart_bytes = wg_partial_bytes(n);
     return n.ws_bytes + n.ws_wgpart_bytes;
+}
+int net_block_tensor(void* h, int block, int what, size_t* off, size_t* bytes) {
+    const Net& n = *(const Net*)h;
+    if (block < 0 || block >= (int)n.blocks.size() || what < 0 || what > 5) return UDAPOSE_ERR_ARG;
+    const Block& b = n.blocks[block];
+    if (what >= 4 && !b.has_ds) return UDAPOSE_ERR_ARG;
+    const BnL* bn[4] = {&b.b1, &b.b2, &b.b3, &b.bd};
+    if (what == 0 || what == 5) {
+        const BnL& z = what == 0 ? b.b3 : b.bd;
+        *off = z.z_off; *bytes = z.npix * z.C * n.es;
+    } else {
+        *off = bn[what - 1]->save_off; *bytes = (size_t)3 * bn[what - 1]->C * 4;
+    }
+    return UDAPOSE_OK;
 }
 void net_out_shape(void* h, int* shp) { Net& n = *(Net*)h; shp[0] = n.N; shp[1] = n.K; shp[2] = n.Hout; shp[3] = n.Wout; }
 
@@ -507,11 +545,12 @@
         CK(conv_bn_fwd(s, n, b.c1, b.b1, params, buffers, wpack, act, ws, training, momentum, nullptr, 1, upd));
         CK(conv_bn_fwd(s, n, b.c2, b.b2, params, buffers, wpack, act, ws, training, momentum, nullptr, 1, upd));
         const elem_t* res = (const elem_t*)(act + b.fin_off);
+        const int ds_form = ds_fold_form(n, b, training);
         if (b.has_ds) {
-            CK(conv_bn_fwd(s, n, b.cd, b.bd, params, buffers, wpack, act, ws, training, momentum, nullptr, 0, upd));
-            res = (const elem_t*)(act + b.fzd_off);
-        }
-        CK(conv_bn_fwd(s, n, b.c3, b.b3, params, buffers, wpack, act, ws, training, momentum, res, 1, upd));
+            CK(conv_bn_fwd(s, n, b.cd, b.bd, params, buffers, wpack, act, ws, training, momentum, nullptr, 0, upd, ds_form != 0, ds_form));
+            res = ds_form ? nullptr : (const elem_t*)(act + b.fzd_off);
+        }
+        CK(conv_bn_fwd(s, n, b.c3, b.b3, params, buffers, wpack, act, ws, training, momentum, res, 1, upd, false, ds_form, ds_form ? &b : nullptr));
     }
     for (int i = 0; i < 3; ++i) CK(conv_bn_fwd(s, n, n.up[i], n.up_bn[i], params, buffers, wpack, act, ws, training, momentum, nullptr, 1, upd));
     ConvEpilogue e;
@@ -525,17 +564,26 @@
 }
 
 namespace {
+int bn_bwd_pre_word(const Net& n) {
+    return n.policy.bn_bwd_chunked | (n.policy.bn_xcd_rows ? (1 << 30) : 0) | (n.policy.bn_xcd_rows >= 2 ? (1 << 29) : 0);
+}
 int conv_bn_bwd(hipStream_t s, const Net& n, const ConvL& c, const BnL& b, const void* const* params, const char* wpack, char* act, char* ws,
                 void* const* grads, float beta, Pool& pool, const void* dz, int dz_f32, elem_t* gout, int relu, const elem_t* dx_res,
-                elem_t** dx_out, bool need_dx, int dx_f32, bool grouped_wgrad, const DgradBnStat* pre = nullptr, DgradBnStat* next = nullptr) {
+                elem_t** dx_out, bool need_dx, int dx_f32, bool grouped_wgrad, const DgradBnStat* pre = nullptr, DgradBnStat* next = nullptr,
+                const Block* ds_of = nullptr, DgradBnStat* ds_pre = nullptr) {
     float* slab = (float*)(ws + n.ws_slab);
     float* coef = (float*)(ws + n.ws_coef) + 4096;
     const float* save = (const float*)(act + b.save_off);
     elem_t* dy = (elem_t*)(ws + c.dy_off);
-    if (pre)
+    if (pre && ds_of) {
+        const float* save_d = (const float*)(act + ds_of->bd.save_off);
+        ds_pre->slab = slab;
+        CK(pw_bn_bwd_pre_ds(s, dz, dz_f32, (const elem_t*)(act + c.y_off), dy, b.npix, b.C, (const float*)params[b.g_idx], save, save + b.C, pre->slab,
+                            pre->rows, coef, (float*)grads[b.g_idx], (float*)grads[b.b_idx], beta, bn_bwd_pre_word(n), (const elem_t*)(act + ds_of->cd.y_off),
+                            save_d, save_d + ds_of->bd.C, slab, &ds_pre->rows));
+    } else if (pre)
         CK(pw_bn_bwd_pre(s, dz, dz_f32, (const elem_t*)(act + c.y_off), dy, b.npix, b.C, (const float*)params[b.g_idx], save, save + b.C, pre->slab,
-                         pre->rows, coef, (float*)grads[b.g_idx], (float*)grads[b.b_idx], beta, n.policy.bn_bwd_chunked | (n.policy.bn_xcd_rows ? (1 << 30) : 0) | (n.policy.bn_xcd_rows >= 2 ? (1 << 29) : 0),
-                         n.policy.bn_bwd_pre_legacy));
+                         pre->rows, coef, (float*)grads[b.g_idx], (float*)grads[b.b_idx], beta, bn_bwd_pre_word(n), n.policy.bn_bwd_pre_legacy));
     else
         CK(pw_bn_bwd(s, dz, dz_f32, (const elem_t*)(act + b.z_off), (const elem_t*)(act + c.y_off), dy, gout, b.npix, b.C, (const float*)params[b.g_idx],
                      save, save + b.C, relu, slab, coef, (float*)grads[b.g_idx], (float*)grads[b.b_idx], beta, (const float*)params[b.b_idx],
@@ -996,8 +1044,11 @@
         Block& b = n.blocks[bi];
         elem_t *dz2 = nullptr, *dz1 = nullptr, *dxd = nullptr, *dxin = nullptr;
         if (fused) nxt = bn_stat_of(n, b.c2, b.b2, params, act, ws, 2);
+        DgradBnStat ds_pre;
+        const bool ds_fold = have && b.has_ds && n.policy.ds_bwd_fold && !n.policy.bn_bwd_pre_legacy &&
+                             (size_t)pw_bn_bwd_pre_ds_rows(b.b3.npix, b.b3.C, cur.rows, bn_bwd_pre_word(n)) * 2 * b.b3.C * 4 <= n.ws_slabf - n.ws_slab;
         CK(conv_bn_bwd(s, n, b.c3, b.b3, params, wpack, act, ws, grads, beta, pool, dz, 0, dz, 1, nullptr, &dz2, true, 0, grouped, have ? &cur : nullptr,
-                       fused ? &nxt : nullptr));
+                       fused ? &nxt : nullptr, ds_fold ? &b : nullptr, &ds_pre));
         if (fused) { cur = nxt; nxt = bn_stat_of(n, b.c1, b.b1, params, act, ws, 2); }
         CK(conv_bn_bwd(s, n, b.c2, b.b2, params, wpack, act, ws, grads, beta, pool, dz2, 0, nullptr, 2, nullptr, &dz1, true, 0, grouped,
                        have ? &cur : nullptr, fused ? &nxt : nullptr));
@@ -1005,7 +1056,8 @@
         pool.put(dz2);
         const elem_t* skip = dz;
         if (b.has_ds) {
-            CK(conv_bn_bwd(s, n, b.cd, b.bd, params, wpack, act, ws, grads, beta, pool, dz, 0, nullptr, 0, nullptr, &dxd, true, 0, grouped));
+            CK(conv_bn_bwd(s, n, b.cd, b.bd, params, wpack, act, ws, grads, beta, pool, dz, 0, nullptr, 0, nullptr, &dxd, true, 0, grouped,
+                           ds_fold ? &ds_pre : nullptr));
             skip = dxd;
         }
         const bool chain = fused && bi > 0;
diff --git a/uda_poseestimation_amd/csrc/pointwise.h b/uda_poseestimation_amd/csrc/pointwise.h
--- a/uda_poseestimation_amd/csrc/pointwise.h
+++ b/uda_poseestimation_amd/csrc/pointwise.h
@@ -32,6 +32,13 @@
 int pw_bn_train_fused_split(hipStream_t s, const float* y, const void* res, void* z, size_t npix, int C, const float* slab, int rows,
                             const float* gamma, const float* beta, float* rm, float* rv, long long* nbt, float momentum, float eps, float* save,
                             int relu, int enabled, void* y16, void* z16, unsigned char* mask);
+int pw_bn_train_fused_takes(size_t npix, int C, int rows, int enabled);
+int pw_bn_train_fused_ds(hipStream_t s, const elem_t* y, const elem_t* yd, elem_t* z, size_t npix, int C, const float* slab, int rows,
+                         const float* gamma, const float* beta, float* rm, float* rv, long long* nbt, float* save, const float* slab_d, int rows_d,
+                         const float* gamma_d, const float* beta_d, float* rm_d, float* rv_d, long long* nbt_d, float* save_d, float momentum, float eps,
+                         int relu, int enabled, unsigned char* mask);
+int pw_bn_apply_ds(hipStream_t s, const elem_t* y, const elem_t* yd, elem_t* z, size_t n, int C, const float* scale, const float* shift,
+                   const float* scale_d, const float* shift_d, int relu, unsigned char* mask, int xcd);
 int pw_bn_running_update_multi(hipStream_t s, const BnRunJob* d_jobs, int njobs, int maxC, const void* act, float momentum);
 int pw_bn_running_update(hipStream_t s, const float* save, int C, float* rm, float* rv, long long* nbt, float momentum);
 int pw_zero_multi(hipStream_t s, const ZeroJob* d_jobs, int njobs, void* base);
@@ -52,6 +59,10 @@
 int pw_bn_bwd_pre(hipStream_t s, const void* g, int g_is_f32, const elem_t* y, elem_t* dy, size_t npix, int C, const float* gamma, const float* mean,
                   const float* invstd, const float* slab, int rows, float* coef, float* dgamma, float* dbeta, float beta_acc, int chunked,
                   int legacy);
+int pw_bn_bwd_pre_ds_rows(size_t npix, int C, int rows, int chunked);
+int pw_bn_bwd_pre_ds(hipStream_t s, const void* g, int g_is_f32, const elem_t* y, elem_t* dy, size_t npix, int C, const float* gamma, const float* mean,
+                     const float* invstd, const float* slab, int rows, float* coef, float* dgamma, float* dbeta, float beta_acc, int chunked,
+                     const elem_t* yd, const float* mean_d, const float* invstd_d, float* slab_d, int* rows_d);
 int pw_maxpool3x3s2_fwd(hipStream_t s, const elem_t* x, elem_t* y, unsigned char* idx, int N, int H, int W, int C);
 int pw_bn_relu_maxpool3x3s2(hipStream_t s, const elem_t* x, elem_t* y, unsigned char* idx, int N, int H, int W, int C, const float* scale,
                             const float* shift);
diff --git a/uda_poseestimation_amd/csrc/pointwise.hip b/uda_poseestimation_amd/csrc/pointwise.hip
--- a/uda_poseestimation_amd/csrc/pointwise.hip
+++ b/uda_poseestimation_amd/csrc/pointwise.hip
@@ -234,6 +234,18 @@
 #pragma unroll
     for (int e = 0; e < 8; ++e) o[e] = bn_relu(o[e], relu);
 }
+template <typename T>
+__device__ __forceinline__ void bn_apply8_ds(const float (&v)[8], const float (&sc)[8], const float (&sh)[8], const T* __restrict__ yd, size_t off,
+                                             const float (&scd)[8], const float (&shd)[8], int relu, float (&o)[8]) {
+    float vd[8];
+    ld8<T>(yd + off, vd);
+#pragma unroll
+    for (int e = 0; e < 8; ++e) o[e] = bn_affine(v[e], sc[e], sh[e]);
+#pragma unroll
+    for (int e = 0; e < 8; ++e) o[e] += (float)(T)bn_relu(bn_affine(vd[e], scd[e], shd[e]), 0);
+#pragma unroll
+    for (int e = 0; e < 8; ++e) o[e] = bn_relu(o[e], relu);
+}
 template <typename T, bool SH>
 __device__ __forceinline__ void bn_store8(T* __restrict__ z, _Float16* __restrict__ z16, unsigned char* __restrict__ mask, size_t off, size_t mi,
                                           const float (&o)[8]) {
@@ -357,22 +369,28 @@
     shift[c] = beta[c] - rm[c] * sc;
 }
 
-template <typename T, typename TY = T, bool SH = false>
+template <typename T, typename TY = T, bool SH = false, bool DS = false>
 __global__ void bn_apply_k(const TY* __restrict__ y, const T* __restrict__ res, T* __restrict__ z, size_t n8, int C,
                            const float* __restrict__ scale, const float* __restrict__ shift, int relu, unsigned char* __restrict__ mask = nullptr,
-                           int xcd = 0, _Float16* __restrict__ y16 = nullptr, _Float16* __restrict__ z16 = nullptr) {
+                           int xcd = 0, _Float16* __restrict__ y16 = nullptr, _Float16* __restrict__ z16 = nullptr,
+                           const float* __restrict__ scale_d = nullptr, const float* __restrict__ shift_d = nullptr) {
     const int G = C >> 3;
     const int c0 = (int)(((size_t)blockIdx.x * TPB + threadIdx.x) % G) * 8;
-    float sc[8], sh[8];
+    float sc[8], sh[8], scd[8], shd[8];
     ld8<float>(scale + c0, sc);
     ld8<float>(shift + c0, sh);
+    if constexpr (DS) {
+        ld8<float>(scale_d + c0, scd);
+        ld8<float>(shift_d + c0, shd);
+    }
     size_t i, iend, istep;
     xcd_stream_range(n8, G, xcd, i, iend, istep);
     for (; i < iend; i += istep) {
         float v[8], o[8];
         ld8<TY>(y + i * 8, v);
         if constexpr (SH) st8_f16(y16 + i * 8, v);
-        bn_apply8<T>(v, sc, sh, res, i * 8, relu, o);
+        if constexpr (DS) bn_apply8_ds<T>(v, sc, sh, res, i * 8, scd, shd, relu, o);
+        else bn_apply8<T>(v, sc, sh, res, i * 8, relu, o);
         bn_store8<T, SH>(z, z16, mask, i * 8, i, o);
     }
 }
@@ -549,46 +567,63 @@
     }
 }
 
-template <typename TY, typename TZ, bool SH = false>
+struct ChunkBn { const float* slab; int rows; const float* gamma; const float* beta; float* running_mean; float* running_var; long long* nbt; float* save; };
+__device__ __forceinline__ void chunk_fwd_coef(const double (*part)[128], int chunk, int sp, int C, double count, const float* __restrict__ gamma,
+                                               const float* __restrict__ beta, float eps, float momentum, float* __restrict__ running_mean,
+                                               float* __restrict__ running_var, long long* __restrict__ nbt, float* __restrict__ save, float* scs,
+                                               float* shs) {
+    const int col = threadIdx.x, c = chunk * 64 + col;
+    double s1 = 0.0, s2 = 0.0;
+#pragma unroll
+    for (int k = 0; k < 8; ++k) { s1 += part[k][col]; s2 += part[k][64 + col]; }
+    double mean, var;
+    bn_stats_finish(s1, s2, count, mean, var);
+    const float invstd = bn_invstd(var, eps);
+    const float sc = bn_scale(gamma[c], invstd);
+    scs[col] = sc;
+    shs[col] = bn_shift(beta[c], (float)mean, sc);
+    if (sp == 0) {
+        const double unb = bn_unbiased_var(var, count);
+        save[c] = (float)mean;
+        save[C + c] = invstd;
+        save[2 * C + c] = (float)unb;
+        if (running_mean) bn_running_update1(running_mean, running_var, c, momentum, (float)mean, (float)unb);
+        if (c == 0 && nbt) *nbt += 1;
+    }
+}
+template <typename TY, typename TZ, bool SH = false, bool DS = false>
 __global__ __launch_bounds__(TPB) void bn_apply_chunk_k(const TY* __restrict__ y, const TZ* __restrict__ res, TZ* __restrict__ z,
                                                         size_t npix, int C, const float* __restrict__ slab, int rows, double count,
                                                         const float* __restrict__ gamma, const float* __restrict__ beta, float eps,
                                                         float momentum, float* __restrict__ running_mean, float* __restrict__ running_var,
                                                         long long* __restrict__ nbt, float* __restrict__ save, int relu, int P,
                                                         unsigned char* __restrict__ mask, int xcd, _Float16* __restrict__ y16 = nullptr,
-                                                        _Float16* __restrict__ z16 = nullptr) {
+                                                        _Float16* __restrict__ z16 = nullptr, ChunkBn ds = ChunkBn{}) {
     __shared__ double part[8][128];
     __shared__ float scs[64], shs[64];
+    __shared__ float scds[DS ? 64 : 1], shds[DS ? 64 : 1];
     int chunk, sp;
     xcd_chunk_of(xcd, chunk, sp);
     slab_colsum64(slab, rows, C, chunk, part);
     __syncthreads();
-    if (threadIdx.x < 64) {
-        const int col = threadIdx.x, c = chunk * 64 + col;
-        double s1 = 0.0, s2 = 0.0;
-#pragma unroll
-        for (int k = 0; k < 8; ++k) { s1 += part[k][col]; s2 += part[k][64 + col]; }
-        double mean, var;
-        bn_stats_finish(s1, s2, count, mean, var);
-        const float invstd = bn_invstd(var, eps);
-        const float sc = bn_scale(gamma[c], invstd);
-        scs[col] = sc;
-        shs[col] = bn_shift(beta[c], (float)mean, sc);
-        if (sp == 0) {
-            const double unb = bn_unbiased_var(var, count);
-            save[c] = (float)mean;
-            save[C + c] = invstd;
-            save[2 * C + c] = (float)unb;
-            if (running_mean) bn_running_update1(running_mean, running_var, c, momentum, (float)mean, (float)unb);
-            if (c == 0 && nbt) *nbt += 1;
-        }
+    if (threadIdx.x < 64) chunk_fwd_coef(part, chunk, sp, C, count, gamma, beta, eps, momentum, running_mean, running_var, nbt, save, scs, shs);
+    if constexpr (DS) {
+        __syncthreads();
+        slab_colsum64(ds.slab, ds.rows, C, chunk, part);
+        __syncthreads();
+        if (threadIdx.x < 64)
+            chunk_fwd_coef(part, chunk, sp, C, count, ds.gamma, ds.beta, eps, momentum, ds.running_mean, ds.running_var, ds.nbt, ds.save, scds, shds);
     }
     __syncthreads();
     const int cg = threadIdx.x & 7, prow = threadIdx.x >> 3;
     const int c0 = chunk * 64 + cg * 8;
-    float sc[8], sh[8];
+    float sc[8], sh[8], scd[8], shd[8];
 #pragma unroll
     for (int e = 0; e < 8; ++e) { sc[e] = scs[cg * 8 + e]; sh[e] = shs[cg * 8 + e]; }
+    if constexpr (DS) {
+#pragma unroll
+        for (int e = 0; e < 8; ++e) { scd[e] = scds[cg * 8 + e]; shd[e] = shds[cg * 8 + e]; }
+    }
     size_t p0, p1;
     pix_range(sp, P, npix, p0, p1);
     for (size_t p = p0 + prow; p < p1; p += 32) {
@@ -596,7 +631,8 @@
         float v[8], o[8];
         ld8<TY>(y + off, v);
         if constexpr (SH) st8_f16(y16 + off, v);
-        bn_apply8<TZ>(v, sc, sh, res, off, relu, o);
+        if constexpr (DS) bn_apply8_ds<TZ>(v, sc, sh, res, off, scd, shd, relu, o);
+        else bn_apply8<TZ>(v, sc, sh, res, off, relu, o);
         bn_store8<TZ, SH>(z, z16, mask, off, off >> 3, o);
     }
 }
@@ -678,34 +714,65 @@
     }
 }
 
-template <typename DZ>
+struct DsBwd { const elem_t* yd; const float* mean; const float* invstd; float* slab; };
+__device__ __forceinline__ void ds_bwd_sums8(const DsBwd& ds, size_t off, const float (&d)[8], const float (&mud)[8], const float (&isd)[8], float (&s1)[8],
+                                             float (&s2)[8]) {
+    const float zero[8] = {0.f, 0.f, 0.f, 0.f, 0.f, 0.f, 0.f, 0.f};
+    const elem8 yyd = *(const elem8*)(ds.yd + off);
+    bn_bwd_sums8(0, d, yyd, elem8{}, zero, zero, mud, isd, s1, s2);
+}
+template <typename DZ, bool DS = false>
 __global__ __launch_bounds__(TPB) void bn_bwd_apply_pre_k(const DZ* __restrict__ g, const elem_t* __restrict__ y, elem_t* __restrict__ dy, size_t n8,
                                                           int C, const float* __restrict__ mean, const float* __restrict__ invstd,
-                                                          const float* __restrict__ coef, int xcd = 0) {
+                                                          const float* __restrict__ coef, int xcd = 0, DsBwd ds = DsBwd{}) {
     const int G = C >> 3;
     const int c0 = (int)(((size_t)blockIdx.x * TPB + threadIdx.x) % G) * 8;
-    float mu[8], is[8], ca[8], cb[8], cc[8];
+    float mu[8], is[8], ca[8], cb[8], cc[8], mud[8], isd[8], s1[8], s2[8];
     ld8<float>(mean + c0, mu);
     ld8<float>(invstd + c0, is);
     ld8<float>(coef + c0, ca);
     ld8<float>(coef + C + c0, cb);
     ld8<float>(coef + 2 * C + c0, cc);
+    if constexpr (DS) {
+        ld8<float>(ds.mean + c0, mud);
+        ld8<float>(ds.invstd + c0, isd);
+#pragma unroll
+        for (int e = 0; e < 8; ++e) { s1[e] = 0.f; s2[e] = 0.f; }
+    }
     size_t i, iend, istep;
     xcd_stream_range(n8, G, xcd, i, iend, istep);
     for (; i < iend; i += istep) {
         float d[8];
         ld8<DZ>(g + i * 8, d);
         const elem8 yy = *(const elem8*)(y + i * 8);
+        if constexpr (DS) ds_bwd_sums8(ds, i * 8, d, mud, isd, s1, s2);
         *(elem8*)(dy + i * 8) = bn_bwd_dy8(d, yy, mu, is, ca, cb, cc);
     }
-}
-
-template <typename DZ>
+    if constexpr (DS) {
+        __shared__ float red[TPB][17];
+#pragma unroll
+        for (int e = 0; e < 8; ++e) { red[threadIdx.x][e] = s1[e]; red[threadIdx.x][8 + e] = s2[e]; }
+        __syncthreads();
+        if ((int)threadIdx.x < G) {
+            float a[16];
+#pragma unroll
+            for (int e = 0; e < 16; ++e) a[e] = 0.f;
+            for (int k = 0; k < TPB / G; ++k)
+#pragma unroll
+                for (int e = 0; e < 16; ++e) a[e] += red[threadIdx.x + k * G][e];
+            float* sp = ds.slab + (size_t)blockIdx.x * 2 * C;
+#pragma unroll
+            for (int e = 0; e < 8; ++e) { sp[c0 + e] = a[e]; sp[C + c0 + e] = a[8 + e]; }
+        }
+    }
+}
+
+template <typename DZ, bool DS = false>
 __global__ __launch_bounds__(TPB) void bn_bwd_apply_pre_chunk_k(const DZ* __restrict__ g, const elem_t* __restrict__ y, elem_t* __restrict__ dy,
                                                                 size_t npix, int C, const float* __restrict__ mean,
                                                                 const float* __restrict__ invstd, const float* __restrict__ gamma,
                                                                 const float* __restrict__ slab, int rows, int P, float* __restrict__ dgamma,
-                                                                float* __restrict__ dbeta, float beta_acc, int xcd) {
+                                                                float* __restrict__ dbeta, float beta_acc, int xcd, DsBwd ds = DsBwd{}) {
     __shared__ double part[8][128];
     __shared__ double tot[2][64];
     int chunk, sp;
@@ -722,11 +789,17 @@
     if (sp == 0 && threadIdx.x < 64 && dgamma) bwd_param_acc(dgamma, dbeta, chunk * 64 + threadIdx.x, beta_acc, tot[0][threadIdx.x], tot[1][threadIdx.x]);
     const int cg = threadIdx.x & 7, prow = threadIdx.x >> 3;
     const int c0 = chunk * 64 + cg * 8;
-    float mu[8], is[8], ga[8], ca[8], cb[8], cc[8];
+    float mu[8], is[8], ga[8], ca[8], cb[8], cc[8], mud[8], isd[8], s1[8], s2[8];
     ld8<float>(mean + c0, mu);
     ld8<float>(invstd + c0, is);
     ld8<float>(gamma + c0, ga);
     chunk_bwd_coef8(tot, cg, (double)npix, ga, is, ca, cb, cc);
+    if constexpr (DS) {
+        ld8<float>(ds.mean + c0, mud);
+        ld8<float>(ds.invstd + c0, isd);
+#pragma unroll
+        for (int e = 0; e < 8; ++e) { s1[e] = 0.f; s2[e] = 0.f; }
+    }
     size_t p0, p1;
     pix_range(sp, P, npix, p0, p1);
     for (size_t p = p0 + prow; p < p1; p += 32) {
@@ -734,7 +807,20 @@
         float d[8];
         ld8<DZ>(g + off, d);
         const elem8 yy = *(const elem8*)(y + off);
+        if constexpr (DS) ds_bwd_sums8(ds, off, d, mud, isd, s1, s2);
         *(elem8*)(dy + off) = bn_bwd_dy8(d, yy, mu, is, ca, cb, cc);
+    }
+    if constexpr (DS) {
+        __shared__ float red[32][8][17];
+#pragma unroll
+        for (int e = 0; e < 8; ++e) { red[prow][cg][e] = s1[e]; red[prow][cg][8 + e] = s2[e]; }
+        __syncthreads();
+        if (threadIdx.x < 128) {
+            const int gq = threadIdx.x >> 4, e = threadIdx.x & 15;
+            float a = 0.f;
+            for (int k = 0; k < 32; ++k) a += red[k][gq][e];
+            ds.slab[((size_t)sp * 2 + (e >> 3)) * C + chunk * 64 + gq * 8 + (e & 7)] = a;
+        }
     }
 }
 
@@ -1001,6 +1087,23 @@
     hipLaunchKernelGGL((bn_apply_chunk_k<elem_t, elem_t>), dim3(g.chunks, g.S), dim3(TPB), 0, s, y, res, z, npix, C, slab, rows, (double)npix, gamma, beta, eps,
                        momentum, rm, rv, nbt, save, relu, g.P, mask, xcd);
     return udapose_check_launch() == UDAPOSE_OK ? 1 : UDAPOSE_ERR_LAUNCH;
+}
+int pw_bn_train_fused_takes(size_t npix, int C, int rows, int enabled) {
+    ChunkGeom g;
+    int xcd;
+    return fused_fwd_geometry(npix, C, rows, enabled, g, xcd);
+}
+int pw_bn_train_fused_ds(hipStream_t s, const elem_t* y, const elem_t* yd, elem_t* z, size_t npix, int C, const float* slab, int rows,
+                         const float* gamma, const float* beta, float* rm, float* rv, long long* nbt, float* save, const float* slab_d, int rows_d,
+                         const float* gamma_d, const float* beta_d, float* rm_d, float* rv_d, long long* nbt_d, float* save_d, float momentum, float eps,
+                         int relu, int enabled, unsigned char* mask) {
+    ChunkGeom g, gd;
+    int xcd;
+    if (!fused_fwd_geometry(npix, C, rows_d, enabled, gd, xcd) || !fused_fwd_geometry(npix, C, rows, enabled, g, xcd)) return UDAPOSE_ERR_ARG;
+    hipLaunchKernelGGL((bn_apply_chunk_k<elem_t, elem_t, false, true>), dim3(g.chunks, g.S), dim3(TPB), 0, s, y, yd, z, npix, C, slab, rows, (double)npix, gamma,
+                       beta, eps, momentum, rm, rv, nbt, save, relu, g.P, mask, xcd, (_Float16*)nullptr, (_Float16*)nullptr,
+                       ChunkBn{slab_d, rows_d, gamma_d, beta_d, rm_d, rv_d, nbt_d, save_d});
+    return udapose_check_launch();
 }
 int pw_bn_train_fused_split(hipStream_t s, const float* y, const void* res, void* z, size_t npix, int C, const float* slab, int rows,
                             const float* gamma, const float* beta, float* rm, float* rv, long long* nbt, float momentum, float eps, float* save,
@@ -1126,6 +1229,15 @@
     hipLaunchKernelGGL(bn_apply_k<elem_t>, dim3(grid), dim3(TPB), 0, s, y, res, z, n / 8, C, scale, shift, relu, mask, ok);
     return udapose_check_launch();
 }
+int pw_bn_apply_ds(hipStream_t s, const elem_t* y, const elem_t* yd, elem_t* z, size_t n, int C, const float* scale, const float* shift,
+                   const float* scale_d, const float* shift_d, int relu, unsigned char* mask, int xcd) {
+    if (C % 8 || n % 8 || !yd || !scale_d || !shift_d) return UDAPOSE_ERR_ARG;
+    const int grid = bn_apply_grid(n / 8, C);
+    const int ok = xcd && pw_bn_apply_xcd_ok(n / 8, C);
+    hipLaunchKernelGGL((bn_apply_k<elem_t, elem_t, false, true>), dim3(grid), dim3(TPB), 0, s, y, yd, z, n / 8, C, scale, shift, relu, mask, ok,
+                       (_Float16*)nullptr, (_Float16*)nullptr, scale_d, shift_d);
+    return udapose_check_launch();
+}
 int pw_bn_apply_split(hipStream_t s, const float* y, const void* res, void* z, size_t n, int C, const float* scale, const float* shift, int relu,
                       void* y16, void* z16, unsigned char* mask, int xcd) {
     if (C % 8 || n % 8) return UDAPOSE_ERR_ARG;
@@ -1197,9 +1309,9 @@
     });
     return udapose_check_launch();
 }
-int pw_bn_bwd_pre(hipStream_t s, const void* g, int g_is_f32, const elem_t* y, elem_t* dy, size_t npix, int C, const float* gamma, const float* mean,
-                  const float* invstd, const float* slab, int rows, float* coef, float* dgamma, float* dbeta, float beta_acc, int chunked,
-                  int legacy) {
+static int bn_bwd_pre_impl(hipStream_t s, const void* g, int g_is_f32, const elem_t* y, elem_t* dy, size_t npix, int C, const float* gamma, const float* mean,
+                           const float* invstd, const float* slab, int rows, float* coef, float* dgamma, float* dbeta, float beta_acc, int chunked,
+                           int legacy, const DsBwd* ds, int* rows_d) {
     const int G = C / 8;
     if (C % 8 || G > 256 || (G & (G - 1)) || rows < 1) return UDAPOSE_ERR_UNSUPPORTED;
     const int xcd = (chunked >> 30) & 1, xcd_stream = (chunked >> 29) & 1;
@@ -1207,11 +1319,18 @@
     if (pw_bn_bwd_pre_takes_chunked(npix, C, rows, chunked)) {
         const ChunkGeom cg = chunk_geometry(npix, C, chunked);
         with_grad_type(g, g_is_f32, [&](auto d) {
-            hipLaunchKernelGGL(bn_bwd_apply_pre_chunk_k<pointee_t<decltype(d)>>, dim3(cg.chunks, cg.S), dim3(TPB), 0, s, d, y, dy, npix, C, mean, invstd, gamma, slab,
-                               rows, cg.P, dgamma, dbeta, beta_acc, xcd);
+            using DZ = pointee_t<decltype(d)>;
+            if (ds)
+                hipLaunchKernelGGL((bn_bwd_apply_pre_chunk_k<DZ, true>), dim3(cg.chunks, cg.S), dim3(TPB), 0, s, d, y, dy, npix, C, mean, invstd, gamma, slab, rows,
+                                   cg.P, dgamma, dbeta, beta_acc, xcd, *ds);
+            else
+                hipLaunchKernelGGL(bn_bwd_apply_pre_chunk_k<DZ>, dim3(cg.chunks, cg.S), dim3(TPB), 0, s, d, y, dy, npix, C, mean, invstd, gamma, slab, rows, cg.P,
+                                   dgamma, dbeta, beta_acc, xcd);
         });
+        if (ds) *rows_d = cg.S;
         return udapose_check_launch();
     }
+    if (ds && legacy) return UDAPOSE_ERR_ARG;
     launch_bwd_finalize(s, slab, rows, C, npix, gamma, invstd, dgamma, dbeta, beta_acc, coef);
     if (legacy) {
         with_grad_type(g, g_is_f32, [&](auto d) {
@@ -1223,9 +1342,28 @@
     const int grid = bn_apply_grid(npix * G, C);
     const int ok = xcd_stream && pw_bn_apply_xcd_ok(npix * G, C);
     with_grad_type(g, g_is_f32, [&](auto d) {
-        hipLaunchKernelGGL(bn_bwd_apply_pre_k<pointee_t<decltype(d)>>, dim3(grid), dim3(TPB), 0, s, d, y, dy, npix * G, C, mean, invstd, coef, ok);
+        using DZ = pointee_t<decltype(d)>;
+        if (ds) hipLaunchKernelGGL((bn_bwd_apply_pre_k<DZ, true>), dim3(grid), dim3(TPB), 0, s, d, y, dy, npix * G, C, mean, invstd, coef, ok, *ds);
+        else hipLaunchKernelGGL(bn_bwd_apply_pre_k<DZ>, dim3(grid), dim3(TPB), 0, s, d, y, dy, npix * G, C, mean, invstd, coef, ok);
     });
-    return udapose_check_launch();
+    if (ds) *rows_d = grid;
+    return udapose_check_launch();
+}
+int pw_bn_bwd_pre(hipStream_t s, const void* g, int g_is_f32, const elem_t* y, elem_t* dy, size_t npix, int C, const float* gamma, const float* mean,
+                  const float* invstd, const float* slab, int rows, float* coef, float* dgamma, float* dbeta, float beta_acc, int chunked,
+                  int legacy) {
+    return bn_bwd_pre_impl(s, g, g_is_f32, y, dy, npix, C, gamma, mean, invstd, slab, rows, coef, dgamma, dbeta, beta_acc, chunked, legacy, nullptr, nullptr);
+}
+int pw_bn_bwd_pre_ds_rows(size_t npix, int C, int rows, int chunked) {
+    if (pw_bn_bwd_pre_takes_chunked(npix, C, rows, chunked & ~(3 << 29))) return chunk_geometry(npix, C, chunked & ~(3 << 29)).S;
+    return bn_apply_grid(npix * (C / 8), C);
+}
+int pw_bn_bwd_pre_ds(hipStream_t s, const void* g, int g_is_f32, const elem_t* y, elem_t* dy, size_t npix, int C, const float* gamma, const float* mean,
+                     const float* invstd, const float* slab, int rows, float* coef, float* dgamma, float* dbeta, float beta_acc, int chunked,
+                     const elem_t* yd, const float* mean_d, const float* invstd_d, float* slab_d, int* rows_d) {
+    if (!yd || !mean_d || !invstd_d || !slab_d || !rows_d) return UDAPOSE_ERR_ARG;
+    const DsBwd ds{yd, mean_d, invstd_d, slab_d};
+    return bn_bwd_pre_impl(s, g, g_is_f32, y, dy, npix, C, gamma, mean, invstd, slab, rows, coef, dgamma, dbeta, beta_acc, chunked, 0, &ds, rows_d);
 }
 int pw_maxpool3x3s2_fwd(hipStream_t s, const elem_t* x, elem_t* y, unsigned char* idx, int N, int H, int W, int C) {
     const int Ho = pool3x3s2_out(H), Wo = pool3x3s2_out(W);
diff --git a/uda_poseestimation_amd/ops.py b/uda_poseestimation_amd/ops.py
--- a/uda_poseestimation_amd/ops.py
+++ b/uda_poseestimation_amd/ops.py
@@ -242,6 +242,16 @@
     return _form(lib_for(y).udapose_bn_bwd_pre_ex(stream(), ptr(g), int(g.dtype == torch.float32), ptr(y), ptr(dy), npix, C_, ptr(gamma), ptr(mean),
                                                   ptr(invstd), ptr(slab), slab.shape[0], ptr(coef), ptr(dgamma), ptr(dbeta), float(beta_acc),
                                                   int(chunked), int(legacy)), "bn_bwd_pre_ex")
+
+
+def bn_bwd_pre_ds(g, y, dy, gamma, mean, invstd, slab, coef, dgamma, dbeta, yd, mean_d, invstd_d, slab_d, beta_acc=0.0, chunked=1):
+    npix, C_ = y.shape
+    rows_d = C.c_int(0)
+    form = _form(lib_for(y).udapose_bn_bwd_pre_ds(stream(), ptr(g), int(g.dtype == torch.float32), ptr(y), ptr(dy), npix, C_, ptr(gamma), ptr(mean),
+                                                  ptr(invstd), ptr(slab), slab.shape[0], ptr(coef), ptr(dgamma), ptr(dbeta), float(beta_acc),
+                                                  int(chunked), ptr(yd), ptr(mean_d), ptr(invstd_d), ptr(slab_d), slab_d.shape[0], C.byref(rows_d)),
+                 "bn_bwd_pre_ds")
+    return form, rows_d.value
 
 
 def bn_relu_maxpool3x3s2(x, y, idx, scale, shift):
```

After: 2065 images/sec, median of 6. 1.01x the previous value.
